# wonheeML/mtl-ssl

Measured on AMD Instinct MI355X. Metric: images/sec training, Faster R-CNN ResNet-101 + aux heads, higher is better.
Workload: dtype f32; 1 GPU; Faster R-CNN ResNet-101 + window/closeness/edgemask heads + refine, synthetic 1024x600 COCO-shaped (90 classes), per-GPU batch 2 (BASELINE.json configs[1]); global_batch=2, parallelism=dp1, pipeline_config=configs/frcnn_resnet101_coco_mtl.config

## Files before the change

### include/mtlssl_hip.h

```cpp
#ifndef MTLSSL_HIP_H_
#define MTLSSL_HIP_H_

#include <stdint.h>

#ifdef __cplusplus
extern "C" {
#endif

typedef void* mtlssl_stream_t;

#define MTLSSL_OK 0
#define MTLSSL_EINVAL (-1)
#define MTLSSL_ELAUNCH (-2)
#define MTLSSL_ECOMM (-3)

#define MTLSSL_ABI_VERSION 20

const char* mtlssl_last_error(void);
int mtlssl_abi_version(void);

int mtlssl_exp_rn(const double* x, double* y, int64_t n, mtlssl_stream_t stream);

typedef struct {
  int32_t N, H, W, C;
  int32_t K, R, S;
  int32_t OH, OW;
  int32_t stride, dilation;
  int32_t pad_t, pad_l;
  int32_t ldy;
} mtlssl_conv_desc;

#define MTLSSL_EPI_BIAS 1
#define MTLSSL_EPI_RESIDUAL 2
#define MTLSSL_EPI_RELU 4
#define MTLSSL_EPI_TANH 8
#define MTLSSL_EPI_RELU6 16
#define MTLSSL_EPI_MASK 32
#define MTLSSL_EPI_ACCUM 64
#define MTLSSL_EPI_MASK6 128

int64_t mtlssl_conv2d_workspace_bytes(const mtlssl_conv_desc* d, int mode);
int mtlssl_conv2d_fwd(const mtlssl_conv_desc* d, const float* x, const float* w,
                      const float* bias, const float* residual, float* y, int epilogue,
                      void* workspace, mtlssl_stream_t stream);
int mtlssl_conv2d_dgrad(const mtlssl_conv_desc* d, const float* dy, const float* w,
                        const float* residual, const float* mask_ref, float* dx, int epilogue,
                        void* workspace, mtlssl_stream_t stream);
int64_t mtlssl_conv2d_filter_xf_bytes(const mtlssl_conv_desc* d, int mode);
int mtlssl_conv2d_filter_xf_variant(const mtlssl_conv_desc* d, int mode);
int mtlssl_conv2d_transform_filter(const mtlssl_conv_desc* d, int mode, int variant, const float* w, float* filter_xf,
                                   mtlssl_stream_t stream);
int mtlssl_conv2d_transform_filters(int variant, int n, const void* w_ptrs, const void* xf_ptrs, const int64_t* ck,
                                    const int32_t* flip, int64_t max_ck, mtlssl_stream_t stream);
int mtlssl_conv2d_fwd_xf(const mtlssl_conv_desc* d, const float* x, const float* w, const float* bias,
                         const float* residual, float* y, int epilogue, void* workspace, const float* filter_xf,
                         int xf_variant, mtlssl_stream_t stream);
int mtlssl_conv2d_dgrad_xf(const mtlssl_conv_desc* d, const float* dy, const float* w, const float* residual,
                           const float* mask_ref, float* dx, int epilogue, void* workspace, const float* filter_xf,
                           int xf_variant, mtlssl_stream_t stream);
int64_t mtlssl_conv2d_input_xf_bytes(const mtlssl_conv_desc* d, int variant);
int mtlssl_conv2d_fwd_keep(const mtlssl_conv_desc* d, const float* x, const float* w, const float* bias,
                           const float* residual, float* y, int epilogue, void* workspace, const float* filter_xf,
                           int xf_variant, float* input_xf, int input_variant, mtlssl_stream_t stream);
int mtlssl_conv2d_wgrad_xf(const mtlssl_conv_desc* d, const float* x, const float* dy,
                           const float* out_scale, float* dw, float* dbias, float beta,
                           void* workspace, const float* input_xf, int input_variant, mtlssl_stream_t stream);
#define MTLSSL_CONV_GROUP_MAX 4
typedef struct {
  const float* w;
  float* y;
  const float* bias;
  int32_t K, ldy, epilogue, reserved;
} mtlssl_conv_group_entry;
int mtlssl_conv2d_fwd_grouped(const mtlssl_conv_desc* d, const float* x, int n, const mtlssl_conv_group_entry* entries,
                              int max_k, int sum_k, mtlssl_stream_t stream);
typedef struct {
  const float* dy;
  const float* w;
  int32_t K, ldy;
} mtlssl_conv_seg_entry;
int mtlssl_conv2d_dgrad_segmented(const mtlssl_conv_desc* d, int n, const mtlssl_conv_seg_entry* entries,
                                  const float* residual, const float* mask_ref, float* dx, int epilogue,
                                  mtlssl_stream_t stream);
int mtlssl_conv2d_wgrad_ex(const mtlssl_conv_desc* d, const float* x, const float* dy,
                           const float* out_scale, float* dw, float* dbias, const float* dbias_scale, float beta,
                           void* workspace, const float* input_xf, int input_variant, mtlssl_stream_t stream);
int64_t mtlssl_conv2d_wgrad_workspace_bytes(const mtlssl_conv_desc* d);
int mtlssl_conv2d_tile_config(const mtlssl_conv_desc* d, int mode);
int mtlssl_conv2d_force_config(const mtlssl_conv_desc* d, int mode, int cfg);
int mtlssl_conv2d_set_winograd(int mode);
int mtlssl_conv2d_set_pointwise(int on);
int mtlssl_conv2d_set_fp32_engine(int mode);
int mtlssl_conv2d_num_dispatches(const mtlssl_conv_desc* d, int mode);
#define MTLSSL_PLAN_INFO_LEN 16
#define MTLSSL_PLAN_DIRECT 0
#define MTLSSL_PLAN_PADDED 1
#define MTLSSL_PLAN_THIN 2
#define MTLSSL_PLAN_S2D 3
#define MTLSSL_PLAN_PARITY 4
#define MTLSSL_PLAN_WINO_F43 5
#define MTLSSL_PLAN_WINO_M7 6
#define MTLSSL_PLAN_VALU 7
int mtlssl_conv2d_plan_info(const mtlssl_conv_desc* d, int mode, int parity_class, int32_t* out);
int64_t mtlssl_conv2d_executed_macs(const mtlssl_conv_desc* d, int mode, int on_mfma);
int mtlssl_conv2d_wgrad(const mtlssl_conv_desc* d, const float* x, const float* dy,
                        const float* out_scale, float* dw, float* dbias, float beta,
                        void* workspace, mtlssl_stream_t stream);

int64_t mtlssl_conv2d_wgrad_grouped_workspace_bytes(const mtlssl_conv_desc* d, int n);
int mtlssl_conv2d_wgrad_grouped(const mtlssl_conv_desc* d, int n, const void* x_ptrs, const void* dy_ptrs,
                                const void* scale_ptrs, const void* dw_ptrs, float beta, void* workspace,
                                mtlssl_stream_t stream);

int mtlssl_depthwise_fwd(const mtlssl_conv_desc* d, const float* x, const float* w, const float* bias,
                         float* y, int epilogue, mtlssl_stream_t stream);
int mtlssl_depthwise_dgrad(const mtlssl_conv_desc* d, const float* dy, const float* w,
                           const float* mask_ref, float* dx, int epilogue, mtlssl_stream_t stream);
int64_t mtlssl_depthwise_wgrad_workspace_bytes(const mtlssl_conv_desc* d);
int mtlssl_depthwise_wgrad(const mtlssl_conv_desc* d, const float* x, const float* dy,
                           const float* out_scale, float* dw, float beta, void* workspace,
                           mtlssl_stream_t stream);
int64_t mtlssl_bn_param_grads_workspace_bytes(int C);
int mtlssl_bn_param_grads(const float* y, const float* g, const float* gamma, const float* beta,
                          float* dgamma, float* dbeta, int64_t rows, int C, float accum, void* workspace,
                          mtlssl_stream_t stream);

int mtlssl_avgpool_fwd(const float* x, float* y, int N, int H, int W, int C, int k, int stride, int pad_t,
                       int pad_l, int OH, int OW, mtlssl_stream_t stream);
int mtlssl_avgpool_bwd(const float* dy, float* dx, int N, int H, int W, int C, int k, int stride, int pad_t,
                       int pad_l, int OH, int OW, mtlssl_stream_t stream);
int mtlssl_copy_channels(const float* src, int src_ld, int src_c0, float* dst, int dst_ld, int dst_c0,
                         int64_t rows, int nc, int accumulate, mtlssl_stream_t stream);

int mtlssl_maxpool_fwd(const float* x, float* y, int N, int H, int W, int C, int k, int stride,
                       int pad_t, int pad_l, int OH, int OW, mtlssl_stream_t stream);
int mtlssl_maxpool_bwd(const float* x, const float* y, const float* dy, float* dx, int N, int H,
                       int W, int C, int k, int stride, int pad_t, int pad_l, int OH, int OW,
                       mtlssl_stream_t stream);
int mtlssl_maxpool_fwd_strided(const float* x, float* y, int N, int H, int W, int C, int k, int stride,
                               int pad_t, int pad_l, int OH, int OW, int ldy, mtlssl_stream_t stream);
int mtlssl_maxpool_bwd_strided(const float* x, const float* y, const float* dy, float* dx, int N, int H,
                               int W, int C, int k, int stride, int pad_t, int pad_l, int OH, int OW, int ldy,
                               mtlssl_stream_t stream);
int mtlssl_spatial_mean_fwd(const float* x, float* y, int N, int HW, int C, mtlssl_stream_t s);
int mtlssl_spatial_mean_bwd(const float* dy, float* dx, int N, int HW, int C, mtlssl_stream_t s);
int mtlssl_spatial_mean_bwd_masked(const float* dy, const float* act, float* dx, int N, int HW, int C,
                                   int relu6, mtlssl_stream_t stream);


int mtlssl_anchors_generate(float* anchors_out, int grid_h, int grid_w, const float* scales,
                            int n_scales, const float* aspect_ratios, int n_ratios, float base_h,
                            float base_w, float stride_y, float stride_x, float offset_y,
                            float offset_x, mtlssl_stream_t stream);

int mtlssl_boxes_prune_outside_window(const float* boxes, int n, float win_ymin, float win_xmin,
                                      float win_ymax, float win_xmax, int32_t* keep_idx_out,
                                      int32_t* count_out, mtlssl_stream_t stream);

int mtlssl_boxes_clip_to_window(const float* boxes, int n, float win_ymin, float win_xmin, float win_ymax,
                                float win_xmax, float* out, mtlssl_stream_t stream);
int mtlssl_gather_rows(const float* src, const int32_t* idx, float* dst, int batch, int n_src,
                       int n_idx, int row_len, mtlssl_stream_t stream);
int mtlssl_scatter_rows(const float* src, const int32_t* idx, float* dst, int batch, int n_dst,
                        int n_idx, int row_len, mtlssl_stream_t stream);

int mtlssl_boxes_decode(const float* rel_codes, const float* anchors, float* boxes_out, int batch,
                        int n, int anchors_batched, float sy, float sx, float sh, float sw,
                        mtlssl_stream_t stream);
int mtlssl_boxes_encode(const float* boxes, const float* anchors, float* codes_out, int n, float sy,
                        float sx, float sh, float sw, mtlssl_stream_t stream);

int64_t mtlssl_rpn_proposals_workspace_bytes(int batch, int n);
int mtlssl_rpn_proposals(const float* rpn_box_encodings, const float* rpn_objectness,
                         const float* anchors, int batch, int n, float img_h, float img_w,
                         float score_thresh, float iou_thresh, int max_proposals,
                         float* proposals_out, float* scores_out, int32_t* num_out,
                         void* workspace, mtlssl_stream_t stream);
int64_t mtlssl_batch_multiclass_nms_workspace_bytes(int batch, int n, int num_classes, int max_per_class);
int mtlssl_batch_multiclass_nms(const float* boxes, const float* scores, int scores_ld,
                                const int32_t* num_valid, int batch, int n, int q, int num_classes,
                                float score_thresh,
                                float iou_thresh, int max_per_class, int max_total,
                                const float* clip_window, int change_coordinate_frame, float* boxes_out,
                                float* scores_out, float* classes_out, int32_t* num_out, void* workspace,
                                mtlssl_stream_t stream);
int mtlssl_score_convert(const float* logits, float* out, int64_t rows, int C, int mode,
                         mtlssl_stream_t stream);
int64_t mtlssl_nms_workspace_bytes(int n);
int mtlssl_nms(const float* boxes, const float* scores, int n, float iou_thresh, int max_out,
               int32_t* selected_out, int32_t* num_out, void* workspace,
               mtlssl_stream_t stream);

#define MTLSSL_EVAL_NMS_MAX_SEGMENT 1024
#define MTLSSL_EVAL_NMS_STANDARD 1
#define MTLSSL_EVAL_NMS_SOFT_LINEAR 2
#define MTLSSL_EVAL_NMS_SOFT_GAUSSIAN 3
int mtlssl_eval_nms(const float* boxes, const float* scores, const int32_t* segment_offsets, int num_segments,
                    int max_segment, int nms_type, double iou_threshold, double sigma, double scale_y, double scale_x,
                    int max_output, int32_t* index_out, float* scores_out, int32_t* count_out,
                    mtlssl_stream_t stream);
int mtlssl_edgemask_agreement(const float* logits, int Hf, int Wf, const float* gt_mask, int h, int w,
                              int32_t* count_out, mtlssl_stream_t stream);
#define MTLSSL_COCO_MATCH_MAX_GT 256
int mtlssl_coco_match(const int32_t* dt_off, const int32_t* gt_off, int num_segments, int max_gt,
                      const double* dt_boxes, const double* gt_boxes, const double* gt_area, const uint8_t* gt_crowd,
                      const double* iou_thrs, int num_iou_thrs, const double* area_rng, int num_area_rng,
                      uint64_t* dt_match, uint64_t* dt_ignore, int32_t* npig, mtlssl_stream_t stream);
#define MTLSSL_PASCAL_MATCH_MAX_GT 256
#define MTLSSL_PASCAL_MATCH_LEFT_OUT 2
int mtlssl_pascal_match(const int32_t* dt_off, const int32_t* gt_off, int num_segments, int max_gt,
                        const double* dt_boxes, const double* gt_boxes, const uint64_t* gt_member,
                        double iou_threshold, int num_subsets, uint64_t* tp, uint64_t* drop, uint8_t* hit,
                        mtlssl_stream_t stream);

#define MTLSSL_AUX_MAX_GT 256
#define MTLSSL_AUX_WINDOW_ATTEMPTS 100
int mtlssl_aux_draw_windows(const float* boxes_norm, const int32_t* num, int batch, int max_gt, int num_windows,
                            double height, double width, double min_obj_size, uint32_t seed, uint32_t step,
                            uint32_t image0, float* window_boxes, mtlssl_stream_t stream);
int mtlssl_aux_window_labels(const float* boxes_norm, const float* classes_bg, const int32_t* num,
                             const float* window_boxes, int batch, int max_gt, int num_classes, int num_windows,
                             double height, double width, float* labels_out, mtlssl_stream_t stream);
int mtlssl_aux_closeness(const float* boxes_norm, const float* classes_bg, const int32_t* num, int batch, int max_gt,
                         int num_classes, double height, double width, float* closeness_out, mtlssl_stream_t stream);
int mtlssl_aux_edgemask(const float* boxes_norm, const int32_t* num, int batch, int max_gt, double height, double width,
                        int mask_size, float* edgemask_out, mtlssl_stream_t stream);

int64_t mtlssl_assign_targets_workspace_bytes(int batch, int n, int max_gt);
int mtlssl_assign_targets(const float* anchors, int anchors_batched, int batch, int n,
                          const float* gt_boxes, const int32_t* num_gt, int max_gt,
                          const float* gt_labels, int label_dim, const float* gt_extra,
                          int extra_dim, const float* unmatched_cls_target, float matched_thresh,
                          float unmatched_thresh, int force_match, int32_t* match_out,
                          float* cls_targets_out, float* cls_weights_out, float* reg_targets_out,
                          float* reg_weights_out, float* extra_targets_out, void* workspace,
                          mtlssl_stream_t stream);

int mtlssl_balanced_sample(const float* indicator, const float* labels, int batch, int n,
                           int batch_size, float positive_fraction, uint32_t seed,
                           uint32_t stream_id0, uint32_t stream_stride, float* sampled_out,
                           mtlssl_stream_t stream);

int mtlssl_sample_proposals(const float* proposals, const int32_t* num_proposals, int batch,
                            int max_p, const float* gt_boxes, const int32_t* num_gt, int max_gt,
// ... 156 lines not shown
```

### mtl_ssl_amd/csrc/conv.hip

```cpp
#include <stdlib.h>

#include <atomic>
#include <mutex>
#include <unordered_map>

#include "conv_mfma.h"
#include "conv_split.h"

namespace mtlssl {


__global__ void __launch_bounds__(256) k_wgrad_reduce(const float* ws, int nsplit, int64_t total4, int K,
                                                      const float* scale, float* dw, float beta, int main_blocks,
                                                      const float* cs_part, int cs_chunks, float* dbias,
                                                      const float* dbias_scale) {
  if ((int)blockIdx.x >= main_blocks) {
    const int lane = threadIdx.x & 63;
    const int k = ((int)blockIdx.x - main_blocks) * 4 + (threadIdx.x >> 6);
    if (k >= K) return;
    float s = 0.f;
    for (int c = lane; c < cs_chunks; c += 64) s += cs_part[(int64_t)c * K + k];
    s = wave_sum(s);
    if (dbias_scale) s *= dbias_scale[k];
    if (lane == 0) dbias[k] = beta != 0.f ? beta * dbias[k] + s : s;
    return;
  }
  const int64_t t = blockIdx.x * (int64_t)blockDim.x + threadIdx.x;
  const int64_t i = t >> 2;
  const int sl = (int)(t & 3);
  const bool live = i < total4;
  floatx4 s = {0.f, 0.f, 0.f, 0.f};
  if (live)
    for (int k = sl; k < nsplit; k += 4) s += reinterpret_cast<const floatx4*>(ws)[(int64_t)k * total4 + i];
#pragma unroll
  for (int e = 0; e < 4; ++e) {
    s[e] += __shfl_xor(s[e], 1, 64);
    s[e] += __shfl_xor(s[e], 2, 64);
  }
  if (!live || sl) return;
  if (scale) s *= *reinterpret_cast<const floatx4*>(scale + (i * 4) % K);
  floatx4* d = reinterpret_cast<floatx4*>(dw) + i;
  *d = beta != 0.f ? beta * *d + s : s;
}

__global__ void __launch_bounds__(256) k_wgrad_reduce_grouped(const float* ws, int nsplit, int64_t total4, int K,
                                                              const float* const* scale_tab, float* const* dw_tab,
                                                              float beta) {
  const int g = blockIdx.y;
  const int64_t t = blockIdx.x * (int64_t)blockDim.x + threadIdx.x;
  const int64_t i = t >> 2;
  const int sl = (int)(t & 3);
  const bool live = i < total4;
  const floatx4* w4 = reinterpret_cast<const floatx4*>(ws) + (int64_t)g * nsplit * total4;
  floatx4 s = {0.f, 0.f, 0.f, 0.f};
  if (live)
    for (int k = sl; k < nsplit; k += 4) s += w4[(int64_t)k * total4 + i];
#pragma unroll
  for (int e = 0; e < 4; ++e) {
    s[e] += __shfl_xor(s[e], 1, 64);
    s[e] += __shfl_xor(s[e], 2, 64);
  }
  if (!live || sl) return;
  const float* scale = scale_tab ? scale_tab[g] : nullptr;
  if (scale) s *= *reinterpret_cast<const floatx4*>(scale + (i * 4) % K);
  floatx4* d = reinterpret_cast<floatx4*>(dw_tab[g]) + i;
  *d = beta != 0.f ? beta * *d + s : s;
}

__global__ void k_conv_direct_fwd(ConvArgs p) {
  int64_t i = blockIdx.x * (int64_t)blockDim.x + threadIdx.x;
  int64_t total = (int64_t)p.M * p.K;
  if (i >= total) return;
  int k = i % p.K;
  int m = i / p.K;
  int ow = m % p.OW, t = m / p.OW, oh = t % p.OH, n = t / p.OH;
  float acc = 0.f;
  for (int r = 0; r < p.R; ++r) {
    int ih = oh * p.stride - p.pt + r * p.dil;
    if (ih < 0 || ih >= p.H) continue;
    for (int s = 0; s < p.S; ++s) {
      int iw = ow * p.stride - p.pl + s * p.dil;
      if (iw < 0 || iw >= p.W) continue;
      const float* xp = p.a + (((int64_t)n * p.H + ih) * p.W + iw) * p.C;
      const float* wp = p.b + ((int64_t)(r * p.S + s) * p.C) * p.K + k;
      for (int c = 0; c < p.C; ++c) acc = fmaf(xp[c], wp[(int64_t)c * p.K], acc);
    }
  }
  if (p.epi & MTLSSL_EPI_BIAS) acc += p.bias[k];
  if (p.epi & MTLSSL_EPI_RESIDUAL) acc += p.residual[i];
  if (p.epi & MTLSSL_EPI_RELU) acc = fmaxf(acc, 0.f);
  if (p.epi & MTLSSL_EPI_RELU6) acc = fminf(fmaxf(acc, 0.f), 6.f);
  if (p.epi & MTLSSL_EPI_TANH) acc = tanhf(acc);
  p.out[i] = acc;
}
__global__ void k_conv_direct_dgrad(ConvArgs p) {
  int64_t i = blockIdx.x * (int64_t)blockDim.x + threadIdx.x;
  int64_t total = (int64_t)p.M * p.C;
  if (i >= total) return;
  int c = i % p.C;
  int m = i / p.C;
  int iw = m % p.W, t = m / p.W, ih = t % p.H, n = t / p.H;
  float acc = 0.f;
  for (int r = 0; r < p.R; ++r) {
    int ny = ih + p.pt - r * p.dil;
    if (ny < 0 || ny % p.stride) continue;
    int oh = ny / p.stride;
    if (oh >= p.OH) continue;
    for (int s = 0; s < p.S; ++s) {
      int nx = iw + p.pl - s * p.dil;
      if (nx < 0 || nx % p.stride) continue;
      int ow = nx / p.stride;
      if (ow >= p.OW) continue;
      const float* gp = p.a + (((int64_t)n * p.OH + oh) * p.OW + ow) * p.K;
      const float* wp = p.b + ((int64_t)(r * p.S + s) * p.C + c) * p.K;
      for (int k = 0; k < p.K; ++k) acc = fmaf(gp[k], wp[k], acc);
    }
  }
  if (p.epi & MTLSSL_EPI_RESIDUAL) acc += p.residual[i];
  if (p.epi & MTLSSL_EPI_ACCUM) acc += p.out[i];
  if (p.epi & MASK_ANY) acc = act_mask(acc, p.mask[i], p.epi);
  p.out[i] = acc;
}
__global__ void k_conv_direct_wgrad(ConvArgs p, const float* scale, float* dw, float beta) {
  int rs = blockIdx.y, c = blockIdx.x;
  int r = rs / p.S, s = rs % p.S;
  int P = p.N * p.OH * p.OW;
  for (int k = threadIdx.x; k < p.K; k += blockDim.x) {
    float acc = 0.f;
    for (int pix = 0; pix < P; ++pix) {
      int ow = pix % p.OW, t = pix / p.OW, oh = t % p.OH, n = t / p.OH;
      int ih = oh * p.stride - p.pt + r * p.dil, iw = ow * p.stride - p.pl + s * p.dil;
      if (ih < 0 || ih >= p.H || iw < 0 || iw >= p.W) continue;
      acc = fmaf(p.a[(((int64_t)n * p.H + ih) * p.W + iw) * p.C + c], p.b[(int64_t)pix * p.K + k], acc);
    }
    if (scale) acc *= scale[k];
    int64_t o = ((int64_t)rs * p.C + c) * p.K + k;
    dw[o] = beta != 0.f ? beta * dw[o] + acc : acc;
  }
}

constexpr int STEM_MAX_CHUNKS = 512;
template <int R_, int S_, int C_>
__global__ void __launch_bounds__(256) k_conv_stem_wgrad(ConvArgs p, int pix_per_chunk, float* part) {
  constexpr int T = R_ * S_ * C_;
  const int KL = p.K <= 32 ? 32 : 64;
  const int k = threadIdx.x % KL, grp = threadIdx.x / KL, ngrp = 256 / KL;
  const int64_t P = (int64_t)p.N * p.OH * p.OW;
  int64_t p0 = (int64_t)blockIdx.x * pix_per_chunk;
  int64_t p1 = p0 + pix_per_chunk < P ? p0 + pix_per_chunk : P;
  float acc[T];
#pragma unroll
  for (int t = 0; t < T; ++t) acc[t] = 0.f;
  if (k < p.K) {
    for (int64_t pix = p0 + grp; pix < p1; pix += ngrp) {
      int ow = pix % p.OW;
      int64_t t2 = pix / p.OW;
      int oh = t2 % p.OH, n = t2 / p.OH;
      float g = p.b[pix * p.K + k];
#pragma unroll
      for (int r = 0; r < R_; ++r) {
        int ih = oh * p.stride - p.pt + r * p.dil;
#pragma unroll
        for (int s = 0; s < S_; ++s) {
// ... 1080 lines not shown
  p.b_bytes = (unsigned)((int64_t)d->R * d->S * d->C * d->K * 4);
  p.M = d->N * d->OH * d->OW;
  p.NG = d->K;
  MTLSSL_REQUIRE(desc_dense(d) || mfma_fwd_ok(d), "conv_fwd: a strided output (ldy = %d) needs C %% 16 == 0 and K >= 16", d->ldy);
  const Route r = route(d, MODE_FWD, workspace != nullptr);
  const mtlssl_conv_desc& q = r.q;
  switch (r.family == FAM_STEM_FWD ? stem_fwd_family(epi) : r.family) {
    case FAM_WINO:
      wino_fwd(d, r.wc.variant, r.wc.tile, x, w, bias, residual, y, epi, workspace, S(stream),
               (filter_xf && xf_variant == r.wc.variant) ? filter_xf : nullptr,
               (input_xf && input_variant == r.wc.variant) ? input_xf : nullptr);
      break;
    case FAM_DIRECT:
      launch_planned<MODE_FWD>(r.plan, p, (float*)workspace, S(stream));
      break;
    case FAM_PADDED: {
      float* x_pad = (float*)workspace;
      float* w_pad = (float*)((char*)workspace + r.front_a);
      hipLaunchKernelGGL(k_pad_rows, dim3(cdiv((int64_t)p.M * q.C, 256)), dim3(256), 0, S(stream), x, (int64_t)p.M, d->C, q.C, x_pad);
      (void)hipMemcpyAsync(w_pad, w, (size_t)d->C * d->K * 4, hipMemcpyDeviceToDevice, S(stream));
      (void)hipMemsetAsync(w_pad + (int64_t)d->C * d->K, 0, (size_t)(q.C - d->C) * d->K * 4, S(stream));
      launch_packed<MODE_FWD>(r, p, x_pad, w_pad, workspace, S(stream));
      break;
    }
    case FAM_THIN:
      hipLaunchKernelGGL(k_pw_thin_fwd, dim3(cdiv(p.M, 4)), dim3(256), 0, S(stream), x, w, bias, residual, y, p.M, d->C, d->K, epi);
      break;
    case FAM_GEMM_SMALL: {
      GemmArgs g{x, w, y, bias, residual, nullptr, p.M, d->K, d->C, epi, 0};
      hipLaunchKernelGGL(k_gemm_small<GM_FWD>, dim3(cdiv(g.N, 64), cdiv(g.M, 64)), dim3(256), 0, S(stream), g);
      break;
    }
    case FAM_S2D: {
      float* xs = (float*)workspace;
      float* wsf = (float*)((char*)workspace + r.front_a);
      hipLaunchKernelGGL(k_s2d_pack, dim3(cdiv((int64_t)q.N * q.H * q.W * 4, 256)), dim3(256), 0, S(stream), x, d->N, d->H, d->W,
                         d->C, d->pad_t, d->pad_l, q.H, q.W, xs);
      hipLaunchKernelGGL(k_s2d_filter, dim3(cdiv((int64_t)q.R * q.S * q.C * q.K, 256)), dim3(256), 0, S(stream), w, d->R, d->S,
                         d->C, d->K, q.R, q.S, wsf);
      launch_packed<MODE_FWD>(r, p, xs, wsf, workspace, S(stream));
      break;
    }
    case FAM_STEM_FWD: {
      dim3 grid(cdiv(d->OW, STEM_T), cdiv(d->OH, STEM_T), d->N);
      hipLaunchKernelGGL(k_conv_smallc_fwd, grid, dim3(256), stem_lds_bytes(d), S(stream), p);
      break;
    }
    default:
      hipLaunchKernelGGL(k_conv_direct_fwd, dim3(cdiv((int64_t)p.M * p.K, 256)), dim3(256), 0, S(stream), p);
  }
  return check_launch("conv2d_fwd");
}

int mtlssl_conv2d_fwd_grouped(const mtlssl_conv_desc* d, const float* x, int n, const mtlssl_conv_group_entry* entries,
                              int max_k, int sum_k, mtlssl_stream_t stream) {
  if (n <= 0) return MTLSSL_OK;
  if (int rc = check_desc(d)) return rc;
  MTLSSL_REQUIRE(is_pointwise(d) && d->dilation == 1, "fwd_grouped: pointwise problems only (1x1, stride 1, no padding)");
  MTLSSL_REQUIRE(d->C % BK == 0, "fwd_grouped: C = %d must be a multiple of %d", d->C, BK);
  MTLSSL_REQUIRE(x && entries && n <= MTLSSL_CONV_GROUP_MAX && max_k >= 16 && sum_k >= max_k, "fwd_grouped: bad arguments");
  ConvArgs p = make_args(d);
  GroupArgs ga;
  memset(&ga, 0, sizeof(ga));
  p.a = x;
  for (int i = 0; i < n; ++i) {
    const mtlssl_conv_group_entry& e = entries[i];
    MTLSSL_REQUIRE(e.w && e.y && e.K >= 16 && e.K % 4 == 0 && e.K <= max_k && (e.ldy == 0 || (e.ldy >= e.K && e.ldy % 4 == 0)) &&
                       !(e.epilogue & (MTLSSL_EPI_RESIDUAL | MASK_ANY | MTLSSL_EPI_ACCUM)) && (!(e.epilogue & MTLSSL_EPI_BIAS) || e.bias),
                   "fwd_grouped: problem %d: K = %d, ldy = %d, epilogue = %d", i, e.K, e.ldy, e.epilogue);
    ga.e[i] = e;
  }
  p.a_bytes = (unsigned)((int64_t)d->N * d->H * d->W * d->C * 4);
  p.M = d->N * d->H * d->W;
  p.NG = max_k; p.K = max_k; p.ldy = 0;
  p.nsplit = 1; p.ks_per_split = 0; p.tile_m0 = 0; p.ws_m0 = 0;
  int cfg = 2;
  double best = 1e30;
  for (int c = 0; c < NCFG; ++c) {
    const int64_t tiles = cdiv(p.M, CFG_BM[c]) * cdiv(sum_k, CFG_BN[c]);
    const double t = tile_time_us(c, tiles, d->C / CFG_BK[c], true);
    if (t < best) { best = t; cfg = c; }
  }
  p.tiles_m = (int)cdiv(p.M, CFG_BM[cfg]);
  p.tiles_n = (int)cdiv(max_k, CFG_BN[cfg]);
  dim3 grid(p.tiles_m * p.tiles_n, n, 1);
  switch (cfg) {
    case 0: hipLaunchKernelGGL((k_conv_mfma_pw_grp<128, 128>), grid, dim3(256), 0, S(stream), p, ga); break;
    case 1: hipLaunchKernelGGL((k_conv_mfma_pw_grp<128, 64>), grid, dim3(256), 0, S(stream), p, ga); break;
    case 2: hipLaunchKernelGGL((k_conv_mfma_pw_grp<64, 64>), grid, dim3(256), 0, S(stream), p, ga); break;
    default: hipLaunchKernelGGL((k_conv_mfma_pw_grp<256, 128>), grid, dim3(512), 0, S(stream), p, ga); break;
  }
  return check_launch("conv2d_fwd_grouped");
}

static int seg_dgrad_cfg_env() {
  static const int v = [] { const char* e = getenv("MTLSSL_SEG_DGRAD_CFG"); return e ? atoi(e) : -1; }();
  return v;
}
int mtlssl_conv2d_dgrad_segmented(const mtlssl_conv_desc* d, int n, const mtlssl_conv_seg_entry* entries,
                                  const float* residual, const float* mask_ref, float* dx, int epi,
                                  mtlssl_stream_t stream) {
  if (int rc = check_desc(d)) return rc;
  MTLSSL_REQUIRE(is_pointwise(d) && d->dilation == 1, "dgrad_segmented: pointwise problems only (1x1, stride 1, no padding)");
  MTLSSL_REQUIRE(entries && dx && n >= 1 && n <= MTLSSL_CONV_GROUP_MAX, "dgrad_segmented: bad arguments (n = %d)", n);
  MTLSSL_REQUIRE(d->C % 4 == 0 && d->C >= 16, "dgrad_segmented: C = %d must be a multiple of 4 and >= 16", d->C);
  MTLSSL_REQUIRE(!(epi & MASK_ANY) || mask_ref, "dgrad_segmented: mask_ref pointer required");
  MTLSSL_REQUIRE(!(epi & MTLSSL_EPI_RESIDUAL) || residual, "dgrad_segmented: residual pointer required");
  MTLSSL_REQUIRE(!(epi & ~(MTLSSL_EPI_RESIDUAL | MASK_ANY)), "dgrad_segmented: epilogue = %d (RESIDUAL / MASK / MASK6 only)", epi);
  const int64_t M = (int64_t)d->N * d->H * d->W;
  SegArgs sa;
  memset(&sa, 0, sizeof(sa));
  int sum_k = 0;
  for (int i = 0; i < n; ++i) {
    const mtlssl_conv_seg_entry& e = entries[i];
    MTLSSL_REQUIRE(e.dy && e.w && e.K >= BK && e.K % BK == 0 && (e.ldy == 0 || (e.ldy >= e.K && e.ldy % 4 == 0)),
                   "dgrad_segmented: segment %d: K = %d, ldy = %d", i, e.K, e.ldy);
    MTLSSL_REQUIRE(((M - 1) * (e.ldy ? e.ldy : e.K) + e.K) * 4 < (int64_t)1 << 32, "dgrad_segmented: segment %d exceeds 4 GiB", i);
    sa.e[i] = e;
    sum_k += e.K;
  }
  mtlssl_conv_desc q = *d;
  q.K = sum_k; q.ldy = 0;
  ConvArgs p = make_args(&q);
  p.a = entries[0].dy; p.b = entries[0].w; p.out = dx; p.residual = residual; p.mask = mask_ref; p.epi = epi;
  p.a_bytes = 0; p.b_bytes = 0;
  p.M = (int)M;
  p.NG = d->C;
  p.nsplit = 1; p.ks_per_split = 0; p.tile_m0 = 0; p.ws_m0 = 0;
  int cfg = seg_dgrad_cfg_env();
  if (cfg < 0 || cfg >= NCFG) {
    cfg = cdiv(p.M, CFG_BM[1]) * cdiv(p.NG, CFG_BN[1]) >= 512 ? 1 : 2;
  }
  p.tiles_m = (int)cdiv(p.M, CFG_BM[cfg]);
  p.tiles_n = (int)cdiv(p.NG, CFG_BN[cfg]);
  dim3 grid(p.tiles_m * p.tiles_n, 1, 1);
  switch (cfg) {
    case 0: hipLaunchKernelGGL((k_conv_mfma_pw_seg<128, 128>), grid, dim3(256), 0, S(stream), p, sa); break;
    case 1: hipLaunchKernelGGL((k_conv_mfma_pw_seg<128, 64>), grid, dim3(256), 0, S(stream), p, sa); break;
    case 2: hipLaunchKernelGGL((k_conv_mfma_pw_seg<64, 64>), grid, dim3(256), 0, S(stream), p, sa); break;
    default: hipLaunchKernelGGL((k_conv_mfma_pw_seg<256, 128>), grid, dim3(512), 0, S(stream), p, sa); break;
  }
  return check_launch("conv2d_dgrad_segmented");
}

int mtlssl_conv2d_dgrad(const mtlssl_conv_desc* d, const float* dy, const float* w,
                        const float* residual, const float* mask_ref, float* dx, int epi,
                        void* workspace, mtlssl_stream_t stream) {
  return mtlssl_conv2d_dgrad_xf(d, dy, w, residual, mask_ref, dx, epi, workspace, nullptr, -1, stream);
}

int mtlssl_conv2d_dgrad_xf(const mtlssl_conv_desc* d, const float* dy, const float* w,
                           const float* residual, const float* mask_ref, float* dx, int epi,
                           void* workspace, const float* filter_xf, int xf_variant, mtlssl_stream_t stream) {
  if (int rc = check_desc(d)) return rc;
  MTLSSL_REQUIRE(!(epi & MASK_ANY) || mask_ref, "conv_dgrad: mask_ref pointer required");
  MTLSSL_REQUIRE(!(epi & MTLSSL_EPI_RESIDUAL) || residual, "conv_dgrad: residual pointer required");
  ConvArgs p = make_args(d);
  p.a = dy; p.b = w; p.out = dx; p.residual = residual; p.mask = mask_ref; p.epi = epi;
  p.a_bytes = ydy_bytes(d);
  p.b_bytes = (unsigned)((int64_t)d->R * d->S * d->C * d->K * 4);
  p.M = d->N * d->H * d->W;
  p.NG = d->C;
  MTLSSL_REQUIRE(desc_dense(d) || mfma_dgrad_ok(d),
                 "conv_dgrad: a strided dy (ldy = %d) needs K %% 16 == 0, C %% 4 == 0 and C >= 16", d->ldy);
  const Route r = route(d, MODE_DGRAD, workspace != nullptr);
  switch (r.family) {
    case FAM_WINO:
      wino_dgrad(d, r.wc.variant, r.wc.tile, dy, w, residual, mask_ref, dx, epi, workspace, S(stream),
                 (filter_xf && xf_variant == r.wc.variant) ? filter_xf : nullptr);
      break;
    case FAM_PARITY:
      parity_dgrad(r, d, dy, w, residual, mask_ref, dx, epi, workspace, S(stream));
      break;
    case FAM_DIRECT:
      launch_planned<MODE_DGRAD>(r.plan, p, (float*)workspace, S(stream));
      break;
    case FAM_PADDED: {
      float* dy_pad = (float*)workspace;
      float* w_pad = (float*)((char*)workspace + r.front_a);
      hipLaunchKernelGGL(k_pad_rows, dim3(cdiv((int64_t)p.M * r.q.K, 256)), dim3(256), 0, S(stream), dy, (int64_t)p.M, d->K, r.q.K, dy_pad);
      hipLaunchKernelGGL(k_pad_rows, dim3(cdiv((int64_t)d->C * r.q.K, 256)), dim3(256), 0, S(stream), w, (int64_t)d->C, d->K, r.q.K, w_pad);
      launch_packed<MODE_DGRAD>(r, p, dy_pad, w_pad, workspace, S(stream));
      break;
    }
    case FAM_GEMM_SMALL: {
      GemmArgs g{dy, w, dx, nullptr, residual, mask_ref, p.M, d->C, d->K, epi, 0};
      hipLaunchKernelGGL(k_gemm_small<GM_DGRAD>, dim3(cdiv(g.N, 64), cdiv(g.M, 64)), dim3(256), 0, S(stream), g);
      break;
    }
    default:
      hipLaunchKernelGGL(k_conv_direct_dgrad, dim3(cdiv((int64_t)p.M * p.C, 256)), dim3(256), 0, S(stream), p);
  }
  return check_launch("conv2d_dgrad");
}

int mtlssl_conv2d_tile_config(const mtlssl_conv_desc* d, int mode) {
  if (!d || mode < MODE_FWD || mode > MODE_WGRAD) return -1;
  const Route r = route(d, mode);
  if (r.family == FAM_WINO) return make_code(1 + r.wc.variant, r.wc.tile);
  if (r.family != FAM_DIRECT && r.family != FAM_PARITY) return -1;
  return make_code(0, mode == MODE_WGRAD ? r.wg.cfg : r.plan.cfg);
}

int64_t mtlssl_conv2d_executed_macs(const mtlssl_conv_desc* d, int mode, int on_mfma) {
  if (!d || mode < MODE_FWD || mode > MODE_WGRAD || check_desc(d)) return 0;
  const int64_t P_out = (int64_t)d->N * d->OH * d->OW, P_in = (int64_t)d->N * d->H * d->W;
  const int64_t taps = (int64_t)d->R * d->S;
  const int64_t direct = (mode == MODE_DGRAD && d->stride == 1 ? P_in : P_out) * taps * d->C * d->K;
  const int64_t gathered = P_in * taps * d->C * d->K;
  const Route r = route(d, mode);
  const mtlssl_conv_desc& q = r.q;
  int64_t mfma = 0;
  switch (r.family) {
    case FAM_WINO: mfma = wino_input_bytes(d, r.wc.variant) / 4 * d->K; break;
    case FAM_DIRECT: mfma = mode == MODE_DGRAD ? gathered : direct; break;
    case FAM_PARITY: mfma = gathered / ((int64_t)d->stride * d->stride); break;
    case FAM_PADDED: mfma = (mode == MODE_DGRAD ? P_in : P_out) * q.C * q.K; break;
    case FAM_S2D: mfma = P_out * q.R * q.S * q.C * q.K; break;
    default: return on_mfma ? 0 : direct;
  }
  return on_mfma ? mfma : 0;
}

int mtlssl_conv2d_force_config(const mtlssl_conv_desc* d, int mode, int cfg) {
  MTLSSL_REQUIRE(d != nullptr && mode >= MODE_FWD && mode <= MODE_WGRAD, "force_config: bad arguments");
  MTLSSL_REQUIRE(cfg < CODE_END, "force_config: plan code out of range (0..%d)", CODE_END - 1);
  TunedKey k = make_key(d, mode);
  {
    std::lock_guard<std::mutex> g(tuned_mutex());
    if (cfg < 0) tuned_map().erase(k); else tuned_map()[k] = cfg;
  }
  routes_clear();
  return MTLSSL_OK;
}

int mtlssl_conv2d_set_fp32_engine(int mode) {
  const int prev = fp32_engine();
  if (mode == 0 || mode == 1) fp32_engine_ref().store(mode);
  return prev;
}

int mtlssl_conv2d_set_winograd(int mode) {
  const int prev = wino_env();
  if (mode >= 0 && mode <= 2) { wino_mode_ref().store(mode); routes_clear(); }
  return prev;
}

int mtlssl_conv2d_set_pointwise(int on) {
  const int prev = pointwise_ref().load();
  if (on == 0 || on == 1) pointwise_ref().store(on);
  return prev;
}

int mtlssl_conv2d_num_dispatches(const mtlssl_conv_desc* d, int mode) {
  if (!d) return 0;
  if (mode != MODE_FWD && mode != MODE_DGRAD) return 1;
  const Route r = route(d, mode);
  return (r.family == FAM_DIRECT || r.family == FAM_PARITY) && r.plan.tail_rows > 0 ? 2 : 1;
}

static void plan_info_gemm(const Plan& pl, int64_t M, int64_t NG, int ksteps, int32_t* out) {
  out[2] = pl.cfg; out[3] = pl.nsplit; out[4] = pl.ks_per_split;
  out[5] = pl.tail_rows; out[6] = pl.tail_rows > 0 ? pl.tail_nsplit : 0; out[7] = pl.tail_rows > 0 ? pl.tail_ks : 0;
  out[8] = ksteps; out[9] = (int32_t)M; out[10] = (int32_t)NG; out[11] = CFG_BM[pl.cfg]; out[12] = CFG_BN[pl.cfg];
}
int mtlssl_conv2d_plan_info(const mtlssl_conv_desc* d, int mode, int parity_class, int32_t* out) {
  MTLSSL_REQUIRE(d != nullptr && out != nullptr && mode >= MODE_FWD && mode <= MODE_WGRAD, "plan_info: bad arguments");
  if (int rc = check_desc(d)) return rc;
  static const int32_t PUBLIC[] = {MTLSSL_PLAN_WINO_F43, MTLSSL_PLAN_DIRECT, MTLSSL_PLAN_PARITY, MTLSSL_PLAN_PADDED, MTLSSL_PLAN_S2D,
                                   MTLSSL_PLAN_THIN,     MTLSSL_PLAN_VALU,   MTLSSL_PLAN_VALU,   MTLSSL_PLAN_VALU,   MTLSSL_PLAN_VALU};
  const Route r = route(d, mode);
  const mtlssl_conv_desc& q = r.q;
  for (int i = 0; i < MTLSSL_PLAN_INFO_LEN; ++i) out[i] = 0;
  out[0] = PUBLIC[r.family];
  out[1] = mtlssl_conv2d_tile_config(d, mode);
  out[2] = -1;
  out[14] = mtlssl_conv2d_num_dispatches(d, mode);
  const int64_t P = (int64_t)d->N * d->OH * d->OW, M = mode == MODE_FWD ? P : (int64_t)d->N * d->H * d->W;
  switch (r.family) {
    case FAM_WINO:
      if (r.wc.variant != 0) out[0] = MTLSSL_PLAN_WINO_M7;
      out[2] = r.wc.tile; out[3] = 1;
      out[9] = (int32_t)(mode == MODE_WGRAD ? d->C : M);
      out[10] = mode == MODE_DGRAD ? d->C : d->K;
      out[11] = CFG_BM[r.wc.tile]; out[12] = CFG_BN[r.wc.tile];
      break;
    case FAM_PARITY: {
      MTLSSL_REQUIRE(parity_class >= 0 && parity_class < 4, "plan_info: parity class %d of an input-parity dgrad", parity_class);
      const ParityProblem c = parity_problem(d, parity_class >> 1, parity_class & 1);
      if (c.Hs == 0 || c.Ws == 0 || c.Rs == 0 || c.Ss == 0) break;
      const Plan& pl = r.parity[parity_class];
      plan_info_gemm(pl, (int64_t)d->N * c.Hs * c.Ws, d->C, c.Rs * c.Ss * (d->K / CFG_BK[pl.cfg]), out);
      break;
    }
    case FAM_DIRECT: case FAM_PADDED: case FAM_S2D:
      if (mode == MODE_WGRAD) {
        const int cfg = r.wg.cfg;
        out[2] = cfg; out[3] = r.wg.nsplit; out[4] = r.wg.pps / CFG_BK[cfg]; out[8] = (int32_t)cdiv(P, CFG_BK[cfg]);
        out[9] = q.C; out[10] = q.K; out[11] = CFG_BM[cfg]; out[12] = CFG_BN[cfg]; out[13] = r.wg.pps;
      } else {
        plan_info_gemm(r.plan, M, mode == MODE_FWD ? q.K : q.C, q.R * q.S * ((mode == MODE_FWD ? q.C : q.K) / CFG_BK[r.plan.cfg]), out);
      }
      break;
    default: break;
  }
  return MTLSSL_OK;
}

int64_t mtlssl_conv2d_wgrad_workspace_bytes(const mtlssl_conv_desc* d) {
  if (!d) return 256;
  return colsum_bytes(d) + route(d, MODE_WGRAD).bytes;
}

static void wgrad_group_plan(const mtlssl_conv_desc* d, int n, int* cfg, int* nsplit, int* pps) {
  const int64_t P = (int64_t)d->N * d->OH * d->OW;
  const int RS = d->R * d->S;
  double best_t = 1e30;
  *cfg = 2; *nsplit = 1; *pps = (int)align_up(P, 16);
  for (int c = 0; c < NCFG; ++c) {
    const int ksteps = (int)cdiv(P, CFG_BK[c]);
    const int64_t tiles = cdiv(d->C, CFG_BM[c]) * cdiv(d->K, CFG_BN[c]) * RS * n;
    for (int s = 1; s <= 16; ++s) {
      if (s > 1 && ksteps * CFG_BK[c] / s < 128) break;
      const int per = (int)cdiv(ksteps, s), ns = (int)cdiv(ksteps, per);
      if (ns != s) continue;
      const double t = tile_time_us(c, tiles * ns, per, desc_is_pointwise(d)) + 2.0 + (double)n * RS * d->C * d->K * 4.0 * (ns + 1) / 3.0e6;
      if (t < best_t) { best_t = t; *cfg = c; *nsplit = ns; *pps = per * CFG_BK[c]; }
    }
  }
}
int64_t mtlssl_conv2d_wgrad_grouped_workspace_bytes(const mtlssl_conv_desc* d, int n) {
  if (!d || n <= 0 || check_desc(d) || !mfma_wgrad_ok(d)) return 0;
  int cfg, ns, pps;
  wgrad_group_plan(d, n, &cfg, &ns, &pps);
  return align_up((int64_t)n * ns * d->R * d->S * d->C * d->K * 4, 256);
}
int mtlssl_conv2d_wgrad_grouped(const mtlssl_conv_desc* d, int n, const void* x_ptrs, const void* dy_ptrs,
                                const void* scale_ptrs, const void* dw_ptrs, float beta, void* workspace,
                                mtlssl_stream_t stream) {
  if (n <= 0) return MTLSSL_OK;
  if (int rc = check_desc(d)) return rc;
  MTLSSL_REQUIRE(mfma_wgrad_ok(d), "wgrad_grouped: the problem is not on the MFMA path (C, K multiples of 4 and >= 16)");
  MTLSSL_REQUIRE(x_ptrs && dy_ptrs && dw_ptrs && workspace, "wgrad_grouped: null table / workspace");
  MTLSSL_REQUIRE(n <= 1024, "wgrad_grouped: at most 1024 problems per launch");
  hipStream_t st = S(stream);
  ConvArgs p = make_args(d);
  p.a_bytes = (unsigned)((int64_t)d->N * d->H * d->W * d->C * 4);
  p.b_bytes = ydy_bytes(d);
  p.a_tab = (const float* const*)x_ptrs;
  p.b_tab = (const float* const*)dy_ptrs;
  int cfg, ns, pps;
  wgrad_group_plan(d, n, &cfg, &ns, &pps);
  MTLSSL_REQUIRE((int64_t)n * ns <= 65535, "wgrad_grouped: grid too large");
  p.out = (float*)workspace;
  p.M = d->C; p.NG = d->K; p.nsplit = ns; p.pix_per_split = pps;
  launch_mfma<MODE_WGRAD>(cfg, p, dim3(1, d->R * d->S, n * ns), st);
  const int64_t total4 = (int64_t)d->R * d->S * d->C * d->K / 4;
  hipLaunchKernelGGL(k_wgrad_reduce_grouped, dim3(cdiv(total4 * 4, 256), n), dim3(256), 0, st, (const float*)workspace, ns,
                     total4, d->K, (const float* const*)scale_ptrs, (float* const*)dw_ptrs, beta);
  return check_launch("conv2d_wgrad_grouped");
}

int mtlssl_conv2d_wgrad(const mtlssl_conv_desc* d, const float* x, const float* dy,
                        const float* out_scale, float* dw, float* dbias, float beta,
                        void* workspace, mtlssl_stream_t stream) {
  return mtlssl_conv2d_wgrad_xf(d, x, dy, out_scale, dw, dbias, beta, workspace, nullptr, -1, stream);
}

int mtlssl_conv2d_wgrad_xf(const mtlssl_conv_desc* d, const float* x, const float* dy,
                           const float* out_scale, float* dw, float* dbias, float beta,
                           void* workspace, const float* input_xf, int input_variant, mtlssl_stream_t stream) {
  return mtlssl_conv2d_wgrad_ex(d, x, dy, out_scale, dw, dbias, nullptr, beta, workspace, input_xf, input_variant, stream);
}

int mtlssl_conv2d_wgrad_ex(const mtlssl_conv_desc* d, const float* x, const float* dy,
                           const float* out_scale, float* dw, float* dbias, const float* dbias_scale, float beta,
                           void* workspace, const float* input_xf, int input_variant, mtlssl_stream_t stream) {
  if (int rc = check_desc(d)) return rc;
  hipStream_t st = S(stream);
  ConvArgs p = make_args(d);
  p.a = x; p.b = dy;
  p.a_bytes = (unsigned)((int64_t)d->N * d->H * d->W * d->C * 4);
  p.b_bytes = ydy_bytes(d);
  const int ldy = desc_ldy(d);
  MTLSSL_REQUIRE(desc_dense(d) || mfma_wgrad_ok(d),
                 "conv_wgrad: a strided dy (ldy = %d) needs C, K %% 4 == 0 and C, K >= 16", d->ldy);
  int64_t P = (int64_t)d->N * d->OH * d->OW;
  MTLSSL_REQUIRE(workspace != nullptr, "conv_wgrad: workspace required");
  float* ws_main = (float*)((char*)workspace + colsum_bytes(d));
  ColsumPlan cp = colsum_plan(P, d->K);
  bool colsum_folded = false;
  auto colsum_partial = [&]() {
    const int kg = (int)cdiv(d->K, (d->K & 3) ? 1 : 4);
    dim3 grid(cdiv(kg, cp.CQ), cp.chunks);
    if (d->K & 3)
      hipLaunchKernelGGL(k_colsum_partial<float>, grid, dim3(256), 0, st, dy, (int)P, d->K, ldy, cp.per_chunk, cp.CQ,
                         (float*)workspace);
    else
      hipLaunchKernelGGL(k_colsum_partial<floatx4>, grid, dim3(256), 0, st, dy, (int)P, d->K, ldy, cp.per_chunk, cp.CQ,
                         (float*)workspace);
  };
  const Route r = route(d, MODE_WGRAD);
  switch (r.family) {
    case FAM_WINO:
      wino_wgrad(d, r.wc.variant, r.wc.tile, x, dy, out_scale, dw, beta, ws_main, st,
                 (input_xf && input_variant == r.wc.variant) ? input_xf : nullptr);
      break;
    case FAM_DIRECT: {
      const bool split = wgrad_on_split_engine(r, d);
      const int ns = split ? r.split_ns : r.wg.nsplit, pps = split ? r.split_pps : r.wg.pps;
      const bool ride = dbias && !split && ns <= COLSUM_MAX_PARTS;
      if (dbias && !ride) colsum_partial();
      p.out = ws_main;
      p.M = d->C; p.NG = d->K; p.nsplit = ns; p.pix_per_split = pps;
      p.cs_part = ride ? (float*)workspace : nullptr;
      if (split) launch_split<MODE_WGRAD, false>(p, dim3(1, d->R * d->S, ns), st);
      else launch_mfma<MODE_WGRAD>(r.wg.cfg, p, dim3(1, d->R * d->S, ns), st);
      int64_t total4 = (int64_t)d->R * d->S * d->C * d->K / 4;
      const int main_blocks = (int)cdiv(total4 * 4, 256);
      hipLaunchKernelGGL(k_wgrad_reduce, dim3(main_blocks + (dbias ? (int)cdiv(d->K, 4) : 0)), dim3(256), 0, st,
                         (const float*)ws_main, ns, total4, d->K, out_scale, dw, beta, main_blocks,
                         (const float*)workspace, ride ? ns : cp.chunks, dbias, dbias_scale);
      colsum_folded = dbias != nullptr;
      break;
    }
    case FAM_PADDED: {
      const mtlssl_conv_desc& q = r.q;
      const int ns = r.wg.nsplit;
      float* dy_pad = ws_main;
      float* ws_q = (float*)((char*)ws_main + r.front_bytes);
      hipLaunchKernelGGL(k_pad_rows, dim3(cdiv(P * q.K, 256)), dim3(256), 0, st, dy, P, d->K, q.K, dy_pad);
      ConvArgs pq = make_args(&q);
      pq.a = x; pq.b = dy_pad; pq.out = ws_q;
      pq.a_bytes = p.a_bytes; pq.b_bytes = (unsigned)(P * q.K * 4);
      pq.M = q.C; pq.NG = q.K; pq.nsplit = ns; pq.pix_per_split = r.wg.pps;
      const bool ride = dbias && (int64_t)ns * q.K <= (int64_t)COLSUM_MAX_PARTS * d->K;
      pq.cs_part = ride ? (float*)workspace : nullptr;
      launch_mfma<MODE_WGRAD>(r.wg.cfg, pq, dim3(1, 1, ns), st);
      const int main_blocks = (int)cdiv((int64_t)d->C * d->K, 256);
      hipLaunchKernelGGL(k_wgrad_reduce_unpad, dim3(main_blocks + (ride ? (int)cdiv(d->K, 256) : 0)), dim3(256), 0, st,
                         (const float*)ws_q, ns, d->C, q.K, d->K, out_scale, dw, beta, main_blocks, (const float*)workspace,
                         dbias, dbias_scale);
      colsum_folded = ride;
      break;
    }
    case FAM_GEMM_SMALL: {
      GemmArgs g{x, dy, ws_main, nullptr, nullptr, nullptr, d->C, d->K, (int)P, 0, r.wg.pps};
      hipLaunchKernelGGL(k_gemm_small<GM_WGRAD>, dim3(cdiv(g.N, 64), cdiv(g.M, 64), r.wg.nsplit), dim3(256), 0, st, g);
      int64_t total = (int64_t)d->C * d->K;
      hipLaunchKernelGGL(k_small_reduce, dim3(cdiv(total, 256)), dim3(256), 0, st, (const float*)ws_main, r.wg.nsplit,
                         total, d->K, out_scale, dw, beta);
      break;
    }
    case FAM_STEM3_WGRAD: {
      hipLaunchKernelGGL((k_conv_stem_wgrad<3, 3, 3>), dim3(r.wg.nsplit), dim3(256), 0, st, p, r.wg.pps, ws_main);
      int64_t total = (int64_t)27 * d->K;
      hipLaunchKernelGGL(k_small_reduce, dim3(cdiv(total, 256)), dim3(256), 0, st, (const float*)ws_main, r.wg.nsplit,
                         total, d->K, out_scale, dw, beta);
      break;
    }
    default:
      hipLaunchKernelGGL(k_conv_direct_wgrad, dim3(d->C, d->R * d->S), dim3(64), 0, st, p, out_scale, dw, beta);
  }
  if (dbias && !colsum_folded) {
    colsum_partial();
    hipLaunchKernelGGL(k_colsum_fold, dim3(cdiv(d->K, 4)), dim3(256), 0, st, (const float*)workspace, cp.chunks, d->K,
                       dbias, beta, dbias_scale);
  }
  return check_launch("conv2d_wgrad");
}

}
```

### mtl_ssl_amd/csrc/conv_mfma.h

```cpp
#pragma once
#include <type_traits>

#include "common.h"

namespace mtlssl {

typedef float floatx16 __attribute__((ext_vector_type(16)));
typedef float floatx4 __attribute__((ext_vector_type(4)));

enum { MODE_FWD = 0, MODE_DGRAD = 1, MODE_WGRAD = 2 };
__device__ __forceinline__ float act_mask(float g, float y, int epi) {
  bool on = y > 0.f && (!(epi & MTLSSL_EPI_MASK6) || y < 6.f);
  return on ? g : 0.f;
}
constexpr int MASK_ANY = MTLSSL_EPI_MASK | MTLSSL_EPI_MASK6;
constexpr int BK = 16;
#ifndef MTLSSL_LAB_FLAGS
#define MTLSSL_LAB_FLAGS 0
#endif
constexpr int LAB = MTLSSL_LAB_FLAGS;

struct ConvArgs {
  const float* a;
  const float* b;
  float* out;
  const float* bias;
  const float* residual;
  const float* mask;
  float* splitk_ws;
  int N, H, W, C, K, R, S, OH, OW, stride, dil, pt, pl;
  int M;
  int NG;
  int epi;
  int tiles_m, tiles_n;
  unsigned a_bytes, b_bytes;
  int nsplit;
  int ks_per_split;
  int pix_per_split;
  int tile_m0;
  int ws_m0;
  int ldy;
  float* cs_part;
  int64_t a_bs, b_bs, o_bs;
  const float* const* a_tab;
  const float* const* b_tab;
};

typedef unsigned uintx4 __attribute__((ext_vector_type(4)));
__host__ __device__ __forceinline__ int args_ldy(const ConvArgs& p) { return p.ldy ? p.ldy : p.K; }

__device__ __forceinline__ floatx4 bufload4(__amdgpu_buffer_rsrc_t rsrc, unsigned voffset,
                                            unsigned soffset) {
  return __builtin_bit_cast(floatx4, __builtin_amdgcn_raw_buffer_load_b128(rsrc, voffset, soffset, 0));
}

template <int BM, int BN, int MODE, int NW, bool PREFETCH_RES = false>
__device__ __forceinline__ void conv_epilogue(const ConvArgs& p, floatx16 (&acc)[BM / (16 * NW)][BN / 64], float* smem,
                                              int m0, int n0) {
  constexpr int WR = NW / 2, TM = BM / (32 * WR), TN = BN / 64, LDT = 36;
  const int tid = threadIdx.x, lane = tid & 63, wid = tid >> 6;
  const int wr = wid >> 1, wc = wid & 1;
  const int lo = lane & 31, hi = lane >> 5;
  if constexpr (LAB & 16)
    if (p.epi != 0x7fffffff) {
      float t = 0.f;
#pragma unroll
      for (int i = 0; i < TM; ++i)
#pragma unroll
        for (int j = 0; j < TN; ++j)
#pragma unroll
          for (int e = 0; e < 16; ++e) t += acc[i][j][e];
      if (t == 1.2345e-30f) p.out[0] = t;
      return;
    }
  const int ldo = p.NG;
  const int ldf = MODE == MODE_FWD ? args_ldy(p) : p.NG;
  float* outp = p.out;
  if constexpr (MODE == MODE_WGRAD)
    outp += ((int64_t)blockIdx.z * gridDim.y + blockIdx.y) * (int64_t)p.M * p.NG;
  const bool raw = (MODE != MODE_WGRAD) && p.nsplit > 1;
  if (raw) outp = p.splitk_ws + (int64_t)blockIdx.z * (int64_t)(p.M - p.ws_m0) * p.NG;
  if (!(p.NG & 3)) {
    float* tile = smem + wid * (32 * LDT);
    const int r_in = lane >> 3, c4 = (lane & 7) * 4;
    const bool use_res = PREFETCH_RES && !raw && (MODE == MODE_FWD || MODE == MODE_DGRAD) && (p.epi & MTLSSL_EPI_RESIDUAL);
    floatx4 res_cur[4], res_nxt[4];
    auto fetch_res = [&](int t, floatx4 (&dst)[4]) {
      const int i = t / TN, j = t % TN;
      const int col = n0 + wc * (BN / 2) + j * 32 + c4;
#pragma unroll
      for (int k = 0; k < 4; ++k) {
        const int row = m0 + wr * (BM / WR) + i * 32 + r_in + 8 * k;
        dst[k] = floatx4{0.f, 0.f, 0.f, 0.f};
        if (use_res && row < p.M && col < p.NG) dst[k] = *reinterpret_cast<const floatx4*>(p.residual + (int64_t)row * ldo + col);
      }
    };
    if constexpr (PREFETCH_RES) fetch_res(0, res_cur);
#pragma unroll
    for (int i = 0; i < TM; ++i) {
#pragma unroll
      for (int j = 0; j < TN; ++j) {
        if constexpr (PREFETCH_RES)
          if (i * TN + j + 1 < TM * TN) fetch_res(i * TN + j + 1, res_nxt);
#pragma unroll
        for (int e = 0; e < 16; ++e) tile[((e & 3) + 8 * (e >> 2) + 4 * hi) * LDT + lo] = acc[i][j][e];
        const int col = n0 + wc * (BN / 2) + j * 32 + c4;
        floatx4 bv = {0.f, 0.f, 0.f, 0.f};
        if constexpr (MODE == MODE_FWD)
          if ((p.epi & MTLSSL_EPI_BIAS) && col < p.NG && !raw) bv = *reinterpret_cast<const floatx4*>(p.bias + col);
#pragma unroll
        for (int k = 0; k < 4; ++k) {
          const int rt = r_in + 8 * k;
          floatx4 v = *reinterpret_cast<const floatx4*>(tile + rt * LDT + c4);
          const int row = m0 + wr * (BM / WR) + i * 32 + rt;
          if (row >= p.M || col >= p.NG) continue;
          if (raw) {
            *reinterpret_cast<floatx4*>(outp + (int64_t)(row - p.ws_m0) * ldo + col) = v;
            continue;
          }
          const int64_t o = (int64_t)row * ldo + col;
          const int64_t of = MODE == MODE_FWD ? (int64_t)row * ldf + col : o;
          if constexpr (MODE == MODE_FWD) {
            v += bv;
            if (p.epi & MTLSSL_EPI_RESIDUAL) v += PREFETCH_RES ? res_cur[k] : *reinterpret_cast<const floatx4*>(p.residual + o);
#pragma unroll
            for (int q = 0; q < 4; ++q) {
              if (p.epi & MTLSSL_EPI_RELU) v[q] = fmaxf(v[q], 0.f);
              if (p.epi & MTLSSL_EPI_RELU6) v[q] = fminf(fmaxf(v[q], 0.f), 6.f);
              if (p.epi & MTLSSL_EPI_TANH) v[q] = tanhf(v[q]);
            }
          } else if constexpr (MODE == MODE_DGRAD) {
            if (p.epi & MTLSSL_EPI_RESIDUAL) v += PREFETCH_RES ? res_cur[k] : *reinterpret_cast<const floatx4*>(p.residual + o);
            if (p.epi & MTLSSL_EPI_ACCUM) v += *reinterpret_cast<const floatx4*>(outp + o);
            if (p.epi & MASK_ANY) {
              floatx4 mk = *reinterpret_cast<const floatx4*>(p.mask + o);
#pragma unroll
              for (int q = 0; q < 4; ++q) v[q] = act_mask(v[q], mk[q], p.epi);
            }
          }
          *reinterpret_cast<floatx4*>(outp + of) = v;
        }
        if constexpr (PREFETCH_RES) {
#pragma unroll
          for (int k = 0; k < 4; ++k) res_cur[k] = res_nxt[k];
        }
      }
    }
    return;
  }
#pragma unroll
  for (int i = 0; i < TM; ++i) {
#pragma unroll
    for (int j = 0; j < TN; ++j) {
      const int col = n0 + wc * (BN / 2) + j * 32 + lo;
      const bool col_ok = col < p.NG;
      float bv = 0.f;
      if constexpr (MODE == MODE_FWD)
        if ((p.epi & MTLSSL_EPI_BIAS) && col_ok) bv = p.bias[col];
#pragma unroll
      for (int e = 0; e < 16; ++e) {
        const int row = m0 + wr * (BM / WR) + i * 32 + (e & 3) + 8 * (e >> 2) + 4 * hi;
        if (row >= p.M || !col_ok) continue;
        const int64_t o = (int64_t)row * ldo + col;
        const int64_t of = MODE == MODE_FWD ? (int64_t)row * ldf + col : o;
        float v = acc[i][j][e];
        if (raw) {
          outp[(int64_t)(row - p.ws_m0) * ldo + col] = v;
          continue;
        }
        if constexpr (MODE == MODE_FWD) {
          v += bv;
          if (p.epi & MTLSSL_EPI_RESIDUAL) v += p.residual[o];
          if (p.epi & MTLSSL_EPI_RELU) v = fmaxf(v, 0.f);
          if (p.epi & MTLSSL_EPI_RELU6) v = fminf(fmaxf(v, 0.f), 6.f);
          if (p.epi & MTLSSL_EPI_TANH) v = tanhf(v);
        } else if constexpr (MODE == MODE_DGRAD) {
          if (p.epi & MTLSSL_EPI_RESIDUAL) v += p.residual[o];
          if (p.epi & MTLSSL_EPI_ACCUM) v += outp[o];
          if (p.epi & MASK_ANY) v = act_mask(v, p.mask[o], p.epi);
        }
        outp[of] = v;
      }
    }
  }
}

struct SegArgs { mtlssl_conv_seg_entry e[MTLSSL_CONV_GROUP_MAX]; };
template <int BM, int BN, int MODE, int BKT, bool BATCH, bool PW = false, bool CS = false, bool SEG = false>
__device__ __forceinline__ void conv_mfma_body(ConvArgs p, const SegArgs sg = SegArgs{}) {
  static_assert(!SEG || (PW && MODE == MODE_DGRAD && !BATCH), "segments: pointwise dgrad only");
  constexpr int NW = BM > 128 ? 8 : 4, NT = 64 * NW, WR = NW / 2;
  constexpr int LDA = BM + 4, LDB = BN + 4;
  constexpr int KQ = BKT / 4;
  constexpr int RP = NT / KQ;
  constexpr int TM = BM / (32 * WR), TN = BN / 64;
  constexpr bool A_KC = (MODE != MODE_WGRAD);
  constexpr bool B_KC = (MODE == MODE_DGRAD);
  constexpr int A_LD = BM / RP, B_LD = BN / RP;
  constexpr unsigned OOB = 0xFFFFFFF0u;
  constexpr int LDT = 36;
  constexpr int SMEM_OPS = 2 * BKT * (LDA + LDB), SMEM_EPI = NW * 32 * LDT;
  __shared__ __attribute__((aligned(16))) float smem[SMEM_OPS > SMEM_EPI ? SMEM_OPS : SMEM_EPI];
  float* const sA = smem;
  float* const sB = smem + 2 * BKT * LDA;

  int nwg = p.tiles_m * p.tiles_n;
  int bid = blockIdx.x;
  {
    int q = nwg / 8, r = nwg % 8, xcd = bid % 8, loc = bid / 8;
    bid = (xcd < r ? xcd * (q + 1) : r * (q + 1) + (xcd - r) * q) + loc;
  }
  const int tile_m = bid / p.tiles_n + p.tile_m0, tile_n = bid % p.tiles_n;
  const int m0 = tile_m * BM, n0 = tile_n * BN;
  const int tid = threadIdx.x, lane = tid & 63, wid = tid >> 6;
  const int wr = wid >> 1, wc = wid & 1;
  const int lo = lane & 31, hi = lane >> 5;
  const int kq4 = (tid % KQ) * 4;

  if constexpr (BATCH) {
    p.a += (int64_t)blockIdx.y * p.a_bs;
    p.b += (int64_t)blockIdx.y * p.b_bs;
    if constexpr (MODE != MODE_WGRAD) p.out += (int64_t)blockIdx.y * p.o_bs;
  }
  if constexpr (MODE == MODE_WGRAD && !BATCH) {
    if (p.a_tab) {
      const int grp = blockIdx.z / p.nsplit;
      p.a = p.a_tab[grp];
      p.b = p.b_tab[grp];
    }
  }
  const int ldy = args_ldy(p);
  int rs_fixed = 0, pix0 = 0, pix1 = 0, ksteps, ks_begin = 0;
  if constexpr (MODE == MODE_FWD) {
    ksteps = p.R * p.S * (p.C / BKT);
  } else if constexpr (MODE == MODE_DGRAD) {
    ksteps = p.R * p.S * (p.K / BKT);
  } else {
    rs_fixed = BATCH ? 0 : blockIdx.y;
    int split = (!BATCH && p.a_tab) ? blockIdx.z % p.nsplit : blockIdx.z;
    int P = p.N * p.OH * p.OW;
    pix0 = split * p.pix_per_split;
    pix1 = min(P, pix0 + p.pix_per_split);
    ksteps = (max(pix1 - pix0, 0) + BKT - 1) / BKT;
  }
  unsigned a_rec = p.a_bytes, b_rec = p.b_bytes;
  if constexpr (PW && MODE == MODE_WGRAD) {
    a_rec = min(a_rec, (unsigned)(max(pix1, 0) * p.C) * 4u);
    b_rec = min(b_rec, (unsigned)(max(pix1, 0) * ldy) * 4u);
  }
  __amdgpu_buffer_rsrc_t rsrc_a = __builtin_amdgcn_make_buffer_rsrc(const_cast<float*>(p.a), 0, a_rec, 0x00020000);
  __amdgpu_buffer_rsrc_t rsrc_b = __builtin_amdgcn_make_buffer_rsrc(const_cast<float*>(p.b), 0, b_rec, 0x00020000);
  if constexpr (MODE != MODE_WGRAD) {
    if (p.nsplit > 1) {
      ks_begin = blockIdx.z * p.ks_per_split;
      ksteps = min(ksteps, ks_begin + p.ks_per_split);
    }
  }

  int a_base[A_LD], a_y[A_LD], a_x[A_LD], a_n[A_LD];
  bool a_ok[A_LD];
  unsigned a_voff[A_LD];
  unsigned b_base[B_LD];
  if constexpr (PW && MODE == MODE_WGRAD) {
#pragma unroll
    for (int i = 0; i < A_LD; ++i) {
      const int u = tid + NT * i;
      const int col = m0 + (u % (BM / 4)) * 4;
      a_voff[i] = col < p.M ? (unsigned)((pix0 + u / (BM / 4)) * p.C + col) * 4u : OOB;
    }
  } else if constexpr (PW) {
#pragma unroll
    for (int i = 0; i < A_LD; ++i) {
      const int m = m0 + (tid / KQ) + RP * i;
      const int ld = MODE == MODE_FWD ? p.C : ldy;
      a_voff[i] = m < p.M ? (unsigned)(m * ld + kq4) * 4u : OOB;
    }
  } else if constexpr (A_KC) {
#pragma unroll
    for (int i = 0; i < A_LD; ++i) {
      int m = m0 + (tid / KQ) + RP * i;
      a_ok[i] = m < p.M;
      int mm = a_ok[i] ? m : 0;
      if constexpr (MODE == MODE_FWD) {
        int ow = mm % p.OW, t = mm / p.OW;
        a_x[i] = ow * p.stride - p.pl;
        a_y[i] = (t % p.OH) * p.stride - p.pt;
        a_n[i] = t / p.OH;
        a_base[i] = ((a_n[i] * p.H + a_y[i]) * p.W + a_x[i]) * p.C + kq4;
      } else {
        int iw = mm % p.W, t = mm / p.W;
        a_x[i] = iw + p.pl;
        a_y[i] = (t % p.H) + p.pt;
        a_n[i] = t / p.H;
        a_base[i] = ((a_n[i] * p.OH + a_y[i]) * p.OW + a_x[i]) * ldy + kq4;
      }
    }
  }
#pragma unroll
  for (int i = 0; i < B_LD; ++i) {
    if constexpr (MODE == MODE_FWD) {
      int u = tid + NT * i;
      int col = n0 + (u % (BN / 4)) * 4;
      b_base[i] = col < p.NG ? (unsigned)((u / (BN / 4)) * p.K + col) * 4u : OOB;
    } else if constexpr (MODE == MODE_DGRAD) {
      int row = n0 + (tid / KQ) + RP * i;
      b_base[i] = row < p.NG ? (unsigned)(row * p.K + kq4) * 4u : OOB;
    } else {
      int u = tid + NT * i;
      int col = n0 + (u % (BN / 4)) * 4;
      if constexpr (PW)
        b_base[i] = col < p.NG ? (unsigned)((pix0 + u / (BN / 4)) * ldy + col) * 4u : OOB;
      else
        b_base[i] = col < p.NG ? (unsigned)col * 4u : OOB;
    }
  }

  int seg_ks0 = 0;
  int seg_b[MTLSSL_CONV_GROUP_MAX] = {0, 0, 0, 0};
  auto seg_setup = [&](auto SI) {
    constexpr int s = decltype(SI)::value;
    const int e_K = sg.e[s].K;
    const int ld = sg.e[s].ldy ? sg.e[s].ldy : e_K;
    rsrc_a = __builtin_amdgcn_make_buffer_rsrc(const_cast<float*>(sg.e[s].dy), 0, (unsigned)((p.M - 1) * ld + e_K) * 4u, 0x00020000);
    rsrc_b = __builtin_amdgcn_make_buffer_rsrc(const_cast<float*>(sg.e[s].w), 0, (unsigned)(p.NG * e_K) * 4u, 0x00020000);
#pragma unroll
    for (int i = 0; i < A_LD; ++i) {
      const int m = m0 + (tid / KQ) + RP * i;
      a_voff[i] = m < p.M ? (unsigned)(m * ld + kq4) * 4u : OOB;
    }
#pragma unroll
    for (int i = 0; i < B_LD; ++i) {
      const int row = n0 + (tid / KQ) + RP * i;
      b_base[i] = row < p.NG ? (unsigned)(row * e_K + kq4) * 4u : OOB;
    }
    seg_ks0 = seg_b[s];
  };
  if constexpr (SEG) {
    static_assert(MTLSSL_CONV_GROUP_MAX == 4, "the boundary ladder in load_tile covers four segments");
    int at = 0;
#pragma unroll
    for (int s = 0; s < MTLSSL_CONV_GROUP_MAX; ++s) {
      seg_b[s] = sg.e[s].K > 0 ? at : 0x7fffffff;
      at += sg.e[s].K / BKT;
    }
    seg_setup(std::integral_constant<int, 0>{});
  }

  int t_r = 0, t_s = 0, t_c = 0;
  if constexpr (!PW && MODE != MODE_WGRAD) {
    const int cpk = (MODE == MODE_FWD ? p.C : p.K) / BKT;
    const int rs = ks_begin / cpk;
    t_c = (ks_begin - rs * cpk) * BKT;
    t_r = rs / p.S;
    t_s = rs - t_r * p.S;
  }
  auto next_tap = [&]() {
    t_c += BKT;
    if (t_c >= (MODE == MODE_FWD ? p.C : p.K)) {
      t_c = 0;
      if (++t_s == p.S) { t_s = 0; ++t_r; }
    }
  };
  int w_n[A_LD], w_oh[A_LD], w_ow[A_LD];
  if constexpr (!PW && MODE == MODE_WGRAD) {
#pragma unroll
    for (int i = 0; i < A_LD; ++i) {
      const int pix = pix0 + (tid + NT * i) / (BM / 4);
      w_ow[i] = pix % p.OW;
      const int t = pix / p.OW;
      w_oh[i] = t % p.OH;
      w_n[i] = t / p.OH;
    }
  }

  floatx4 rA[2][A_LD], rB[2][B_LD];
  using Set0 = std::integral_constant<int, 0>;
  using Set1 = std::integral_constant<int, 1>;

  auto load_tile = [&](int ks, auto SET) {
    floatx4 (&ra)[A_LD] = rA[decltype(SET)::value];
    floatx4 (&rb)[B_LD] = rB[decltype(SET)::value];
    if constexpr (PW && MODE == MODE_WGRAD) {
      const unsigned sa = (unsigned)(ks * BKT * p.C) * 4u, sb = (unsigned)(ks * BKT * ldy) * 4u;
#pragma unroll
      for (int i = 0; i < A_LD; ++i) ra[i] = bufload4(rsrc_a, __builtin_elementwise_add_sat(a_voff[i], sa), 0);
#pragma unroll
      for (int i = 0; i < B_LD; ++i) rb[i] = bufload4(rsrc_b, __builtin_elementwise_add_sat(b_base[i], sb), 0);
    } else if constexpr (PW) {
      if constexpr (SEG) {
        if (ks == seg_b[1]) seg_setup(std::integral_constant<int, 1>{});
        else if (ks == seg_b[2]) seg_setup(std::integral_constant<int, 2>{});
        else if (ks == seg_b[3]) seg_setup(std::integral_constant<int, 3>{});
      }
      const unsigned ka = (unsigned)((SEG ? ks - seg_ks0 : ks) * BKT) * 4u;
#pragma unroll
      for (int i = 0; i < A_LD; ++i) ra[i] = bufload4(rsrc_a, a_voff[i], ka);
      const unsigned so = MODE == MODE_FWD ? (unsigned)(ks * BKT * p.K) * 4u : ka;
#pragma unroll
      for (int i = 0; i < B_LD; ++i) rb[i] = bufload4(rsrc_b, b_base[i], so);
      if constexpr (MODE == MODE_FWD)
        if (p.NG & 3) {
#pragma unroll
          for (int i = 0; i < B_LD; ++i) {
            int left = p.NG - (n0 + ((tid + NT * i) % (BN / 4)) * 4);
#pragma unroll
            for (int e = 1; e < 4; ++e) rb[i][e] = e < left ? rb[i][e] : 0.f;
          }
        }
    } else if constexpr (MODE == MODE_FWD) {
      const int dy = t_r * p.dil, dx = t_s * p.dil;
      const int tapoff = (dy * p.W + dx) * p.C + t_c;
      next_tap();
#pragma unroll
      for (int i = 0; i < A_LD; ++i) {
        int ih = a_y[i] + dy, iw = a_x[i] + dx;
        bool ok = a_ok[i] && (unsigned)ih < (unsigned)p.H && (unsigned)iw < (unsigned)p.W;
        ra[i] = bufload4(rsrc_a, ok ? (unsigned)(a_base[i] + tapoff) * 4u : OOB, 0);
      }
      unsigned so = (unsigned)(ks * BKT * p.K) * 4u;
#pragma unroll
      for (int i = 0; i < B_LD; ++i) rb[i] = bufload4(rsrc_b, b_base[i], so);
      if (p.NG & 3) {
#pragma unroll
        for (int i = 0; i < B_LD; ++i) {
          int left = p.NG - (n0 + ((tid + NT * i) % (BN / 4)) * 4);
#pragma unroll
          for (int e = 1; e < 4; ++e) rb[i][e] = e < left ? rb[i][e] : 0.f;
        }
      }
    } else if constexpr (MODE == MODE_DGRAD) {
      const int rs = t_r * p.S + t_s, k0 = t_c;
      const int dy = t_r * p.dil, dx = t_s * p.dil;
      next_tap();
      if (p.stride == 1) {
        int tapoff = k0 - (dy * p.OW + dx) * ldy;
#pragma unroll
        for (int i = 0; i < A_LD; ++i) {
          int oh = a_y[i] - dy, ow = a_x[i] - dx;
          bool ok = a_ok[i] && (unsigned)oh < (unsigned)p.OH && (unsigned)ow < (unsigned)p.OW;
          ra[i] = bufload4(rsrc_a, ok ? (unsigned)(a_base[i] + tapoff) * 4u : OOB, 0);
        }
      } else {
#pragma unroll
        for (int i = 0; i < A_LD; ++i) {
          int ny = a_y[i] - dy, nx = a_x[i] - dx;
          bool ok = a_ok[i] && ny >= 0 && nx >= 0 && (ny % p.stride == 0) && (nx % p.stride == 0);
          int oh = ny / p.stride, ow = nx / p.stride;
          ok = ok && oh < p.OH && ow < p.OW;
          int off = ((a_n[i] * p.OH + oh) * p.OW + ow) * ldy + k0 + kq4;
          ra[i] = bufload4(rsrc_a, ok ? (unsigned)off * 4u : OOB, 0);
        }
      }
      unsigned so = (unsigned)(rs * p.C * p.K + k0) * 4u;
#pragma unroll
      for (int i = 0; i < B_LD; ++i) rb[i] = bufload4(rsrc_b, b_base[i], so);
    } else {
      int r = rs_fixed / p.S, s = rs_fixed - r * p.S;
#pragma unroll
      for (int i = 0; i < A_LD; ++i) {
        int u = tid + NT * i;
        int kr = u / (BM / 4), m4 = u % (BM / 4);
        int pix = pix0 + ks * BKT + kr;
        bool ok = pix < pix1;
        const int ih = w_oh[i] * p.stride - p.pt + r * p.dil, iw = w_ow[i] * p.stride - p.pl + s * p.dil;
        ok = ok && (unsigned)ih < (unsigned)p.H && (unsigned)iw < (unsigned)p.W && (m0 + m4 * 4) < p.M;
        const int off = ((w_n[i] * p.H + ih) * p.W + iw) * p.C;
        ra[i] = bufload4(rsrc_a, ok ? (unsigned)(off + m0 + m4 * 4) * 4u : OOB, 0);
        w_ow[i] += BKT;
        while (w_ow[i] >= p.OW) {
          w_ow[i] -= p.OW;
          if (++w_oh[i] == p.OH) { w_oh[i] = 0; ++w_n[i]; }
        }
      }
#pragma unroll
      for (int i = 0; i < B_LD; ++i) {
        int u = tid + NT * i;
        int pix = pix0 + ks * BKT + u / (BN / 4);
        rb[i] = bufload4(rsrc_b, (pix < pix1 && b_base[i] != OOB) ? b_base[i] + (unsigned)(pix * ldy) * 4u : OOB, 0);
      }
    }
  };

  static_assert(!CS || (MODE == MODE_WGRAD && !BATCH), "column sums ride on the plain wgrad launch only");
  bool do_cs = false;
  floatx4 cs[CS ? B_LD : 1];
  if constexpr (CS) {
    do_cs = p.cs_part != nullptr && tile_m == 0 && rs_fixed == 0 && p.a_tab == nullptr;
#pragma unroll
    for (int i = 0; i < B_LD; ++i) cs[i] = floatx4{0.f, 0.f, 0.f, 0.f};
  }
  auto store_tile = [&](int buf, auto SET) {
    floatx4 (&ra)[A_LD] = rA[decltype(SET)::value];
    floatx4 (&rb)[B_LD] = rB[decltype(SET)::value];
    float* a = sA + buf * (BKT * LDA);
    float* b = sB + buf * (BKT * LDB);
    if constexpr (CS)
      if (do_cs) {
#pragma unroll
        for (int i = 0; i < B_LD; ++i) cs[i] += rb[i];
      }
#pragma unroll
    for (int i = 0; i < A_LD; ++i) {
      if constexpr (A_KC) {
        int row = (tid / KQ) + RP * i;
        a[(kq4 + 0) * LDA + row] = ra[i].x; a[(kq4 + 1) * LDA + row] = ra[i].y;
        a[(kq4 + 2) * LDA + row] = ra[i].z; a[(kq4 + 3) * LDA + row] = ra[i].w;
      } else {
        int u = tid + NT * i;
        *reinterpret_cast<floatx4*>(a + (u / (BM / 4)) * LDA + (u % (BM / 4)) * 4) = ra[i];
      }
    }
#pragma unroll
    for (int i = 0; i < B_LD; ++i) {
      if constexpr (B_KC) {
        int row = (tid / KQ) + RP * i;
        b[(kq4 + 0) * LDB + row] = rb[i].x; b[(kq4 + 1) * LDB + row] = rb[i].y;
        b[(kq4 + 2) * LDB + row] = rb[i].z; b[(kq4 + 3) * LDB + row] = rb[i].w;
      } else {
        int u = tid + NT * i;
        *reinterpret_cast<floatx4*>(b + (u / (BN / 4)) * LDB + (u % (BN / 4)) * 4) = rb[i];
      }
    }
  };

  floatx16 acc[TM][TN];
#pragma unroll
  for (int i = 0; i < TM; ++i)
#pragma unroll
    for (int j = 0; j < TN; ++j)
#pragma unroll
      for (int e = 0; e < 16; ++e) acc[i][j][e] = 0.f;

  const int nk = ksteps - ks_begin;
  if (nk > 0) {
    load_tile(ks_begin, Set0{});
    store_tile(0, Set0{});
  }
  if (nk > 1) load_tile(ks_begin + 1, Set1{});
  __syncthreads();
  auto kstep = [&](int it, auto next, auto spare) {
    const int cur = it & 1;
    if constexpr (!(LAB & 1))
      if (it + 2 < nk) load_tile(ks_begin + it + 2, spare);
    const float* a = sA + cur * (BKT * LDA) + wr * (BM / WR) + lo;
    const float* b = sB + cur * (BKT * LDB) + wc * (BN / 2) + lo;
    float fa[2][TM], fb[2][TN];
#pragma unroll
    for (int i = 0; i < TM; ++i) fa[0][i] = a[hi * LDA + i * 32];
#pragma unroll
    for (int j = 0; j < TN; ++j) fb[0][j] = b[hi * LDB + j * 32];
#pragma unroll
    for (int kk = 0; kk < BKT / 2; ++kk) {
      const int cs = kk & 1, ns = cs ^ 1;
      if (kk + 1 < BKT / 2) {
        const int kr = 2 * (kk + 1) + hi;
        if constexpr (LAB & 8) {
#pragma unroll
          for (int i = 0; i < TM; ++i) fa[ns][i] = fa[cs][i] * 1.0001f;
#pragma unroll
          for (int j = 0; j < TN; ++j) fb[ns][j] = fb[cs][j] * 0.9999f;
        } else {
#pragma unroll
          for (int i = 0; i < TM; ++i) fa[ns][i] = a[kr * LDA + i * 32];
#pragma unroll
          for (int j = 0; j < TN; ++j) fb[ns][j] = b[kr * LDB + j * 32];
        }
      }
      __builtin_amdgcn_sched_barrier(0);
#pragma unroll
      for (int i = 0; i < TM; ++i)
#pragma unroll
        for (int j = 0; j < TN; ++j)
          acc[i][j] = __builtin_amdgcn_mfma_f32_32x32x2f32(fa[cs][i], fb[cs][j], acc[i][j], 0, 0, 0);
      __builtin_amdgcn_sched_barrier(0);
    }
    if constexpr (!(LAB & 2))
      if (it + 1 < nk) store_tile(cur ^ 1, next);
    if constexpr (!(LAB & 4)) __syncthreads();
  };
  for (int it = 0; it < nk; it += 2) {
    kstep(it, Set1{}, Set0{});
    if (it + 1 < nk) kstep(it + 1, Set0{}, Set1{});
  }

  if constexpr (CS) {
    if (do_cs) {
      floatx4* red = reinterpret_cast<floatx4*>(smem);
#pragma unroll
      for (int i = 0; i < B_LD; ++i) red[tid + NT * i] = cs[i];
      __syncthreads();
      if (tid < BN / 4) {
        floatx4 t = red[tid];
#pragma unroll
        for (int r = 1; r < BKT; ++r) t += red[r * (BN / 4) + tid];
        const int col = n0 + tid * 4;
        if (col < p.NG) *reinterpret_cast<floatx4*>(p.cs_part + (int64_t)blockIdx.z * p.NG + col) = t;
      }
      __syncthreads();
    }
  }
  conv_epilogue<BM, BN, MODE, NW>(p, acc, smem, m0, n0);
}


template <int BM, int BN, int MODE, int BKT, int NSTAGE, bool BATCH, bool PWISE = false, bool CS = false>
__device__ __forceinline__ void conv_glds_body(ConvArgs p) {
  constexpr int NW = BM > 128 ? 8 : 4, WR = NW / 2;
  constexpr int TM = BM / (32 * WR), TN = BN / 64;
  constexpr bool A_KC = (MODE != MODE_WGRAD);
  constexpr bool B_KC = (MODE == MODE_DGRAD);
  constexpr int QPR = BKT / 4;
  constexpr int RPP = 64 / QPR;
  constexpr int RSH = QPR == 4 ? 2 : 1;
  constexpr int A_FL = BM * BKT, B_FL = BN * BKT;
  constexpr int STAGE = A_FL + B_FL;
  constexpr int PA = BM * BKT / 256 / NW, PB = BN * BKT / 256 / NW;
  constexpr int G = BKT / 8;
  constexpr unsigned OOB = 0xFFFFFFF0u;
  constexpr int LDT = 36;
  constexpr int SMEM_OPS = NSTAGE * STAGE, SMEM_EPI = NW * 32 * LDT;
  __shared__ __attribute__((aligned(16))) float smem[SMEM_OPS > SMEM_EPI ? SMEM_OPS : SMEM_EPI];
  typedef __attribute__((address_space(3))) void* lds_ptr_t;

  int nwg = p.tiles_m * p.tiles_n;
  int bid = blockIdx.x;
  {
    int q = nwg / 8, r = nwg % 8, xcd = bid % 8, loc = bid / 8;
    bid = (xcd < r ? xcd * (q + 1) : r * (q + 1) + (xcd - r) * q) + loc;
  }
  const int tile_m = bid / p.tiles_n + p.tile_m0, tile_n = bid % p.tiles_n;
  const int m0 = tile_m * BM, n0 = tile_n * BN;
  const int tid = threadIdx.x, lane = tid & 63, wid = tid >> 6;
  const int wr = wid >> 1, wc = wid & 1;
  const int lo = lane & 31, hi = lane >> 5;
  auto kc_row = [&](int piece) { return piece * RPP + lane / QPR; };
  auto kc_quad4 = [&](int row) { return (((lane % QPR) ^ ((row >> RSH) & (QPR - 1)))) * 4; };

  if constexpr (BATCH) {
    p.a += (int64_t)blockIdx.y * p.a_bs;
    p.b += (int64_t)blockIdx.y * p.b_bs;
    if constexpr (MODE != MODE_WGRAD) p.out += (int64_t)blockIdx.y * p.o_bs;
  }
  int rs_fixed = 0, pix0 = 0, pix1 = 0, ksteps, ks_begin = 0;
  if constexpr (MODE == MODE_FWD) {
    ksteps = p.R * p.S * (p.C / BKT);
  } else if constexpr (MODE == MODE_DGRAD) {
    ksteps = p.R * p.S * (p.K / BKT);
  } else {
    rs_fixed = BATCH ? 0 : blockIdx.y;
    int split = blockIdx.z;
    int P = p.N * p.OH * p.OW;
    pix0 = split * p.pix_per_split;
    pix1 = min(P, pix0 + p.pix_per_split);
    ksteps = (max(pix1 - pix0, 0) + BKT - 1) / BKT;
  }
  if constexpr (MODE != MODE_WGRAD) {
    if (p.nsplit > 1) {
      ks_begin = blockIdx.z * p.ks_per_split;
      ksteps = min(ksteps, ks_begin + p.ks_per_split);
    }
  }

  const int ldy = args_ldy(p);
  unsigned a_rec = p.a_bytes, b_rec = p.b_bytes;
  if constexpr (PWISE && MODE == MODE_WGRAD) {
    a_rec = min(a_rec, (unsigned)(max(pix1, 0) * p.C) * 4u);
    b_rec = min(b_rec, (unsigned)(max(pix1, 0) * ldy) * 4u);
  }
  const __amdgpu_buffer_rsrc_t rsrc_a = __builtin_amdgcn_make_buffer_rsrc(const_cast<float*>(p.a), 0, a_rec, 0x00020000);
  const __amdgpu_buffer_rsrc_t rsrc_b = __builtin_amdgcn_make_buffer_rsrc(const_cast<float*>(p.b), 0, b_rec, 0x00020000);

  int a_base[PA], a_y[PA], a_x[PA], a_n[PA], a_q4[PA];
  bool a_ok[PA];
  unsigned a_voff[PA];
  unsigned b_base[PB];
  if constexpr (PWISE && MODE == MODE_WGRAD) {
#pragma unroll
    for (int i = 0; i < PA; ++i) {
      const int pos = (wid * PA + i) * 64 + lane;
      const int col = m0 + (pos % (BM / 4)) * 4;
      a_voff[i] = col < p.M ? (unsigned)((pix0 + pos / (BM / 4)) * p.C + col) * 4u : OOB;
    }
  } else if constexpr (PWISE) {
#pragma unroll
    for (int i = 0; i < PA; ++i) {
      const int row = kc_row(wid * PA + i);
      const int m = m0 + row;
      a_voff[i] = m < p.M ? (unsigned)(m * (MODE == MODE_FWD ? p.C : ldy) + kc_quad4(row)) * 4u : OOB;
    }
  } else if constexpr (A_KC) {
#pragma unroll
    for (int i = 0; i < PA; ++i) {
      const int row = kc_row(wid * PA + i);
      a_q4[i] = kc_quad4(row);
      int m = m0 + row;
      a_ok[i] = m < p.M;
      int mm = a_ok[i] ? m : 0;
      if constexpr (MODE == MODE_FWD) {
        int ow = mm % p.OW, t = mm / p.OW;
        a_x[i] = ow * p.stride - p.pl;
        a_y[i] = (t % p.OH) * p.stride - p.pt;
        a_n[i] = t / p.OH;
        a_base[i] = ((a_n[i] * p.H + a_y[i]) * p.W + a_x[i]) * p.C + a_q4[i];
      } else {
        int iw = mm % p.W, t = mm / p.W;
        a_x[i] = iw + p.pl;
        a_y[i] = (t % p.H) + p.pt;
        a_n[i] = t / p.H;
        a_base[i] = ((a_n[i] * p.OH + a_y[i]) * p.OW + a_x[i]) * ldy + a_q4[i];
      }
    }
  }
#pragma unroll
  for (int i = 0; i < PB; ++i) {
    const int pos = (wid * PB + i) * 64 + lane;
    if constexpr (MODE == MODE_FWD) {
      int col = n0 + (pos % (BN / 4)) * 4;
      b_base[i] = col < p.NG ? (unsigned)((pos / (BN / 4)) * p.K + col) * 4u : OOB;
    } else if constexpr (MODE == MODE_DGRAD) {
      const int row = kc_row(wid * PB + i);
      b_base[i] = n0 + row < p.NG ? (unsigned)((n0 + row) * p.K + kc_quad4(row)) * 4u : OOB;
    } else {
      int col = n0 + (pos % (BN / 4)) * 4;
      if constexpr (PWISE)
        b_base[i] = col < p.NG ? (unsigned)((pix0 + pos / (BN / 4)) * ldy + col) * 4u : OOB;
      else
        b_base[i] = col < p.NG ? (unsigned)col * 4u : OOB;
    }
  }

  auto issue_tile = [&](int ks, int st) {
    if constexpr (LAB & 32) ks = ks_begin;
    float* sa = smem + st * STAGE + wid * (PA * 256);
    float* sb = smem + st * STAGE + A_FL + wid * (PB * 256);
    if constexpr (PWISE && MODE == MODE_WGRAD) {
      const unsigned sa_off = (unsigned)(ks * BKT * p.C) * 4u, sb_off = (unsigned)(ks * BKT * ldy) * 4u;
#pragma unroll
      for (int i = 0; i < PA; ++i)
        __builtin_amdgcn_raw_ptr_buffer_load_lds(rsrc_a, (lds_ptr_t)(sa + i * 256), 16, __builtin_elementwise_add_sat(a_voff[i], sa_off), 0, 0, 0);
#pragma unroll
      for (int i = 0; i < PB; ++i)
        __builtin_amdgcn_raw_ptr_buffer_load_lds(rsrc_b, (lds_ptr_t)(sb + i * 256), 16, __builtin_elementwise_add_sat(b_base[i], sb_off), 0, 0, 0);
    } else if constexpr (PWISE) {
      const unsigned ka = (unsigned)(ks * BKT) * 4u;
      const unsigned so = MODE == MODE_FWD ? (unsigned)(ks * BKT * p.K) * 4u : ka;
#pragma unroll
      for (int i = 0; i < PA; ++i)
        __builtin_amdgcn_raw_ptr_buffer_load_lds(rsrc_a, (lds_ptr_t)(sa + i * 256), 16, a_voff[i], ka, 0, 0);
#pragma unroll
      for (int i = 0; i < PB; ++i)
        __builtin_amdgcn_raw_ptr_buffer_load_lds(rsrc_b, (lds_ptr_t)(sb + i * 256), 16, b_base[i], so, 0, 0);
    } else if constexpr (MODE == MODE_FWD) {
      int cpk = p.C / BKT;
      int rs = ks / cpk, c0 = (ks - rs * cpk) * BKT;
      int r = rs / p.S, s = rs - r * p.S;
      int dy = r * p.dil, dx = s * p.dil;
      int tapoff = (dy * p.W + dx) * p.C + c0;
      if constexpr (!(LAB & 64)) {
#pragma unroll
        for (int i = 0; i < PA; ++i) {
          int ih = a_y[i] + dy, iw = a_x[i] + dx;
          bool ok = a_ok[i] && (unsigned)ih < (unsigned)p.H && (unsigned)iw < (unsigned)p.W;
          __builtin_amdgcn_raw_ptr_buffer_load_lds(rsrc_a, (lds_ptr_t)(sa + i * 256), 16,
                                                   ok ? (unsigned)(a_base[i] + tapoff) * 4u : OOB, 0, 0, 0);
        }
      }
      unsigned so = (unsigned)(ks * BKT * p.K) * 4u;
      if constexpr (!(LAB & 128)) {
#pragma unroll
        for (int i = 0; i < PB; ++i)
          __builtin_amdgcn_raw_ptr_buffer_load_lds(rsrc_b, (lds_ptr_t)(sb + i * 256), 16, b_base[i], so, 0, 0);
      }
    } else if constexpr (MODE == MODE_DGRAD) {
      int kpk = p.K / BKT;
      int rs = ks / kpk, k0 = (ks - rs * kpk) * BKT;
      int r = rs / p.S, s = rs - r * p.S;
      int dy = r * p.dil, dx = s * p.dil;
      if (p.stride == 1) {
        int tapoff = k0 - (dy * p.OW + dx) * ldy;
#pragma unroll
        for (int i = 0; i < PA; ++i) {
          int oh = a_y[i] - dy, ow = a_x[i] - dx;
          bool ok = a_ok[i] && (unsigned)oh < (unsigned)p.OH && (unsigned)ow < (unsigned)p.OW;
          __builtin_amdgcn_raw_ptr_buffer_load_lds(rsrc_a, (lds_ptr_t)(sa + i * 256), 16,
                                                   ok ? (unsigned)(a_base[i] + tapoff) * 4u : OOB, 0, 0, 0);
        }
      } else {
#pragma unroll
        for (int i = 0; i < PA; ++i) {
          int ny = a_y[i] - dy, nx = a_x[i] - dx;
          bool ok = a_ok[i] && ny >= 0 && nx >= 0 && (ny % p.stride == 0) && (nx % p.stride == 0);
          int oh = ny / p.stride, ow = nx / p.stride;
          ok = ok && oh < p.OH && ow < p.OW;
          int off = ((a_n[i] * p.OH + oh) * p.OW + ow) * ldy + k0 + a_q4[i];
          __builtin_amdgcn_raw_ptr_buffer_load_lds(rsrc_a, (lds_ptr_t)(sa + i * 256), 16,
                                                   ok ? (unsigned)off * 4u : OOB, 0, 0, 0);
        }
      }
      unsigned so = (unsigned)(rs * p.C * p.K + k0) * 4u;
#pragma unroll
      for (int i = 0; i < PB; ++i)
        __builtin_amdgcn_raw_ptr_buffer_load_lds(rsrc_b, (lds_ptr_t)(sb + i * 256), 16, b_base[i], so, 0, 0);
    } else {
      int r = rs_fixed / p.S, s = rs_fixed - r * p.S;
#pragma unroll
      for (int i = 0; i < PA; ++i) {
        const int pos = (wid * PA + i) * 64 + lane;
        int kr = pos / (BM / 4), m4 = pos % (BM / 4);
        int pix = pix0 + ks * BKT + kr;
        bool ok = pix < pix1;
        int off = 0;
        if (p.R == 1 && p.S == 1 && p.stride == 1) {
          off = pix * p.C;
        } else {
          int ow = pix % p.OW, t = pix / p.OW;
          int oh = t % p.OH, n = t / p.OH;
          int ih = oh * p.stride - p.pt + r * p.dil, iw = ow * p.stride - p.pl + s * p.dil;
          ok = ok && (unsigned)ih < (unsigned)p.H && (unsigned)iw < (unsigned)p.W;
          off = ((n * p.H + ih) * p.W + iw) * p.C;
        }
        ok = ok && (m0 + m4 * 4) < p.M;
        __builtin_amdgcn_raw_ptr_buffer_load_lds(rsrc_a, (lds_ptr_t)(sa + i * 256), 16,
                                                 ok ? (unsigned)(off + m0 + m4 * 4) * 4u : OOB, 0, 0, 0);
      }
#pragma unroll
      for (int i = 0; i < PB; ++i) {
        const int pos = (wid * PB + i) * 64 + lane;
        int pix = pix0 + ks * BKT + pos / (BN / 4);
        __builtin_amdgcn_raw_ptr_buffer_load_lds(
            rsrc_b, (lds_ptr_t)(sb + i * 256), 16,
            (pix < pix1 && b_base[i] != OOB) ? b_base[i] + (unsigned)(pix * ldy) * 4u : OOB, 0, 0, 0);
      }
    }
  };

  floatx16 acc[TM][TN];
#pragma unroll
  for (int i = 0; i < TM; ++i)
#pragma unroll
    for (int j = 0; j < TN; ++j)
#pragma unroll
      for (int e = 0; e < 16; ++e) acc[i][j][e] = 0.f;

  int fa_off[TM], fb_off[TN];
#pragma unroll
  for (int i = 0; i < TM; ++i) {
    const int row = wr * (BM / WR) + i * 32 + lo;
    fa_off[i] = A_KC ? row * BKT + (((hi * (QPR / 2)) ^ ((row >> RSH) & (QPR - 1))) * 4) : hi * (BKT / 2) * BM + row;
  }
#pragma unroll
  for (int j = 0; j < TN; ++j) {
    const int col = wc * (BN / 2) + j * 32 + lo;
    fb_off[j] = B_KC ? col * BKT + (((hi * (QPR / 2)) ^ ((col >> RSH) & (QPR - 1))) * 4) : hi * (BKT / 2) * BN + col;
  }

  const int nk = ksteps - ks_begin;
  constexpr int NDMA = ((LAB & 64) ? 0 : PA) + ((LAB & 128) ? 0 : PB);
#pragma unroll
  for (int s = 0; s < NSTAGE - 1; ++s)
    if (s < nk) issue_tile(ks_begin + s, s);
  if (NSTAGE == 3 && nk > 1) asm volatile("s_waitcnt vmcnt(%0)" ::"n"(NDMA) : "memory");
  else asm volatile("s_waitcnt vmcnt(0)" ::: "memory");
  __builtin_amdgcn_s_barrier();
  asm volatile("" ::: "memory");

  bool do_cs = false;
  float csum = 0.f;
  static_assert(!CS || (MODE == MODE_WGRAD && !BATCH), "column sums ride on the plain wgrad launch only");
  if constexpr (CS) do_cs = p.cs_part != nullptr && tile_m == 0 && rs_fixed == 0;
  int cur = 0, nxt = NSTAGE - 1;
  for (int it = 0; it < nk; ++it) {
    const bool more = it + NSTAGE - 1 < nk;
    if constexpr (!(LAB & 1))
      if (more) issue_tile(ks_begin + it + NSTAGE - 1, nxt);
    const float* a = smem + cur * STAGE;
    const float* b = a + A_FL;
    if constexpr (CS)
      if (do_cs && tid < BN) {
#pragma unroll
        for (int k = 0; k < BKT; ++k) csum += b[k * BN + tid];
      }
    float fa[TM][BKT / 2], fb[TN][BKT / 2];
    auto read_group = [&](auto GI) {
      constexpr int g = decltype(GI)::value;
#pragma unroll
      for (int i = 0; i < TM; ++i) {
        if constexpr (A_KC) {
          floatx4 v = *reinterpret_cast<const floatx4*>(a + (fa_off[i] ^ (g * 4)));
          fa[i][4 * g + 0] = v.x; fa[i][4 * g + 1] = v.y; fa[i][4 * g + 2] = v.z; fa[i][4 * g + 3] = v.w;
        } else {
#pragma unroll
          for (int t = 0; t < 4; ++t) fa[i][4 * g + t] = a[fa_off[i] + (4 * g + t) * BM];
        }
      }
#pragma unroll
      for (int j = 0; j < TN; ++j) {
        if constexpr (B_KC) {
          floatx4 v = *reinterpret_cast<const floatx4*>(b + (fb_off[j] ^ (g * 4)));
          fb[j][4 * g + 0] = v.x; fb[j][4 * g + 1] = v.y; fb[j][4 * g + 2] = v.z; fb[j][4 * g + 3] = v.w;
        } else {
#pragma unroll
          for (int t = 0; t < 4; ++t) fb[j][4 * g + t] = b[fb_off[j] + (4 * g + t) * BN];
        }
      }
    };
    auto mma = [&](int t) {
#pragma unroll
      for (int i = 0; i < TM; ++i)
#pragma unroll
        for (int j = 0; j < TN; ++j)
          acc[i][j] = __builtin_amdgcn_mfma_f32_32x32x2f32(fa[i][t], fb[j][t], acc[i][j], 0, 0, 0);
    };
    if constexpr (LAB & 8) {
#pragma unroll
      for (int t = 0; t < BKT / 2; ++t) {
#pragma unroll
        for (int i = 0; i < TM; ++i) fa[i][t] = (float)(lane + it + t) * 1e-3f;
#pragma unroll
        for (int j = 0; j < TN; ++j) fb[j][t] = (float)(lane - it - t) * 1e-3f;
      }
#pragma unroll
      for (int t = 0; t < BKT / 2; ++t) mma(t);
    } else {
      read_group(std::integral_constant<int, 0>{});
      auto group = [&](auto GI) {
        constexpr int g = decltype(GI)::value;
        __builtin_amdgcn_sched_barrier(0);
        mma(4 * g);
        __builtin_amdgcn_sched_barrier(0);
        if constexpr (g + 1 < G) read_group(std::integral_constant<int, g + 1>{});
        __builtin_amdgcn_sched_barrier(0);
        mma(4 * g + 1); mma(4 * g + 2); mma(4 * g + 3);
      };
      group(std::integral_constant<int, 0>{});
      group(std::integral_constant<int, 1>{});
      if constexpr (G > 2) {
        group(std::integral_constant<int, 2>{});
        group(std::integral_constant<int, 3>{});
      }
    }
    __builtin_amdgcn_sched_barrier(0);
    if constexpr (!(LAB & 4)) {
      if (NSTAGE == 3 && more) asm volatile("s_waitcnt vmcnt(%0)" ::"n"(NDMA) : "memory");
      else asm volatile("s_waitcnt vmcnt(0)" ::: "memory");
      __builtin_amdgcn_s_barrier();
    }
    asm volatile("" ::: "memory");
    cur = cur + 1 == NSTAGE ? 0 : cur + 1;
    nxt = nxt + 1 == NSTAGE ? 0 : nxt + 1;
  }
  if constexpr (CS)
    if (do_cs && tid < BN && n0 + tid < p.NG) p.cs_part[(int64_t)blockIdx.z * p.NG + n0 + tid] = csum;
  conv_epilogue<BM, BN, MODE, NW>(p, acc, smem, m0, n0);
}

template <int BM, int BN, int BKT, int NSTAGE>
constexpr int glds_waves() {
  constexpr int lds = NSTAGE * (BM + BN) * BKT * 4;
  constexpr int nw = BM > 128 ? 8 : 4;
  constexpr int blocks = 163840 / lds;
  constexpr int w = blocks * nw / 4;
  return w > 4 ? 4 : (w < 1 ? 1 : w);
}
template <int BM, int BN, int MODE, int BKT, int NSTAGE>
__global__ void __launch_bounds__(BM > 128 ? 512 : 256, (glds_waves<BM, BN, BKT, NSTAGE>()))
k_conv_glds(ConvArgs p) {
  conv_glds_body<BM, BN, MODE, BKT, NSTAGE, false>(p);
}
template <int BM, int BN, int MODE, int BKT, int NSTAGE>
__global__ void __launch_bounds__(BM > 128 ? 512 : 256, (glds_waves<BM, BN, BKT, NSTAGE>()))
k_conv_glds_pw(ConvArgs p) {
  conv_glds_body<BM, BN, MODE, BKT, NSTAGE, false, true>(p);
}
template <int BM, int BN, int BKT, int NSTAGE>
__global__ void __launch_bounds__(BM > 128 ? 512 : 256, (glds_waves<BM, BN, BKT, NSTAGE>()))
k_conv_glds_cs(ConvArgs p) {
  conv_glds_body<BM, BN, MODE_WGRAD, BKT, NSTAGE, false, false, true>(p);
}
template <int BM, int BN, int BKT, int NSTAGE>
__global__ void __launch_bounds__(BM > 128 ? 512 : 256, (glds_waves<BM, BN, BKT, NSTAGE>()))
k_conv_glds_pw_cs(ConvArgs p) {
  conv_glds_body<BM, BN, MODE_WGRAD, BKT, NSTAGE, false, true, true>(p);
}
template <int BM, int BN, int MODE, int BKT, int NSTAGE>
__global__ void __launch_bounds__(BM > 128 ? 512 : 256, (glds_waves<BM, BN, BKT, NSTAGE>()))
k_wino_glds(ConvArgs p) {
  conv_glds_body<BM, BN, MODE, BKT, NSTAGE, true, true>(p);
}

template <int BM, int BN, int MODE, int BKT>
__global__ void __launch_bounds__(BM > 128 ? 512 : 256, (BM > 128 ? 2 : BM * BN >= 128 * 128 ? (BKT > 16 ? 2 : 3) : 4))
k_conv_mfma(ConvArgs p) {
  conv_mfma_body<BM, BN, MODE, BKT, false>(p);
}
template <int BM, int BN, int MODE>
__global__ void __launch_bounds__(BM > 128 ? 512 : 256, (BM > 128 ? 2 : BM * BN >= 128 * 128 ? 3 : 4))
k_conv_mfma_pw(ConvArgs p) {
  conv_mfma_body<BM, BN, MODE, 16, false, true>(p);
}
template <int BM, int BN, int BKT>
__global__ void __launch_bounds__(BM > 128 ? 512 : 256, (BM > 128 ? 2 : BM * BN >= 128 * 128 ? (BKT > 16 ? 2 : 3) : 4))
k_conv_mfma_cs(ConvArgs p) {
  conv_mfma_body<BM, BN, MODE_WGRAD, BKT, false, false, true>(p);
}
template <int BM, int BN>
__global__ void __launch_bounds__(BM > 128 ? 512 : 256, (BM > 128 ? 2 : BM * BN >= 128 * 128 ? 3 : 4))
k_conv_mfma_pw_cs(ConvArgs p) {
  conv_mfma_body<BM, BN, MODE_WGRAD, 16, false, true, true>(p);
}
struct GroupArgs { mtlssl_conv_group_entry e[MTLSSL_CONV_GROUP_MAX]; };
template <int BM, int BN>
__global__ void __launch_bounds__(BM > 128 ? 512 : 256, (BM > 128 ? 2 : BM * BN >= 128 * 128 ? 3 : 4))
k_conv_mfma_pw_grp(ConvArgs p, GroupArgs g) {
  static_assert(MTLSSL_CONV_GROUP_MAX == 4, "the select chain below covers four problems");
  const int gy = blockIdx.y;
  const mtlssl_conv_group_entry e = gy == 0 ? g.e[0] : gy == 1 ? g.e[1] : gy == 2 ? g.e[2] : g.e[3];
  p.b = e.w; p.out = e.y; p.bias = e.bias;
  p.NG = e.K; p.K = e.K; p.ldy = e.ldy; p.epi = e.epilogue;
  p.b_bytes = (unsigned)(p.C * e.K) * 4u;
  p.tiles_n = (e.K + BN - 1) / BN;
  if ((int)blockIdx.x >= p.tiles_m * p.tiles_n) return;
  conv_mfma_body<BM, BN, MODE_FWD, 16, false, true>(p);
}
template <int BM, int BN>
__global__ void __launch_bounds__(BM > 128 ? 512 : 256, (BM > 128 ? 2 : BM * BN >= 128 * 128 ? 3 : 4))
k_conv_mfma_pw_seg(ConvArgs p, SegArgs g) {
  conv_mfma_body<BM, BN, MODE_DGRAD, 16, false, true, false, true>(p, g);
// ... 51 lines not shown
```

### mtl_ssl_amd/frcnn.py

```python
import os

import torch

from . import nn, ops

f32, i32 = torch.float32, torch.int32


def _init_from_hyperparams(hp):
    ini = hp.initializer
    which = ini.which_oneof(["truncated_normal_initializer", "variance_scaling_initializer"])
    if which == "truncated_normal_initializer":
        return ("truncated_normal", float(ini.truncated_normal_initializer.stddev))
    if which == "variance_scaling_initializer":
        v = ini.variance_scaling_initializer
        return ("variance_scaling", float(v.factor), str(v.mode), bool(v.uniform))
    return ("variance_scaling", 1.0, "FAN_AVG", True)


def _l2_from_hyperparams(hp):
    reg = hp.regularizer
    if reg.has("l2_regularizer"):
        return float(reg.l2_regularizer.weight)
    return 0.0
# ... 555 lines not shown
        clo = pd["closeness_predictions"] if mtl.closeness else None
        net = ops.refine_concat(cls, win, clo, B, N2, self.N_EXPAND, bool(mtl.global_closeness))
        hidden, sctx = net, None
        if self.refine_stack is not None:
            hidden, sctx = self.refine_stack.forward(net, self._is_training, self.seed, self.step)
        refined = self.refine_fc.forward(hidden)
        pd["_refine_hidden"], pd["_refine_ctx"] = hidden, sctx
        if mtl.refine_residue:
            ops.axpby(cls, refined, 1.0, 1.0)
        pd["mtl_refined_class_predictions_with_background"] = refined
        pd["_refine_in"] = net
        return pd

    def postprocess(self, pd):
        c = self.cfg
        B, H, W, _ = pd["image_shape"]
        if c.first_stage_only:
            boxes, scores, num = ops.rpn_proposals(
                pd["rpn_box_encodings"], pd["rpn_objectness_predictions_with_background"], pd["anchors"],
                H, W, c.first_stage_nms_score_threshold, c.first_stage_nms_iou_threshold,
                int(c.first_stage_max_proposals))
            if self._is_training:
                gt = self._format_groundtruth_data(H, W)
                _, norm, num = self._second_stage_proposals(boxes, num, gt, H, W)
                return {"detection_boxes": norm, "num_detections": num}
            return {"detection_boxes": ops.scale_channels(boxes, self._hw_scales(H, W)[1]), "detection_scores": scores,
                    "num_detections": num}
        key = "mtl_refined_class_predictions_with_background"
        cls = pd[key] if (self._mtl.refine and key in pd) else pd["class_predictions_with_background"]
        N, K = self.max_num_proposals, self.num_classes
        enc = pd["refined_box_encodings"].reshape(1, B * N * K, 4).contiguous()
        tiled = pd["proposal_boxes"].view(B, N, 1, 4).expand(B, N, K, 4).reshape(B * N * K, 4).contiguous()
        boxes = ops.boxes_decode(enc, tiled).view(B, N, K, 4)
        pp = c.second_stage_post_processing
        conv = ops.score_convert(cls.reshape(B * N, K + 1).contiguous(), pp.score_converter).view(B, N, K + 1)
        nms = pp.batch_non_max_suppression
        ob, os_, oc, on = ops.batch_multiclass_nms(
            boxes, conv, nms.score_threshold, nms.iou_threshold, int(nms.max_detections_per_class),
            int(nms.max_total_detections), clip_window=[0.0, 0.0, float(H), float(W)],
            change_coordinate_frame=True, num_valid=pd["num_proposals"], col0=1, num_classes=K)
        return {"detection_boxes": ob, "detection_scores": os_, "detection_classes": oc, "num_detections": on}

    def loss(self, pd, loss_scale=1.0, part="all"):
        second = not self._first_stage_only
        new = {}
        if part == "late":
            losses, d, cls_s = pd["_losses_early"], pd["_d"], pd["_cls_s"]
        else:
            losses, d, cls_s = {}, {}, None
            self._loss_rpn(pd, self.step, losses, new, True)
            if second:
                cls_s = self._loss_box_classifier(pd, losses, new, True)
                self._loss_window_class(pd, losses, new, True)
            self._loss_edgemask(pd, losses, new, True)
        if part == "early":
            pd["_losses_early"], pd["_cls_s"] = losses, cls_s
        elif second:
            self._loss_refined_classifier(pd, cls_s, losses, new, True)
        g = float(loss_scale)
        if g != 1.0:
            for t in new.values():
                ops.axpby(t, t, g, 0.0)
        d.update(new)
        pd["_d"] = d
        return losses

    def eval_loss(self, pd, image_index=0):
        if self._is_training:
            raise ValueError("eval_loss is the loss of an inference model; a training model calls loss()")
        if self._hard_miner is not None:
            raise ValueError("eval_config.calc_loss with a hard_example_miner is not supported")
        second = not self._first_stage_only
        losses = {}
        self._loss_rpn(pd, int(image_index), losses, None, False)
        if second:
            cls_s = self._loss_box_classifier(pd, losses, None, False)
            if self._mtl.window and self._window["classes"].numel() == 0:
                losses["window_class_loss"] = torch.zeros((1,), dtype=f32, device=self.ps.device)
            else:
                self._loss_window_class(pd, losses, None, False)
        self._loss_edgemask(pd, losses, None, False)
        if second:
            self._loss_refined_classifier(pd, cls_s, losses, None, False)
        return losses

    def _unmatched_class_targets(self):
        if "um" not in self._consts:
            dev = self.ps.device
            self._consts["um"] = torch.zeros((1,), dtype=f32, device=dev)
            self._consts["um2"] = torch.tensor([1.0] + [0.0] * self.num_classes, dtype=f32, device=dev)
        return self._consts["um"], self._consts["um2"]

    def _loss_rpn(self, pd, draw, losses, d, want_grad):
        c = self.cfg
        B, H, W, _ = pd["image_shape"]
        gt = self._format_groundtruth_data(H, W)
        anchors = pd["anchors"]
        n = anchors.shape[0]
        um, _ = self._unmatched_class_targets()
        tg = ops.assign_targets(anchors, gt["boxes_abs"], gt["num"], None, um, 0.7, 0.3, True)
        cls_t = tg["cls_targets"].view(B, n)
        sampled = ops.balanced_sample(tg["cls_weights"], cls_t, int(c.first_stage_minibatch_size),
                                      c.first_stage_positive_balance_fraction, self.seed,
                                      (2 * draw * 65536) & 0xFFFFFFFF, 2)
        loc_s, obj_s = ops.rpn_loss_scales(sampled, tg["reg_weights"],
                                           c.first_stage_localization_loss_weight / B,
                                           c.first_stage_objectness_loss_weight / B)
        rl, d_enc = ops.smooth_l1(pd["rpn_box_encodings"], tg["reg_targets"], loc_s, 3.0, want_grad=want_grad)
        losses["first_stage_localization_loss"] = ops.reduce_sum(rl)
        rl, d_obj = ops.softmax_ce(pd["rpn_objectness_predictions_with_background"], ops.onehot2(cls_t), obj_s,
                                   want_grad=want_grad)
        losses["first_stage_objectness_loss"] = ops.reduce_sum(rl)
        if want_grad:
            d["rpn_box_encodings"], d["rpn_objectness"] = d_enc, d_obj
        pd["_rpn_targets"] = dict(tg, sampled=sampled)

    def _loss_box_classifier(self, pd, losses, d, want_grad):
        c, mtl = self.cfg, self._mtl
        B, H, W, _ = pd["image_shape"]
        gt = self._format_groundtruth_data(H, W)
        N2, K1 = self.max_num_proposals, self.num_classes + 1
        _, um2 = self._unmatched_class_targets()
        dt = ops.assign_targets(pd["proposal_boxes"], gt["boxes_abs"], gt["num"], gt["classes_bg"], um2,
                                0.5, 0.5, False, gt_extra=gt["closeness"] if mtl.closeness else None)
        cls_s, loc_s2, clo_s = ops.detector_loss_scales(
            dt["cls_weights"], dt["reg_weights"], pd["num_proposals"],
            dt.get("extra_targets") if mtl.closeness else None,
            c.second_stage_classification_loss_weight, c.second_stage_localization_loss_weight,
            mtl.closeness_loss_weight)
        cls_targets = dt["cls_targets"].view(B * N2, K1)
        rl_loc, d_box = ops.box_select_smooth_l1(pd["refined_box_encodings"], cls_targets,
                                                 dt["reg_targets"].view(B * N2, 4), loc_s2.view(-1), 1.0,
                                                 want_grad=want_grad)
        rl_cls, d_cls = ops.softmax_ce(pd["class_predictions_with_background"], cls_targets, cls_s.view(-1),
                                       want_grad=want_grad)
        if self._hard_miner is not None:
            hm = self._hard_miner
            lm, cm, sel, nsel = ops.hard_example_mining(rl_loc.view(B, N2), rl_cls.view(B, N2), pd["proposal_boxes"],
                                                        pd["num_proposals"], d_box, d_cls, hm["num_hard_examples"],
                                                        hm["iou_threshold"], hm["loss_type"])
            rl_loc, rl_cls = lm, cm
            pd["_mined"] = (sel, nsel)
        losses["second_stage_localization_loss"] = ops.reduce_sum(rl_loc)
        losses["second_stage_classification_loss"] = ops.reduce_sum(rl_cls)
        if want_grad:
            d["refined_box_encodings"], d["class_predictions"] = d_box, d_cls
        pd["_det_targets"] = dt
        if mtl.closeness:
            rl, d_clo = ops.softmax_ce(pd["closeness_predictions"], dt["extra_targets"].view(B * N2, K1),
                                       clo_s.view(-1), col0=1, want_grad=want_grad)
            losses["closeness_classification_loss"] = ops.reduce_sum(rl)
            if want_grad:
                d["closeness_predictions"] = d_clo
        return cls_s

    def _loss_refined_classifier(self, pd, cls_s, losses, d, want_grad):
        c, mtl = self.cfg, self._mtl
        if not mtl.refine:
            return
        dt = pd["_det_targets"]
        rs = cls_s if c.second_stage_classification_loss_weight == mtl.refined_classification_loss_weight \
            else ops.detector_loss_scales(dt["cls_weights"], dt["reg_weights"], pd["num_proposals"], None,
                                          mtl.refined_classification_loss_weight, 0.0, 0.0)[0]
        cls_targets = dt["cls_targets"].view(-1, self.num_classes + 1)
        rl, d_ref = ops.softmax_ce(pd["mtl_refined_class_predictions_with_background"], cls_targets, rs.view(-1),
                                   want_grad=want_grad)
        losses["refined_classification_loss"] = ops.reduce_sum(rl)
        if want_grad:
            d["refined_class_predictions"] = d_ref

    def _loss_window_class(self, pd, losses, d, want_grad):
        mtl = self._mtl
        if not mtl.window:
            return
        wc = self._window["classes"].view(-1, self.num_classes + 1)
        ws = torch.full((wc.shape[0],), mtl.window_class_loss_weight / wc.shape[0], dtype=f32, device=self.ps.device)
        rl, d_win = ops.softmax_ce(pd["window_class_predictions"], wc, ws, want_grad=want_grad)
        losses["window_class_loss"] = ops.reduce_sum(rl)
        if want_grad:
            d["window_class_predictions"] = d_win

    def _loss_edgemask(self, pd, losses, d, want_grad):
        mtl = self._mtl
        if not mtl.edgemask:
            return
        B = pd["image_shape"][0]
        em = self._edgemask
        mh, mw = em.shape[2], em.shape[3]
        tgt, sc = ops.edgemask_targets(em, mtl.edgemask_loss_weight / (B * mh * mw))
        pr = ops.resize_bilinear_fwd(pd["edgemask_predictions"], mh, mw)
        rl, d_pr = ops.softmax_ce(pr, tgt, sc.view(-1), want_grad=want_grad)
        losses["edgemask_loss"] = ops.reduce_sum(rl)
        if want_grad:
            d["edgemask_resized"] = d_pr

    def _backward_refiner(self, pd, d):
        mtl = self._mtl
        d_ref = d["refined_class_predictions"]
        self.refine_fc.wgrad(pd["_refine_hidden"], d_ref)
        if self.refine_stack is not None:
            g_h = self.refine_fc.dgrad(pd["_refine_hidden"].shape, d_ref)
            self.refine_stack.backward(pd["_refine_ctx"], g_h, need_input_grad=False)
        if mtl.refine_residue and not mtl.stop_gradient_for_prediction_org:
            ops.axpby(d_ref, d["class_predictions"], 1.0, 1.0)

    def backward(self, pd):
        mtl = self._mtl
        d = pd["_d"]
        F = pd["rpn_features_to_crop"]
        B = F.shape[0]
        if self._first_stage_only:
            dF = torch.zeros_like(F)
            return self._backward_first_stage(pd, d, F, dF, B)
        dF = torch.empty_like(F)
        if mtl.refine:
            self._backward_refiner(pd, d)
        d_cls = d["class_predictions"]
        c = self.cfg
        feat = pd["_feat"]
        g_feat = self.box_predictor.backward(pd["_bp"], d_cls, d["refined_box_encodings"].view(feat.shape[0], -1),
                                             feat.shape, **self.tower.out_mask(feat))
        stop = bool(mtl.stop_gradient_for_aux_tasks)
        shared = self._shared_classifier
        gw_shared = None
        if shared:
            if mtl.closeness:
                gcl = self.closeness_predictor.backward(pd["_cp"], d["closeness_predictions"], None, feat.shape,
                                                        need_feat_grad=not stop, **self.tower.out_mask(feat))
                if not stop:
                    ops.axpby(gcl, g_feat, 1.0, 1.0)
            if mtl.window and not stop:
                wfeat = pd["_wfeat"]
                g = self.window_predictor.backward(pd["_wp"], d["window_class_predictions"], None, wfeat.shape,
                                                   **self.window_tower.out_mask(wfeat))
                hook, self.ps.grad_ready_hook = self.ps.grad_ready_hook, None
                gw_shared = self.tower.backward(g, wfeat, pd["_wctx"], need_input_grad=True, masked=True)
                self.ps.grad_ready_hook = hook
        crop_args = (int(c.initial_crop_size), int(c.maxpool_kernel_size), int(c.maxpool_stride))

        def aux_backward(collect=None):
            if shared:
                if mtl.window and stop:
                    wfeat = pd["_wfeat"]
                    self.window_predictor.backward(pd["_wp"], d["window_class_predictions"], None, wfeat.shape,
                                                   need_feat_grad=False)
                return
            todo = []
            if mtl.closeness:
                cfeat = pd["_cfeat"]
                g = self.closeness_predictor.backward(pd["_cp"], d["closeness_predictions"], None, cfeat.shape,
                                                      **self.closeness_tower.out_mask(cfeat))
                gc = self.closeness_tower.backward(g, cfeat, pd["_cctx"], need_input_grad=not stop, masked=True)
                if not stop:
                    todo.append((gc, pd["_argmax"], pd["proposal_boxes_normalized"].view(-1, 4), pd["_box_ind"]))
            if mtl.window:
                wfeat = pd["_wfeat"]
                g = self.window_predictor.backward(pd["_wp"], d["window_class_predictions"], None, wfeat.shape,
                                                   **self.window_tower.out_mask(wfeat))
                gw = self.window_tower.backward(g, wfeat, pd["_wctx"], need_input_grad=not stop, masked=True)
                if not stop:
                    todo.append((gw, pd["_wargmax"], pd["_wboxes"], pd["_wbox_ind"]))
            if collect is not None:
                collect.extend(todo)
            else:
                for gx, am, bx, bi in todo:
                    ops.roi_crop_pool_bwd(gx, am, F.shape, bx, bi, *crop_args, dfeat=dF)

        cur = torch.cuda.current_stream()
        aux = self._aux_stream() if (mtl.closeness or mtl.window) else None
        pending = []
        if aux is not None and not shared:
            aux.wait_stream(cur)
            with torch.cuda.stream(aux):
                aux_backward(collect=pending)
        g_crops = self.tower.backward(g_feat, feat, pd["_tower_ctx"], need_input_grad=True, masked=True,
                                      wgrad=nn.INLINE_WGRAD if shared else self._wgrad_exec())
        ops.roi_crop_pool_bwd(g_crops, pd["_argmax"], F.shape, pd["proposal_boxes_normalized"].view(-1, 4),
                              pd["_box_ind"], *crop_args, dfeat=dF, accumulate=False)
        if gw_shared is not None:
            ops.roi_crop_pool_bwd(gw_shared, pd["_wargmax"], F.shape, pd["_wboxes"], pd["_wbox_ind"], *crop_args, dfeat=dF)
        if pending:
            ops.wait_on(aux, "backward: aux towers released early", cur)
            for gx, am, bx, bi in pending:
                gx.record_stream(cur)
                ops.roi_crop_pool_bwd(gx, am, F.shape, bx, bi, *crop_args, dfeat=dF)
        if aux is None:
            aux_backward()
        elif shared and stop:
            aux.wait_stream(cur)
            with torch.cuda.stream(aux):
                aux_backward()
        return self._backward_first_stage(pd, d, F, dF, B, aux if stop else None)

    def _backward_first_stage(self, pd, d, F, dF, B, side=None):
        mtl = self._mtl
        if mtl.edgemask:
            em_pred = pd["edgemask_predictions"]
            g = ops.resize_bilinear_bwd(d["edgemask_resized"], em_pred.shape)
            g = ops.tanh_bwd(em_pred, g)
            self.edgemask_conv.wgrad(F, g)
            self.edgemask_conv.dgrad(F.shape, g, out=dF, accum=True)
        rpn_feat = pd["rpn_box_predictor_features"]
        n_all = pd["_n_all"]
        g_enc = ops.scatter_rows(d["rpn_box_encodings"], pd["_keep"], n_all).view(B, F.shape[1], F.shape[2], -1)
        g_obj = ops.scatter_rows(d["rpn_objectness"], pd["_keep"], n_all).view(B, F.shape[1], F.shape[2], -1)
        self.rpn_box.wgrad(rpn_feat, g_enc)
        self.rpn_cls.wgrad(rpn_feat, g_obj)
        g_rf = self.rpn_box.dgrad(rpn_feat.shape, g_enc)
        relu = self.rpn_conv.activation == "relu"
        self.rpn_cls.dgrad(rpn_feat.shape, g_obj, out=g_rf, accum=True, mask_ref=rpn_feat if relu else None)
        wg = self._wgrad_exec()
        wg.run(self.rpn_conv, F, g_rf)
        gpF = self.rpn_conv.dgrad(F.shape, g_rf, out=dF, accum=True, mask_ref=F,
                                  mask6=self._feature_extractor.out_act == "relu6")
        pd["_gpF"] = gpF
        ops.mark("heads_backward")
        self._feature_extractor.backward_proposal_features(gpF, pd["_trunk_ctx"], wgrad=wg)
        if side is not None:
            ops.wait_on(side, "backward end: aux stream")
        if wg.stream is not None:
            ops.wait_on(wg.stream, "backward end: filter-gradient stream")
```

### mtl_ssl_amd/inception_resnet_v2.py

```python
import torch

from . import nn, ops

EPS = 1e-3
XAVIER = ("variance_scaling", 1.0, "FAN_AVG", True)


def _conv(ps, scope, cin, cout, k, stride=1, padding="SAME", rate=1, trainable=True, wd=0.0):
    return nn.ConvBN(ps, scope, cin, cout, k, stride, rate, padding, trainable, wd, EPS, init=XAVIER,
                     bn_trainable=trainable, bn_scale=False)


class Pool(nn.Layer):

    def __init__(self, kind, k, stride, padding):
        super().__init__()
        self.kind, self.k, self.stride, self.padding = kind, k, stride, padding

    def forward(self, x, out=None):
        if self.kind == "max":
            y, self.pads = ops.maxpool_fwd(x, self.k, self.stride, self.padding, out=out)
        else:
            assert out is None
            y, self.pads = ops.avgpool_fwd(x, self.k, self.stride, self.padding)
# ... 127 lines not shown
            segs = []
            for ci, ch in enumerate(self.chains):
                a = acts[ci]
                gp = g_cat[..., self.offs[ci]:self.offs[ci] + self.couts[ci]]
                for li in range(len(ch) - 1, 0, -1):
                    l, xin = ch[li], a[li]
                    if isinstance(l, Pool):
                        gp = l.input_grad(xin, a[li + 1], gp)
                    else:
                        wgrad.run(l, xin, gp)
                        gp = l.dgrad(xin.shape, gp, mask_ref=None if isinstance(ch[li - 1], Pool) else xin)
                wgrad.run(ch[0], x, gp)
                segs.append((ch[0].desc(x.shape), gp, ch[0].w_eff))
            if not need_input_grad:
                return None
            return ops.conv2d_dgrad_segmented(segs, residual, mask_ref, nn.dgrad_epilogue(residual, mask_ref=mask_ref))
        order = sorted(range(len(self.chains)), key=lambda i: not isinstance(self.chains[i][0], Pool))
        assert not isinstance(self.chains[order[-1]][0], Pool)
        dx = None
        for n, ci in enumerate(order):
            ch, a = self.chains[ci], acts[ci]
            gp = g_cat[..., self.offs[ci]:self.offs[ci] + self.couts[ci]]
            last = n == len(order) - 1
            for li in range(len(ch) - 1, -1, -1):
                l, xin = ch[li], a[li]
                if not isinstance(l, Pool):
                    wgrad.run(l, xin, gp)
                if li > 0:
                    if isinstance(l, Pool):
                        gp = l.input_grad(xin, a[li + 1], gp)
                    else:
                        prev_pool = isinstance(ch[li - 1], Pool)
                        gp = l.dgrad(xin.shape, gp, mask_ref=None if prev_pool else xin)
                    continue
                if not need_input_grad:
                    break
                if isinstance(l, Pool):
                    g_in = l.input_grad(xin, a[1], gp)
                    if dx is None:
                        dx = g_in
                        if residual is not None:
                            ops.axpby(residual, dx, 1.0, 1.0)
                    else:
                        ops.axpby(g_in, dx, 1.0, 1.0)
                elif dx is None:
                    dx = l.dgrad(x.shape, gp, residual=residual, mask_ref=mask_ref if last else None)
                else:
                    l.dgrad(x.shape, gp, out=dx, accum=True, mask_ref=mask_ref if last else None)
        return dx


class ResBlock:

    def __init__(self, ps, scope, cin, chains, scale, relu, trainable, wd):
        self.br = Branches(chains)
        mixed_c = sum(ch[-1].w.shape[-1] for ch in chains)
        self.up = ResidualUp(ps, scope + "/Conv2d_1x1", mixed_c, cin, scale, trainable, wd)
        self.relu = relu

    def layers(self):
        return self.br.layers() + [self.up]

    def forward(self, x, save):
        mixed, acts = self.br.forward(x, save)
        return self.up.forward(mixed, x, self.relu), ((mixed, acts) if save else None)

    def backward(self, gp, ctx, mask_input=True, wgrad=nn.INLINE_WGRAD):
        mixed, acts = ctx
        x = acts[0][0]
        wgrad.run(self.up, mixed, gp)
        g_mixed = self.up.dgrad(mixed.shape, gp, mask_ref=mixed)
        return self.br.backward(g_mixed, acts, residual=gp, mask_ref=x if mask_input else None, wgrad=wgrad)


class MixedBlock:

    def __init__(self, chains):
        self.br = Branches(chains)

    def layers(self):
        return self.br.layers()

    def forward(self, x, save):
        return self.br.forward(x, save)

    def backward(self, g_cat, acts, mask_input=True, need_input_grad=True, wgrad=nn.INLINE_WGRAD):
        return self.br.backward(g_cat, acts, None, acts[0][0] if mask_input else None, need_input_grad, wgrad=wgrad)


def block35(ps, s, t, wd):
    ch = [[_conv(ps, s + "/Branch_0/Conv2d_1x1", 320, 32, 1, trainable=t, wd=wd)],
          [_conv(ps, s + "/Branch_1/Conv2d_0a_1x1", 320, 32, 1, trainable=t, wd=wd),
           _conv(ps, s + "/Branch_1/Conv2d_0b_3x3", 32, 32, 3, trainable=t, wd=wd)],
          [_conv(ps, s + "/Branch_2/Conv2d_0a_1x1", 320, 32, 1, trainable=t, wd=wd),
           _conv(ps, s + "/Branch_2/Conv2d_0b_3x3", 32, 48, 3, trainable=t, wd=wd),
           _conv(ps, s + "/Branch_2/Conv2d_0c_3x3", 48, 64, 3, trainable=t, wd=wd)]]
    return ResBlock(ps, s, 320, ch, 0.17, True, t, wd)


def block17(ps, s, t, wd, rate):
    ch = [[_conv(ps, s + "/Branch_0/Conv2d_1x1", 1088, 192, 1, trainable=t, wd=wd)],
          [_conv(ps, s + "/Branch_1/Conv2d_0a_1x1", 1088, 128, 1, trainable=t, wd=wd),
           _conv(ps, s + "/Branch_1/Conv2d_0b_1x7", 128, 160, (1, 7), rate=rate, trainable=t, wd=wd),
           _conv(ps, s + "/Branch_1/Conv2d_0c_7x1", 160, 192, (7, 1), rate=rate, trainable=t, wd=wd)]]
    return ResBlock(ps, s, 1088, ch, 0.10, True, t, wd)


def block8(ps, s, t, wd, scale=0.20, relu=True):
    ch = [[_conv(ps, s + "/Branch_0/Conv2d_1x1", 2080, 192, 1, trainable=t, wd=wd)],
          [_conv(ps, s + "/Branch_1/Conv2d_0a_1x1", 2080, 192, 1, trainable=t, wd=wd),
           _conv(ps, s + "/Branch_1/Conv2d_0b_1x3", 192, 224, (1, 3), trainable=t, wd=wd),
           _conv(ps, s + "/Branch_1/Conv2d_0c_3x1", 224, 256, (3, 1), trainable=t, wd=wd)]]
    return ResBlock(ps, s, 2080, ch, scale, relu, t, wd)


class InceptionTower(nn.Tower):
    out_act = "relu"
    supports_wgrad_stream = True

    def __init__(self, ps, scope, trainable, wd):
        p, t = scope + "/InceptionResnetV2/", trainable
        m = p + "Mixed_7a/"
        self.mixed_7a = MixedBlock([
            [_conv(ps, m + "Branch_0/Conv2d_0a_1x1", 1088, 256, 1, trainable=t, wd=wd),
             _conv(ps, m + "Branch_0/Conv2d_1a_3x3", 256, 384, 3, 2, "VALID", trainable=t, wd=wd)],
            [_conv(ps, m + "Branch_1/Conv2d_0a_1x1", 1088, 256, 1, trainable=t, wd=wd),
             _conv(ps, m + "Branch_1/Conv2d_1a_3x3", 256, 288, 3, 2, "VALID", trainable=t, wd=wd)],
            [_conv(ps, m + "Branch_2/Conv2d_0a_1x1", 1088, 256, 1, trainable=t, wd=wd),
             _conv(ps, m + "Branch_2/Conv2d_0b_3x3", 256, 288, 3, trainable=t, wd=wd),
             _conv(ps, m + "Branch_2/Conv2d_1a_3x3", 288, 320, 3, 2, "VALID", trainable=t, wd=wd)],
            [Pool("max", 3, 2, "VALID")]])
        self.blocks = [block8(ps, p + "Repeat/block8_%d" % (i + 1), t, wd) for i in range(9)]
        self.blocks.append(block8(ps, p + "Block8", t, wd, scale=1.0, relu=False))
        self.conv_7b = _conv(ps, p + "Conv2d_7b_1x1", 2080, 1536, 1, trainable=t, wd=wd)
        self.cout, self.trainable = 1536, trainable

    def layers(self):
        return self.mixed_7a.layers() + [l for b in self.blocks for l in b.layers()] + [self.conv_7b]

    @staticmethod
    def out_hw(p):
        q = (p - 3) // 2 + 1
        return (q, q)

    def forward(self, crops, save):
        x, c7 = self.mixed_7a.forward(crops, save)
        ctxs = []
        for b in self.blocks:
            x, c = b.forward(x, save)
            ctxs.append(c)
        out = self.conv_7b.forward(x)
        return out, ((c7, ctxs, x) if save else None)

    def backward(self, g_out, out, ctx, need_input_grad, masked=False, wgrad=nn.INLINE_WGRAD):
        c7, ctxs, pre7b = ctx
        gp = g_out if masked else ops.relu_bwd(out, g_out)
        wgrad.run(self.conv_7b, pre7b, gp)
        gp = self.conv_7b.dgrad(pre7b.shape, gp)
        for i in range(len(self.blocks) - 1, -1, -1):
            gp = self.blocks[i].backward(gp, ctxs[i], mask_input=True, wgrad=wgrad)
        return self.mixed_7a.backward(gp, c7, mask_input=False, need_input_grad=need_input_grad, wgrad=wgrad)


class FasterRCNNInceptionResnetV2FeatureExtractor(nn.FeatureExtractor):
    out_act = "relu"
    supports_wgrad_stream = True
    min_image_size = None

    def __init__(self, ps, is_training, first_stage_features_stride=16, weight_decay=0.0,
                 first_stage_scope="FirstStageFeatureExtractor"):
        super().__init__(ps, is_training, first_stage_features_stride, weight_decay)
        t, wd = is_training, weight_decay
        atrous = first_stage_features_stride == 8
        p = first_stage_scope + "/InceptionResnetV2/"
        self.stem = [_conv(ps, p + "Conv2d_1a_3x3", 3, 32, 3, 2, trainable=t, wd=wd),
                     _conv(ps, p + "Conv2d_2a_3x3", 32, 32, 3, trainable=t, wd=wd),
                     _conv(ps, p + "Conv2d_2b_3x3", 32, 64, 3, trainable=t, wd=wd),
                     Pool("max", 3, 2, "SAME"),
                     _conv(ps, p + "Conv2d_3b_1x1", 64, 80, 1, trainable=t, wd=wd),
                     _conv(ps, p + "Conv2d_4a_3x3", 80, 192, 3, trainable=t, wd=wd),
                     Pool("max", 3, 2, "SAME")]
        m = p + "Mixed_5b/"
        self.mixed_5b = MixedBlock([
            [_conv(ps, m + "Branch_0/Conv2d_1x1", 192, 96, 1, trainable=t, wd=wd)],
            [_conv(ps, m + "Branch_1/Conv2d_0a_1x1", 192, 48, 1, trainable=t, wd=wd),
             _conv(ps, m + "Branch_1/Conv2d_0b_5x5", 48, 64, 5, trainable=t, wd=wd)],
            [_conv(ps, m + "Branch_2/Conv2d_0a_1x1", 192, 64, 1, trainable=t, wd=wd),
             _conv(ps, m + "Branch_2/Conv2d_0b_3x3", 64, 96, 3, trainable=t, wd=wd),
             _conv(ps, m + "Branch_2/Conv2d_0c_3x3", 96, 96, 3, trainable=t, wd=wd)],
            [Pool("avg", 3, 1, "SAME"), _conv(ps, m + "Branch_3/Conv2d_0b_1x1", 192, 64, 1, trainable=t, wd=wd)]])
        self.blocks35 = [block35(ps, p + "Repeat/block35_%d" % (i + 1), t, wd) for i in range(10)]
        m = p + "Mixed_6a/"
        s6 = 1 if atrous else 2
        self.mixed_6a = MixedBlock([
            [_conv(ps, m + "Branch_0/Conv2d_1a_3x3", 320, 384, 3, s6, trainable=t, wd=wd)],
            [_conv(ps, m + "Branch_1/Conv2d_0a_1x1", 320, 256, 1, trainable=t, wd=wd),
             _conv(ps, m + "Branch_1/Conv2d_0b_3x3", 256, 256, 3, trainable=t, wd=wd),
             _conv(ps, m + "Branch_1/Conv2d_1a_3x3", 256, 384, 3, s6, trainable=t, wd=wd)],
            [Pool("max", 3, s6, "SAME")]])
        rate = 2 if atrous else 1
        self.blocks17 = [block17(ps, p + "Repeat_1/block17_%d" % (i + 1), t, wd, rate) for i in range(20)]
        self.cout = 1088

    def layers(self):
        return (list(self.stem) + self.mixed_5b.layers() + [l for b in self.blocks35 for l in b.layers()]
                + self.mixed_6a.layers() + [l for b in self.blocks17 for l in b.layers()])

    def preprocess(self, resized_inputs):
        return self.to_unit_range(resized_inputs)

    def extract_proposal_features(self, x, save=True):
        self.check_inputs(x)
        acts = [x]
        for l in self.stem:
            acts.append(l.forward(acts[-1]))
        x, c5 = self.mixed_5b.forward(acts[-1], save)
        c35 = []
        for b in self.blocks35:
            x, c = b.forward(x, save)
            c35.append(c)
        x, c6 = self.mixed_6a.forward(x, save)
        c17 = []
        for b in self.blocks17:
            x, c = b.forward(x, save)
            c17.append(c)
        return x, ((acts, c5, c35, c6, c17) if save else None)

    def backward_proposal_features(self, gp, ctx, wgrad=nn.INLINE_WGRAD):
        if not self.is_training:
            return
        acts, c5, c35, c6, c17 = ctx
        for i in range(len(self.blocks17) - 1, -1, -1):
            gp = self.blocks17[i].backward(gp, c17[i], wgrad=wgrad)
        gp = self.mixed_6a.backward(gp, c6, wgrad=wgrad)
        for i in range(len(self.blocks35) - 1, -1, -1):
            gp = self.blocks35[i].backward(gp, c35[i], wgrad=wgrad)
        g = self.mixed_5b.backward(gp, c5, mask_input=False, wgrad=wgrad)
        for i in range(len(self.stem) - 1, -1, -1):
            l, xin, y = self.stem[i], acts[i], acts[i + 1]
            if isinstance(l, Pool):
                g = l.input_grad(xin, y, g)
                g = ops.relu_bwd(xin, g, out=g)
                continue
            wgrad.run(l, xin, g)
            if i == 0:
                break
            prev_pool = isinstance(self.stem[i - 1], Pool)
            g = l.dgrad(xin.shape, g, mask_ref=None if prev_pool else xin)

    def box_classifier_tower(self, scope, trainable):
        return InceptionTower(self.ps, scope, trainable and self.is_training, self.weight_decay)
```

### mtl_ssl_amd/lib.py

```python
import ctypes
import os
import re

HERE = os.path.dirname(os.path.abspath(__file__))
HEADER = os.path.join(HERE, "..", "include", "mtlssl_hip.h")
LIB_PATH = os.environ.get("MTLSSL_LIB_PATH") or os.path.join(HERE, "libmtlssl_hip.so")


class ConvDesc(ctypes.Structure):
    _fields_ = [(n, ctypes.c_int32) for n in
                ("N", "H", "W", "C", "K", "R", "S", "OH", "OW", "stride", "dilation",
                 "pad_t", "pad_l", "ldy")]


_SCALARS = {
    "int": ctypes.c_int, "int32_t": ctypes.c_int32, "int64_t": ctypes.c_int64,
    "uint32_t": ctypes.c_uint32, "float": ctypes.c_float, "double": ctypes.c_double,
    "mtlssl_stream_t": ctypes.c_void_p, "mtlssl_comm_t": ctypes.c_void_p,
}


def _ctype(decl):
    decl = decl.strip()
    if "*" in decl:
        if "mtlssl_conv_desc" in decl:
            return ctypes.POINTER(ConvDesc)
        return ctypes.c_void_p
    base = decl.replace("const", "").split()
    return _SCALARS[base[0]]


def parse_header(path=HEADER):
    text = open(path).read()
    text = re.sub(r"/\*.*?\*/", "", text, flags=re.S)
    protos = {}
    for m in re.finditer(r"\b(int|int64_t|const char\*)\s+(mtlssl_\w+)\s*\(([^)]*)\)\s*;", text):
        ret, name, args = m.group(1), m.group(2), m.group(3)
        restype = {"int": ctypes.c_int, "int64_t": ctypes.c_int64,
                   "const char*": ctypes.c_char_p}[ret]
        argtypes = []
        if args.strip() not in ("", "void"):
            for a in args.split(","):
                a = a.strip()
                a = re.sub(r"\s*\w+$", "", a) if not a.endswith("*") else a
                argtypes.append(_ctype(a))
        protos[name] = (restype, argtypes)
    return protos


class MtlsslError(RuntimeError):
    pass


class _Lib:
    def __init__(self):
        if not os.path.exists(LIB_PATH):
            raise MtlsslError(
                "%s not found: build it with `python -m mtl_ssl_amd.build` "
                "(there is no CPU fallback for the product path)" % LIB_PATH)
        import torch
        self.cdll = ctypes.CDLL(LIB_PATH)
        self.protos = parse_header()
        want = int(re.search(r"#define\s+MTLSSL_ABI_VERSION\s+(\d+)", open(HEADER).read()).group(1))
        self.cdll.mtlssl_abi_version.restype = ctypes.c_int
        have = self.cdll.mtlssl_abi_version()
        if have != want:
            raise MtlsslError("%s has ABI version %d, include/mtlssl_hip.h declares %d: rebuild it with "
                              "`python -m mtl_ssl_amd.build`" % (LIB_PATH, have, want))
        for name, (restype, argtypes) in self.protos.items():
            fn = getattr(self.cdll, name)
            fn.restype = restype
            fn.argtypes = argtypes
            if restype is ctypes.c_int and name not in ("mtlssl_abi_version", "mtlssl_conv2d_tile_config", "mtlssl_conv2d_num_dispatches",
                                                        "mtlssl_conv2d_set_winograd", "mtlssl_conv2d_set_fp32_engine", "mtlssl_conv2d_filter_xf_variant",
                                                        "mtlssl_conv2d_set_pointwise"):
                setattr(self, name[len("mtlssl_"):], self._checked(fn, name))
            else:
                setattr(self, name[len("mtlssl_"):], fn)

    def _checked(self, fn, name):
        last_error = self.cdll.mtlssl_last_error

        def call(*args):
            rc = fn(*args)
            if rc != 0:
                raise MtlsslError("%s failed (%d): %s" % (name, rc, last_error().decode()))
        return call


_lib = None


def lib():
    global _lib
    if _lib is None:
        _lib = _Lib()
    return _lib


def ptr(t):
    return None if t is None else t.data_ptr()
```

### mtl_ssl_amd/mobilenet.py

```python
from . import nn, ops

_CONV_DEFS = [("conv", 2, 32), ("sep", 1, 64), ("sep", 2, 128), ("sep", 1, 128), ("sep", 2, 256),
              ("sep", 1, 256), ("sep", 2, 512), ("sep", 1, 512), ("sep", 1, 512), ("sep", 1, 512),
              ("sep", 1, 512), ("sep", 1, 512)]
_INIT = ("truncated_normal", 0.09)
EPS = 1e-3
_DW_GAMMA = 3.5


class _PlainDepthwise(nn.DepthwiseBN):

    def __init__(self, ps, scope, c, stride, trainable):
        super().__init__(ps, scope, c, 3, stride, 1, trainable, 0.0, EPS, None, _INIT, batch_norm=False)

    def prepare(self):
        self.scale = None
        self.shift = None
        self.w_eff = self.ps.value(self.w.name).view(self.w_eff_shape)

    def forward(self, x):
        return ops.depthwise_fwd(self.desc(x.shape), x, self.w_eff, None, 0)


class MobilenetTower(nn.Tower):
    out_act = "relu6"

    def __init__(self, ps, scope, cin, trainable, weight_decay):
        p = scope + "/MobilenetV1/"
        self.dw12 = _PlainDepthwise(ps, p + "Conv2d_12_pointwise", cin, 2, trainable)
        self.pw12 = _sep_pointwise(ps, p + "Conv2d_12_pointwise", cin, 1024, trainable)
        self.dw13 = _PlainDepthwise(ps, p + "Conv2d_13_pointwise", 1024, 1, trainable)
        self.pw13 = _sep_pointwise(ps, p + "Conv2d_13_pointwise", 1024, 1024, trainable)
        self.cout = 1024
        self.trainable = trainable

    def layers(self):
        return [self.dw12, self.pw12, self.dw13, self.pw13]

    @staticmethod
    def out_hw(p):
        return (-(-p // 2), -(-p // 2))

    def forward(self, crops, save):
        d12 = self.dw12.forward(crops)
        a12 = self.pw12.forward(d12)
        d13 = self.dw13.forward(a12)
        a13 = self.pw13.forward(d13)
        return a13, ((crops, d12, a12, d13) if save else None)

    def backward(self, g_out, out, ctx, need_input_grad, masked=False, wgrad=nn.INLINE_WGRAD):
        crops, d12, a12, d13 = ctx
        gp = g_out if masked else ops.relu6_bwd(out, g_out)
        self.pw13.bn_grad(out, gp)
        self.pw13.wgrad(d13, gp)
        g = self.pw13.dgrad(d13.shape, gp)
        self.dw13.wgrad(a12, g)
        gp = self.dw13.dgrad(a12.shape, g, mask_ref=a12, mask6=True)
        self.pw12.bn_grad(a12, gp)
        self.pw12.wgrad(d12, gp)
        g = self.pw12.dgrad(d12.shape, gp)
        self.dw12.wgrad(crops, g)
        return self.dw12.dgrad(crops.shape, g) if need_input_grad else None


def _sep_pointwise(ps, scope, cin, cout, trainable):
    return nn.ConvBN(ps, scope, cin, cout, 1, 1, 1, "SAME", trainable, 0.0, EPS, act="relu6", init=_INIT,
                     bn_trainable=trainable, weights_name="pointwise_weights")


class FasterRCNNMobilenetV1FeatureExtractor(nn.FeatureExtractor):
    out_act = "relu6"

    def __init__(self, ps, is_training, first_stage_features_stride=16, weight_decay=0.0,
                 first_stage_scope="FirstStageFeatureExtractor"):
        super().__init__(ps, is_training, first_stage_features_stride, weight_decay)
        if first_stage_features_stride != 16:
            raise ValueError("MobileNet extractor: only first_stage_features_stride 16 is built")
        p = first_stage_scope + "/MobilenetV1/"
        self.stages = []
        cin = 3
        for i, (kind, stride, depth) in enumerate(_CONV_DEFS):
            if kind == "conv":
                self.stages.append(nn.ConvBN(ps, p + "Conv2d_%d" % i, cin, depth, 3, stride, 1, "SAME",
                                             is_training, weight_decay, EPS, act="relu6", init=_INIT,
                                             bn_trainable=is_training))
            else:
                self.stages.append(nn.DepthwiseBN(ps, p + "Conv2d_%d_depthwise" % i, cin, 3, stride, 1,
                                                  is_training, 0.0, EPS, "relu6", _INIT, is_training,
                                                  gamma_init=_DW_GAMMA))
                self.stages.append(nn.ConvBN(ps, p + "Conv2d_%d_pointwise" % i, cin, depth, 1, 1, 1, "SAME",
                                             is_training, weight_decay, EPS, act="relu6", init=_INIT,
                                             bn_trainable=is_training))
            cin = depth
        self.cout = cin

    def layers(self):
        return list(self.stages)

    def preprocess(self, resized_inputs):
        return self.to_unit_range(resized_inputs)

    def extract_proposal_features(self, x, save=True):
        self.check_inputs(x)
        acts = [x]
        for l in self.stages:
            x = l.forward(x)
            acts.append(x)
        return x, (acts if save else None)

    def backward_proposal_features(self, gp, acts, wgrad=nn.INLINE_WGRAD):
        if not self.is_training:
            return
        for i in range(len(self.stages) - 1, -1, -1):
            l, xin = self.stages[i], acts[i]
            l.bn_grad(acts[i + 1], gp)
            l.wgrad(xin, gp)
            if i == 0:
                break
            gp = l.dgrad(xin.shape, gp, mask_ref=xin, mask6=True)

    def box_classifier_tower(self, scope, trainable):
        return MobilenetTower(self.ps, scope, self.cout, trainable and self.is_training, self.weight_decay)
```

### mtl_ssl_amd/nn.py

```python
import torch

from . import ops

f32 = torch.float32


def _refresh_bn(layer):
    if layer.bn_trainable:
        ps = layer.ps
        if layer.gamma is not None:
            torch.mul(ps.value(layer.gamma.name), layer.inv_std, out=layer.scale)
        torch.addcmul(ps.value(layer.beta.name), ps.value(layer.mean.name), layer.scale, value=-1.0,
                      out=layer.shift)


class WgradStream:

    def __init__(self, stream):
        self.stream = stream

    def run(self, layer, x, g):
        if not layer.trainable:
            return
        ev = torch.cuda.Event()
        ev.record(torch.cuda.current_stream())
        self.stream.wait_event(ev)
        for t in (x, g):
            t.record_stream(self.stream)
        with torch.cuda.stream(self.stream):
            layer.wgrad(x, g)


class _InlineWgrad:
    stream = None

    @staticmethod
    def run(layer, x, g):
        layer.wgrad(x, g)


INLINE_WGRAD = _InlineWgrad()


_ACT_EPILOGUE = {None: 0, "relu": ops.EPI_RELU, "relu6": ops.EPI_RELU6, "tanh": ops.EPI_TANH}


def act_epilogue(act):
    return _ACT_EPILOGUE[act]


def dgrad_epilogue(residual=None, accum=False, mask_ref=None, mask6=False):
    return ((ops.EPI_RESIDUAL if residual is not None else 0) | (ops.EPI_ACCUM if accum else 0)
            | ((ops.EPI_MASK6 if mask6 else ops.EPI_MASK) if mask_ref is not None else 0))


class Layer:
    trainable = False
    bn_trainable = False
    gamma = beta = None
    w_eff = None
    ldy = 0

    def __init__(self):
        self._desc = {}

    def prepare(self):
        """Allocate what depends on the finalized ParamStore (shadow filters, normaliser constants)."""

    def refold(self):
        """Recompute the normaliser constants after an optimizer step (the CPU path of FasterRCNNMetaArch.refold)."""

    def wgrad(self, x, g):
        """Accumulate the gradients of the layer's variables and report them final (ParamStore.grad_ready)."""

    def grad_vars(self):
        bn = (self.gamma, self.beta) if self.bn_trainable else ()
        return tuple(v for v in ((self.w,) if self.trainable else ()) + bn if v is not None)

    def geometry(self):
        raise NotImplementedError

    def desc(self, shape):
        d = self._desc.get(tuple(shape))
        if d is None:
            d = self._desc[tuple(shape)] = ops.conv_desc(shape, *self.geometry(), ldy=self.ldy)
        return d


class _FrozenBN(Layer):

    def _add_batch_norm(self, c, gamma_init, bn_scale=True):
        ps, bn, t = self.ps, self.scope + "/BatchNorm/", self.bn_trainable
        if bn_scale:
            self.gamma = ps.add(bn + "gamma", (c,), ("uniform", 0.8 * gamma_init, 1.2 * gamma_init), t)
        self.beta = ps.add(bn + "beta", (c,), ("uniform", -0.1, 0.1), t)
        self.mean = ps.add(bn + "moving_mean", (c,), ("uniform", -0.1, 0.1), False)
        self.var = ps.add(bn + "moving_variance", (c,), ("uniform", 0.8, 1.2), False)

    def prepare(self):
        ps = self.ps
        b = ps.value(self.beta.name)
        m, v = ps.value(self.mean.name), ps.value(self.var.name)
        self.inv_std = torch.rsqrt(v + self.eps)
        self.scale = ((ps.value(self.gamma.name) * self.inv_std) if self.gamma is not None
                      else self.inv_std.clone()).contiguous()
        self.shift = (b - m * self.scale).contiguous()
        if self.w.trainable:
            self.w_eff = ps.register_fold(self.w, self.scale).view(self.w_eff_shape)
        else:
            self.w_eff = torch.empty(self.w_eff_shape, dtype=f32, device=ps.device)
            ops.scale_channels(ps.value(self.w.name).view(self.w_eff_shape), self.scale, self.w_eff)

    def refold(self):
        _refresh_bn(self)

    def bn_grad(self, y, gp):
        if self.bn_trainable and self.gamma is not None:
            ps = self.ps
            ops.bn_param_grads(y, gp, ps.value(self.gamma.name), ps.value(self.beta.name),
                               ps.grad(self.gamma.name), ps.grad(self.beta.name), beta=1.0)
            ps.grad_ready(self.gamma, self.beta)


class ConvBN(_FrozenBN):

    def __init__(self, ps, scope, cin, cout, k, stride=1, dilation=1, padding="SAME",
                 trainable=True, weight_decay=0.0, eps=1e-5, gamma_init=1.0, relu=True, act=None,
                 init=("variance_scaling", 2.0, "FAN_IN", False), bn_trainable=False,
                 weights_name="weights", bn_scale=True):
        super().__init__()
        self.ps, self.scope = ps, scope
        self.bn_trainable = bn_trainable
        self.k, self.stride, self.dilation, self.padding, self.eps = k, stride, dilation, padding, eps
        self.trainable = trainable
        self.act = act if act is not None else ("relu" if relu else None)
        self.relu = self.act is not None
        kh, kw = k if isinstance(k, tuple) else (k, k)
        self.w = ps.add(scope + "/" + weights_name, (kh, kw, cin, cout), init, trainable, weight_decay)
        self.w_eff_shape = self.w.shape
        self._add_batch_norm(cout, gamma_init, bn_scale)
        self._kept = {}

    def geometry(self):
        return self.w.shape, self.stride, self.dilation, self.padding

    def forward(self, x, residual=None, relu=None, keep=False, out=None):
        act = self.act if relu is None else ("relu" if relu else None)
        epi = ops.EPI_BIAS | act_epilogue(act) | (ops.EPI_RESIDUAL if residual is not None else 0)
        return ops.conv2d_fwd(self.desc(x.shape), x, self.w_eff, self.shift, residual, epi, out=out,
                              xf_cache=self.ps.filter_cache,
                              keep_input_xf=self._keep_slot() if (keep and self.trainable and self.k == 3) else None)

    def _keep_slot(self):
        if len(self._kept) > 8:
            self._kept.clear()
        return self._kept

    def wgrad(self, x, g):
        if self.trainable:
            db = self.ps.grad(self.beta.name) if (self.bn_trainable and self.gamma is None) else None
            ops.conv2d_wgrad(self.desc(x.shape), x, g, self.ps.grad(self.w.name), out_scale=self.scale,
                             dbias=db, beta=1.0, input_xf=self._kept.pop(x.data_ptr(), None))
            self.ps.grad_ready(self.w, self.beta if db is not None else None)

    def dgrad(self, x_shape, g, residual=None, mask_ref=None, out=None, accum=False, mask6=False):
        return ops.conv2d_dgrad(self.desc(x_shape), g, self.w_eff, residual, mask_ref,
                                dgrad_epilogue(residual, accum, mask_ref, mask6), out=out, xf_cache=self.ps.filter_cache)


class DepthwiseBN(_FrozenBN):

    def __init__(self, ps, scope, c, k=3, stride=1, dilation=1, trainable=True, weight_decay=0.0, eps=1e-3,
                 act="relu6", init=("truncated_normal", 0.09), bn_trainable=False, gamma_init=1.0, batch_norm=True):
        super().__init__()
        self.ps, self.scope, self.c = ps, scope, c
        self.bn_trainable = bn_trainable
        self.k, self.stride, self.dilation, self.eps, self.act = k, stride, dilation, eps, act
        self.trainable = trainable
        self.w = ps.add(scope + "/depthwise_weights", (k, k, c, 1), init, trainable, weight_decay)
        self.w_eff_shape = (k, k, c)
        if batch_norm:
            self._add_batch_norm(c, gamma_init)

    def geometry(self):
        return (self.k, self.k, self.c, self.c), self.stride, self.dilation, "SAME"

    def forward(self, x):
        return ops.depthwise_fwd(self.desc(x.shape), x, self.w_eff, self.shift, ops.EPI_BIAS | act_epilogue(self.act))

    def wgrad(self, x, g):
        if self.trainable:
            ops.depthwise_wgrad(self.desc(x.shape), x, g, self.ps.grad(self.w.name), out_scale=self.scale,
                                beta=1.0)
            self.ps.grad_ready(self.w)

    def dgrad(self, x_shape, g, mask_ref=None, mask6=False):
        return ops.depthwise_dgrad(self.desc(x_shape), g, self.w_eff, mask_ref,
                                   dgrad_epilogue(None, False, mask_ref, mask6))


class Conv(Layer):

    def __init__(self, ps, scope, cin, cout, k, init, trainable=True, weight_decay=0.0,
                 activation=None, fc=False, rate=1):
        super().__init__()
        self.ps, self.scope, self.k, self.trainable, self.activation = ps, scope, k, trainable, activation
        self.rate = rate
        shape = (cin, cout) if fc else (k, k, cin, cout)
        self.fc = fc
        self.w = ps.add(scope + "/weights", shape, init, trainable, weight_decay)
        self.b = ps.add(scope + "/biases", (cout,), ("zeros",), trainable)
        self.cin, self.cout = cin, cout

    def _w4(self):
        w = self.ps.value(self.w.name)
        return w.view(1, 1, self.cin, self.cout) if self.fc else w

    def geometry(self):
        return (self.k, self.k, self.cin, self.cout), 1, self.rate, "SAME"

    def forward(self, x):
        x4 = x.view(x.shape[0], 1, 1, self.cin) if self.fc else x
        epi = ops.EPI_BIAS | act_epilogue(self.activation)
        y = ops.conv2d_fwd(self.desc(x4.shape), x4, self._w4(), self.ps.value(self.b.name), None, epi,
                           xf_cache=self.ps.filter_cache)
        return y.view(x.shape[0], self.cout) if self.fc else y

    def wgrad(self, x, g):
        if not self.trainable:
            return
        x4 = x.view(x.shape[0], 1, 1, self.cin) if self.fc else x
        g4 = g.view(g.shape[0], 1, 1, self.cout) if self.fc else g
        gw = self.ps.grad(self.w.name)
        ops.conv2d_wgrad(self.desc(x4.shape), x4, g4, gw.view(self.k, self.k, self.cin, self.cout),
                         dbias=self.ps.grad(self.b.name), beta=1.0)
        self.ps.grad_ready(self.w, self.b)

    def dgrad(self, x_shape, g, residual=None, mask_ref=None, out=None, accum=False, mask6=False):
        x4s = (x_shape[0], 1, 1, self.cin) if self.fc else tuple(x_shape)
        g4 = g.view(g.shape[0], 1, 1, self.cout) if self.fc else g
        dx = ops.conv2d_dgrad(self.desc(x4s), g4, self._w4(), residual, mask_ref,
                              dgrad_epilogue(residual, accum, mask_ref, mask6), out=out, xf_cache=self.ps.filter_cache)
        return dx.view(x_shape) if self.fc else dx


DROPOUT_SEED_SALT = 0x6D2B79F5


def dropout_stream(step, slot):
    return (((int(step) & 0xFFFFFF) << 8) | (int(slot) & 0xFF)) & 0xFFFFFFFF


class FCStack:

    def __init__(self, ps, scopes, cin, widths, init, trainable, weight_decay, activation="relu", keep_prob=None,
                 slot0=0):
        if activation not in ("relu", None):
            raise ValueError("fully connected stacks support RELU or NONE activations, got %r" % (activation,))
        self.layers, self.activation = [], activation
        for scope, cout in zip(scopes, widths):
            self.layers.append(Conv(ps, scope, cin, cout, 1, init, trainable, weight_decay, activation=activation, fc=True))
            cin = cout
        self.cout = cin
        self.keep_prob = None if (keep_prob is None or keep_prob >= 1.0) else float(keep_prob)
        self.slot0 = slot0

    def forward(self, x, training, seed, step):
        ctx = []
        for i, l in enumerate(self.layers):
            a = l.forward(x)
            drop = training and self.keep_prob is not None
            dseed = (int(seed) ^ DROPOUT_SEED_SALT) & 0xFFFFFFFF
            y = ops.dropout(a, self.keep_prob, dseed, dropout_stream(step, self.slot0 + i)) if drop else a
            ctx.append((x, a, (dseed, dropout_stream(step, self.slot0 + i)) if drop else None))
            x = y
        return x, ctx

    def backward(self, ctx, g, need_input_grad=True):
        for i in range(len(self.layers) - 1, -1, -1):
            l = self.layers[i]
            x, a, drop = ctx[i]
            if drop is not None:
                g = ops.dropout(g, self.keep_prob, drop[0], drop[1])
            if self.activation == "relu":
                g = ops.relu_bwd(a, g)
            l.wgrad(x, g)
            if i == 0 and not need_input_grad:
                return None
            g = l.dgrad(x.shape, g)
        return g


class Bottleneck:

    def __init__(self, ps, scope, cin, depth, depth_bottleneck, stride, rate=1, trainable=True,
                 weight_decay=0.0, bn_trainable=False):
        s = scope + "/bottleneck_v1/"
        self.stride, self.cin, self.depth = stride, cin, depth
        self.shortcut = None
        if depth != cin:
            self.shortcut = ConvBN(ps, s + "shortcut", cin, depth, 1, stride, 1, "SAME", trainable,
                                   weight_decay, relu=False, bn_trainable=bn_trainable)
        self.conv1 = ConvBN(ps, s + "conv1", cin, depth_bottleneck, 1, 1, 1, "SAME", trainable, weight_decay,
                            bn_trainable=bn_trainable)
        self.conv2 = ConvBN(ps, s + "conv2", depth_bottleneck, depth_bottleneck, 3, stride, rate,
                            "RESNET_SAME", trainable, weight_decay, bn_trainable=bn_trainable)
        self.conv3 = ConvBN(ps, s + "conv3", depth_bottleneck, depth, 1, 1, 1, "SAME", trainable,
                            weight_decay, gamma_init=0.3, relu=True, bn_trainable=bn_trainable)
        self.trainable = trainable
        self.bn_trainable = bn_trainable

    def layers(self):
        return [l for l in (self.shortcut, self.conv1, self.conv2, self.conv3) if l is not None]

    def forward(self, x, save):
        if self.shortcut is not None:
            sc = self.shortcut.forward(x)
        elif self.stride > 1:
            sc, _ = ops.maxpool_fwd(x, 1, self.stride, "SAME")
        else:
            sc = x
        a1 = self.conv1.forward(x)
        a2 = self.conv2.forward(a1, keep=save)
        out = self.conv3.forward(a2, residual=sc)
        ctx = (x, a1, a2, sc if (self.shortcut is None and self.stride > 1) else None) if save else None
        if save and self.bn_trainable:
            ctx = ctx + (out, sc)
        return out, ctx

    def backward(self, gp, ctx, need_input_grad=True, mask_input=True, wgrad=INLINE_WGRAD):
        x, a1, a2, sc_sub = ctx[:4]
        if self.bn_trainable:
            out, sc = ctx[4], ctx[5]
            o3 = ops.axpby(sc, out.clone(), -1.0, 1.0)
            self.conv3.bn_grad(o3, gp)
            del o3
            if self.shortcut is not None:
                self.shortcut.bn_grad(sc, gp)
        wgrad.run(self.conv3, a2, gp)
        gp2 = self.conv3.dgrad(a2.shape, gp, mask_ref=a2)
        if self.bn_trainable:
            self.conv2.bn_grad(a2, gp2)
        wgrad.run(self.conv2, a1, gp2)
        gp1 = self.conv2.dgrad(a1.shape, gp2, mask_ref=a1)
        if self.bn_trainable:
            self.conv1.bn_grad(a1, gp1)
        wgrad.run(self.conv1, x, gp1)
        if self.shortcut is not None:
            wgrad.run(self.shortcut, x, gp)
        if not need_input_grad:
            return None
        if self.shortcut is not None:
            addend = self.shortcut.dgrad(x.shape, gp)
        elif self.stride > 1:
            addend = ops.maxpool_bwd(x, sc_sub, gp, 1, self.stride, (0, 0))
        else:
            addend = gp
        return self.conv1.dgrad(x.shape, gp1, residual=addend, mask_ref=x if mask_input else None)


class BlockStack:

    def __init__(self, ps, prefix, cin, blocks, output_stride=None, current_stride=1, weight_decay=0.0,
                 bn_trainable=False):
        self.units = []
        rate = 1
        for (scope, base_depth, num_units, stride, trainable) in blocks:
            for i in range(num_units):
                ustride = stride if i == num_units - 1 else 1
                name = "%s/%s/unit_%d" % (prefix, scope, i + 1)
                if output_stride is not None and current_stride == output_stride:
                    u = Bottleneck(ps, name, cin, base_depth * 4, base_depth, 1, rate, trainable, weight_decay, bn_trainable)
                    rate *= ustride
                else:
                    u = Bottleneck(ps, name, cin, base_depth * 4, base_depth, ustride, 1, trainable, weight_decay,
                                   bn_trainable)
                    current_stride *= ustride
                u.block = scope
                self.units.append(u)
                cin = base_depth * 4
        self.cout = cin

    def layers(self):
        return [l for u in self.units for l in u.layers()]


class Tower:
    supports_wgrad_stream = False

    @staticmethod
    def out_hw(p):
        return (p, p)

    @classmethod
    def out_mask(cls, feat):
        return dict(mask_ref=None if cls.out_act is None else feat, mask6=cls.out_act == "relu6")

    def backward(self, g_out, out, ctx, need_input_grad, masked=False, wgrad=INLINE_WGRAD):
        raise NotImplementedError


class FeatureExtractor:
    supports_wgrad_stream = False
    supports_rfcn = True
    min_image_size = 33
    _neg_one = None

    def __init__(self, ps, is_training, first_stage_features_stride, weight_decay):
        if first_stage_features_stride not in (8, 16):
            raise ValueError("`first_stage_features_stride` must be 8 or 16.")
        self.ps, self.is_training, self.weight_decay = ps, is_training, weight_decay

    def check_inputs(self, x):
        if x.dim() != 4:
            raise ValueError("`preprocessed_inputs` must be 4 dimensional, got a tensor of shape %s" % (tuple(x.shape),))
        m = self.min_image_size
        if m is not None and (x.shape[1] < m or x.shape[2] < m):
            raise ValueError("image size must at least be %d in both height and width." % m)

    def to_unit_range(self, resized_inputs):
        x = torch.empty_like(resized_inputs)
        ops.axpby(resized_inputs, x, 2.0 / 255.0, 0.0)
        if self._neg_one is None:
            self._neg_one = torch.full((3,), -1.0, dtype=torch.float32, device=x.device)
        return ops.bias_add_channels(x, self._neg_one)

    def backward_proposal_features(self, gp, ctx, wgrad=INLINE_WGRAD):
        raise NotImplementedError
```

### mtl_ssl_amd/ops.py

```python
import ctypes
import os

import numpy as np
import torch

from .lib import ConvDesc, lib, ptr

EPI_BIAS, EPI_RESIDUAL, EPI_RELU, EPI_TANH, EPI_RELU6, EPI_MASK, EPI_ACCUM, EPI_MASK6 = 1, 2, 4, 8, 16, 32, 64, 128
f32 = torch.float32
i32 = torch.int32


_raw_stream = getattr(torch._C, "_cuda_getCurrentRawStream", None)
_cur_device = getattr(torch._C, "_cuda_getDevice", None)


def _stream():
    if _raw_stream is not None and _cur_device is not None:
        return _raw_stream(_cur_device())
    return torch.cuda.current_stream().cuda_stream


def _chk(t, dtype=f32):
    assert t.is_cuda and t.is_contiguous() and t.dtype == dtype, (t.device, t.dtype, t.is_contiguous())
# ... 321 lines not shown
    return lib().conv2d_set_pointwise(int(on))


def set_fp32_engine(mode):
    return lib().conv2d_set_fp32_engine(int(mode))


def _autotune(d, mode, run):
    key = _plan_key(d, mode)
    if key in _tuned:
        return
    _tuned[key] = None
    L, ref = lib(), ctypes.byref(d)
    default = L.conv2d_tile_config(ref, mode)
    if default < 0:
        return
    known = _plans().get(",".join(str(v) for v in key))
    if known is not None:
        if known >= 0:
            L.conv2d_force_config(ref, mode, int(known))
        return
    if not AUTOTUNE:
        return
    times = {}
    for cfg in (PLAN_CODES if TUNE_ENGINES else PLAN_CODES[:ENGINE1_CFG0]):
        L.conv2d_force_config(ref, mode, cfg)
        if L.conv2d_tile_config(ref, mode) != cfg:
            continue
        run()
        s, e = torch.cuda.Event(enable_timing=True), torch.cuda.Event(enable_timing=True)
        s.record()
        for _ in range(TUNE_RUNS):
            run()
        e.record()
        e.synchronize()
        times[cfg] = s.elapsed_time(e)
    L.conv2d_force_config(ref, mode, -1)
    best = min(times, key=times.get)
    if not (best != default and times[best] < (1.0 - TUNE_MARGIN) * times.get(default, float("inf"))):
        best = default
    if best != default:
        L.conv2d_force_config(ref, mode, best)
    _tuned[key] = (default, best, times)


class FilterXfCache:

    def __init__(self):
        self.entries = {}

    def get(self, d, mode, w):
        variant = lib().conv2d_filter_xf_variant(ctypes.byref(d), mode)
        if variant < 0:
            return None, -1
        key = (w.data_ptr(), d.C, d.K, mode, variant)
        cur = torch.cuda.current_stream()
        e = self.entries.get(key)
        if e is None:
            nbytes = lib().conv2d_filter_xf_bytes(ctypes.byref(d), mode)
            e = {"U": torch.empty(int(nbytes) // 4, dtype=f32, device=w.device), "d": d, "mode": mode, "variant": variant,
                 "w": w, "event": torch.cuda.Event(), "waited": {cur.cuda_stream}}
            lib().conv2d_transform_filter(ctypes.byref(d), mode, variant, ptr(_chk(w)), ptr(e["U"]), cur.cuda_stream)
            e["event"].record(cur)
            self.entries[key] = e
        elif cur.cuda_stream not in e["waited"]:
            wait_on(e["event"], "filter_cache_refresh", cur)
            e["waited"].add(cur.cuda_stream)
        return e["U"], variant

    CHUNK_BYTES = 48 << 20

    def _tables(self):
        if getattr(self, "_tab_n", None) != (len(self.entries), self.CHUNK_BYTES):
            chunks, cur, cur_bytes = [], [], 0
            for e in self.entries.values():
                nb = e["U"].numel() * 4
                if cur and (cur[0]["variant"] != e["variant"] or (cur_bytes + nb > self.CHUNK_BYTES > 0)):
                    chunks.append(cur)
                    cur, cur_bytes = [], 0
                cur.append(e)
                cur_bytes += nb
            if cur:
                chunks.append(cur)
            self._tab = []
            for es in chunks:
                dev = es[0]["U"].device
                self._tab.append(dict(
                    variant=es[0]["variant"], entries=es,
                    n=len(es), max_ck=max(e["d"].C * e["d"].K for e in es),
                    w=torch.tensor([e["w"].data_ptr() for e in es], dtype=torch.int64, device=dev),
                    u=torch.tensor([e["U"].data_ptr() for e in es], dtype=torch.int64, device=dev),
                    ck=torch.tensor([e["d"].C * e["d"].K for e in es], dtype=torch.int64, device=dev),
                    flip=torch.tensor([int(e["mode"] == 1) for e in es], dtype=i32, device=dev)))
            self._tab_n = (len(self.entries), self.CHUNK_BYTES)
        return self._tab

    def refresh(self, stream=None):
        if not self.entries:
            return
        cur = torch.cuda.current_stream()
        run_on = stream if stream is not None else cur
        tabs = self._tables()
        if stream is not None:
            stream.wait_stream(cur)
        for t in tabs:
            lib().conv2d_transform_filters(t["variant"], t["n"], ptr(t["w"]), ptr(t["u"]), ptr(t["ck"]), ptr(t["flip"]),
                                           t["max_ck"], run_on.cuda_stream)
            ev = torch.cuda.Event()
            ev.record(run_on)
            for e in t["entries"]:
                e["event"], e["waited"] = ev, {run_on.cuda_stream}


def _shared_input_variant(d):
    if not (d.R == 3 and d.S == 3):
        return -1
    v = lib().conv2d_filter_xf_variant(ctypes.byref(d), 0)
    return v if (v >= 0 and v == lib().conv2d_filter_xf_variant(ctypes.byref(d), 2)) else -1


def _conv_ws(d, mode, device):
    nb = lib().conv2d_workspace_bytes(ctypes.byref(d), mode)
    return workspace(nb, "wgrad" if mode == 2 else "splitk", device) if nb else None


def conv2d_fwd(d, x, w, bias=None, residual=None, epilogue=0, out=None, xf_cache=None, keep_input_xf=None):
    if d.ldy:
        assert out is not None, "a strided forward writes into the caller's concatenated map"
        _chk_y(d, out)
    y = out if out is not None else torch.empty((d.N, d.OH, d.OW, d.K), dtype=f32, device=x.device)
    if PROFILER is None:
        def run():
            lib().conv2d_fwd(ctypes.byref(d), ptr(_chk(x)), ptr(_chk(w)), ptr(bias), ptr(residual), ptr(y), epilogue,
                             ptr(_conv_ws(d, 0, x.device)), _stream())
        _autotune(d, 0, run)
    t0 = PROFILER.begin(d, 0) if PROFILER is not None else None
    if ACCOUNT is not None:
        ACCOUNT.add(d, 0)
    ws = _conv_ws(d, 0, x.device)
    U, variant = xf_cache.get(d, 0, w) if (xf_cache is not None and d.R == 3 and d.S == 3) else (None, -1)
    V, vvar = None, -1
    if keep_input_xf is not None:
        vvar = _shared_input_variant(d)
        if vvar >= 0:
            V = torch.empty(int(lib().conv2d_input_xf_bytes(ctypes.byref(d), vvar)) // 4, dtype=f32, device=x.device)
            keep_input_xf[x.data_ptr()] = (V, vvar)
    lib().conv2d_fwd_keep(ctypes.byref(d), ptr(_chk(x)), ptr(_chk(w)), ptr(bias), ptr(residual),
                          ptr(y), epilogue, ptr(ws), ptr(U), variant, ptr(V), vvar, _stream())
    if t0 is not None:
        PROFILER.end(d, 0, t0)
    return y


def conv2d_dgrad(d, dy, w, residual=None, mask_ref=None, epilogue=0, out=None, xf_cache=None):
    dx = out if out is not None else torch.empty((d.N, d.H, d.W, d.C), dtype=f32, device=dy.device)
    if PROFILER is None:
        def run():
            tmp = workspace(4 * d.N * d.H * d.W * d.C, "tune_out", dy.device)
            lib().conv2d_dgrad(ctypes.byref(d), ptr(_chk_y(d, dy)), ptr(_chk(w)), ptr(residual), ptr(mask_ref), ptr(tmp),
                               epilogue & ~EPI_ACCUM, ptr(_conv_ws(d, 1, dy.device)), _stream())
        _autotune(d, 1, run)
    t0 = PROFILER.begin(d, 1) if PROFILER is not None else None
    if ACCOUNT is not None:
        ACCOUNT.add(d, 1)
    ws = _conv_ws(d, 1, dy.device)
    U, variant = xf_cache.get(d, 1, w) if (xf_cache is not None and d.R == 3 and d.S == 3) else (None, -1)
    lib().conv2d_dgrad_xf(ctypes.byref(d), ptr(_chk_y(d, dy)), ptr(_chk(w)), ptr(residual), ptr(mask_ref),
                          ptr(dx), epilogue, ptr(ws), ptr(U), variant, _stream())
    if t0 is not None:
        PROFILER.end(d, 1, t0)
    return dx


def conv2d_wgrad(d, x, dy, dw, out_scale=None, dbias=None, beta=0.0, input_xf=None, dbias_scale=None):
    if PROFILER is None:
        def run():
            tmp = workspace(4 * d.R * d.S * d.C * d.K, "tune_out", x.device)
            lib().conv2d_wgrad(ctypes.byref(d), ptr(_chk(x)), ptr(_chk_y(d, dy)), ptr(out_scale), ptr(tmp), None, 0.0,
                               ptr(_conv_ws(d, 2, x.device)), _stream())
        _autotune(d, 2, run)
    ws = _conv_ws(d, 2, x.device)
    t0 = PROFILER.begin(d, 2) if PROFILER is not None else None
    if ACCOUNT is not None:
        ACCOUNT.add(d, 2)
    V, vvar = input_xf if input_xf is not None else (None, -1)
    if V is not None:
        V.record_stream(torch.cuda.current_stream())
    lib().conv2d_wgrad_ex(ctypes.byref(d), ptr(_chk(x)), ptr(_chk_y(d, dy)), ptr(out_scale), ptr(dw),
                          ptr(dbias), ptr(dbias_scale), float(beta), ptr(ws), ptr(V), vvar, _stream())
    if t0 is not None:
        PROFILER.end(d, 2, t0)
    return dw


_ptr_tables = {}


def _ptr_table(tensors, device):
    key = tuple(t.data_ptr() if t is not None else 0 for t in tensors)
    tab = _ptr_tables.get(key)
    if tab is None:
        if len(_ptr_tables) > 4096:
            _ptr_tables.clear()
        tab = torch.tensor(key, dtype=torch.int64, device=device)
        _ptr_tables[key] = tab
    return tab


def conv2d_wgrad_grouped(d, xs, dys, dws, scales=None, beta=0.0):
    n = len(xs)
    dev = xs[0].device
    for t in list(xs) + list(dys) + list(dws):
        _chk(t)
    if ACCOUNT is not None:
        ACCOUNT.add(d, 2, n)
    nb = lib().conv2d_wgrad_grouped_workspace_bytes(ctypes.byref(d), n)
    ws = workspace(nb, "wgrad_grouped", dev)
    lib().conv2d_wgrad_grouped(ctypes.byref(d), n, ptr(_ptr_table(xs, dev)), ptr(_ptr_table(dys, dev)),
                               ptr(_ptr_table(scales, dev)) if scales is not None else None,
                               ptr(_ptr_table(dws, dev)), float(beta), ptr(ws), _stream())


GROUPED_FWD = os.environ.get("MTLSSL_GROUPED_FWD", "1") != "0"
GROUPED_FWD_MAX_ROWS = 20000


class _GroupEntry(ctypes.Structure):
    _fields_ = [("w", ctypes.c_void_p), ("y", ctypes.c_void_p), ("bias", ctypes.c_void_p), ("K", ctypes.c_int32),
                ("ldy", ctypes.c_int32), ("epilogue", ctypes.c_int32), ("reserved", ctypes.c_int32)]


def conv2d_fwd_grouped(x, problems):
    d0 = problems[0][0]
    outs = []
    for d, w, bias, epi, out in problems:
        assert desc_is_pointwise(d) and (d.N, d.H, d.W, d.C) == (d0.N, d0.H, d0.W, d0.C) and d.C % 16 == 0 \
            and d.K % 4 == 0 and d.K >= 16 and not (epi & EPI_RESIDUAL), (d.C, d.K, epi)
        if out is None:
            assert not d.ldy
            out = torch.empty((d.N, d.OH, d.OW, d.K), dtype=f32, device=x.device)
        else:
            _chk_y(d, out)
        _chk(w)
        outs.append(out)
    ks = [d.K for d, _, _, _, _ in problems]
    assert len(problems) <= 4, len(problems)
    tab = (_GroupEntry * len(problems))()
    for i, ((d, w, bias, epi, _), out) in enumerate(zip(problems, outs)):
        tab[i] = _GroupEntry(w.data_ptr(), out.data_ptr(), bias.data_ptr() if bias is not None else 0, d.K, int(d.ldy),
                             int(epi), 0)
    dsum = None
    if ACCOUNT is not None or PROFILER is not None:
        dsum = ConvDesc(d0.N, d0.H, d0.W, d0.C, sum(ks), 1, 1, d0.OH, d0.OW, 1, 1, 0, 0, 0)
    t0 = PROFILER.begin(dsum, 0) if PROFILER is not None else None
    if ACCOUNT is not None:
        ACCOUNT.add(dsum, 0)
    lib().conv2d_fwd_grouped(ctypes.byref(d0), ptr(_chk(x)), len(problems), ctypes.addressof(tab), max(ks), sum(ks), _stream())
    if t0 is not None:
        PROFILER.end(dsum, 0, t0)
    return outs


SEG_DGRAD = os.environ.get("MTLSSL_SEG_DGRAD", "1") != "0"


class _SegEntry(ctypes.Structure):
    _fields_ = [("dy", ctypes.c_void_p), ("w", ctypes.c_void_p), ("K", ctypes.c_int32), ("ldy", ctypes.c_int32)]


def conv2d_dgrad_segmented(segments, residual=None, mask_ref=None, epilogue=0):
    d0 = segments[0][0]
    assert 1 <= len(segments) <= 4, len(segments)
    tab = (_SegEntry * len(segments))()
    for i, (d, dy, w) in enumerate(segments):
        assert desc_is_pointwise(d) and (d.N, d.H, d.W, d.C) == (d0.N, d0.H, d0.W, d0.C) and d.K % 16 == 0, (d.C, d.K)
        tab[i] = _SegEntry(_chk_y(d, dy).data_ptr(), _chk(w).data_ptr(), d.K, int(d.ldy))
    dx = torch.empty((d0.N, d0.H, d0.W, d0.C), dtype=f32, device=segments[0][1].device)
    dsum = None
    if ACCOUNT is not None or PROFILER is not None:
        dsum = ConvDesc(d0.N, d0.H, d0.W, d0.C, sum(d.K for d, _, _ in segments), 1, 1, d0.OH, d0.OW, 1, 1, 0, 0, 0)
    t0 = PROFILER.begin(dsum, 1) if PROFILER is not None else None
    if ACCOUNT is not None:
        ACCOUNT.add(dsum, 1)
    lib().conv2d_dgrad_segmented(ctypes.byref(d0), len(segments), ctypes.addressof(tab), ptr(residual), ptr(mask_ref), ptr(dx),
                                 int(epilogue), _stream())
    if t0 is not None:
        PROFILER.end(dsum, 1, t0)
    return dx


def depthwise_fwd(d, x, w, bias=None, epilogue=0):
    y = torch.empty((d.N, d.OH, d.OW, d.K), dtype=f32, device=x.device)
    t0 = _hbm_begin("depthwise_fwd")
    lib().depthwise_fwd(ctypes.byref(d), ptr(_chk(x)), ptr(_chk(w)), ptr(bias), ptr(y), epilogue, _stream())
    if t0 is not None:
        HBM_PROFILER.end("depthwise_fwd", 4 * (x.numel() + y.numel()), t0)
    return y


def depthwise_dgrad(d, dy, w, mask_ref=None, epilogue=0):
    dx = torch.empty((d.N, d.H, d.W, d.C), dtype=f32, device=dy.device)
    t0 = _hbm_begin("depthwise_dgrad")
    lib().depthwise_dgrad(ctypes.byref(d), ptr(_chk(dy)), ptr(_chk(w)), ptr(mask_ref), ptr(dx), epilogue,
                          _stream())
    if t0 is not None:
        HBM_PROFILER.end("depthwise_dgrad", 4 * (dy.numel() + dx.numel() + (dx.numel() if mask_ref is not None else 0)), t0)
    return dx


def depthwise_wgrad(d, x, dy, dw, out_scale=None, beta=0.0):
    ws = workspace(lib().depthwise_wgrad_workspace_bytes(ctypes.byref(d)), "dwgrad", x.device)
    t0 = _hbm_begin("depthwise_wgrad")
    lib().depthwise_wgrad(ctypes.byref(d), ptr(_chk(x)), ptr(_chk(dy)), ptr(out_scale), ptr(dw), float(beta),
                          ptr(ws), _stream())
    if t0 is not None:
        HBM_PROFILER.end("depthwise_wgrad", 4 * (x.numel() + dy.numel()), t0)
    return dw


def bn_param_grads(y, g, gamma, beta_param, dgamma, dbeta, beta=0.0):
    C = y.shape[-1]
    ws = workspace(lib().bn_param_grads_workspace_bytes(int(C)), "bngrad", y.device)
    lib().bn_param_grads(ptr(_chk(y)), ptr(_chk(g)), ptr(gamma), ptr(beta_param), ptr(dgamma), ptr(dbeta),
                         y.numel() // C, int(C), float(beta), ptr(ws), _stream())
    return dgamma, dbeta


def pool_geometry(H, W, k, stride, padding):
    if padding == "SAME":
        pt, OH = same_pad(H, k, stride)
        pl, OW = same_pad(W, k, stride)
    else:
        pt = pl = 0
        OH, OW = (H - k) // stride + 1, (W - k) // stride + 1
    return pt, pl, OH, OW


def _slice_ld(t, C):
    assert t.is_cuda and t.dtype == f32 and t.dim() == 4 and t.shape[-1] == C and t.stride(-1) == 1 \
        and t.stride(-3) == t.stride(-2) * t.shape[-2], (tuple(t.shape), t.stride())
    return int(t.stride(-2))

# ... 799 lines not shown
```

### mtl_ssl_amd/resnet.py

```python
import torch

from . import nn, ops

RESNET_UNITS = {"resnet_v1_50": (3, 4, 6, 3), "resnet_v1_101": (3, 4, 23, 3),
                "resnet_v1_152": (3, 8, 36, 3)}


class BoxClassifierTower(nn.Tower):
    out_act = "relu"
    supports_wgrad_stream = True

    def __init__(self, ps, scope, arch, cin, trainable, weight_decay, bn_trainable=False):
        self.stack = nn.BlockStack(ps, "%s/%s" % (scope, arch), cin,
                                   [("block4", 512, 3, 1, trainable)], None, 1, weight_decay, bn_trainable)
        self.trainable = trainable
        self.cout = self.stack.cout

    def layers(self):
        return self.stack.layers()

    def forward(self, crops, save):
        x, ctxs = crops, []
        for u in self.stack.units:
            x, c = u.forward(x, save)
            ctxs.append(c)
        return x, (ctxs if save else None)

    def backward(self, g_out, out, ctxs, need_input_grad, masked=False, wgrad=nn.INLINE_WGRAD):
        gp = g_out if masked else ops.relu_bwd(out, g_out)
        units = self.stack.units
        for i in range(len(units) - 1, -1, -1):
            first = i == 0
            gp = units[i].backward(gp, ctxs[i], need_input_grad=(need_input_grad or not first),
                                   mask_input=not first, wgrad=wgrad)
        return gp


class FasterRCNNResnetV1FeatureExtractor(nn.FeatureExtractor):
    channel_means = (123.68, 116.779, 103.939)
    out_act = "relu"
    supports_wgrad_stream = True

    def __init__(self, ps, architecture, is_training, first_stage_features_stride=16,
                 weight_decay=0.0, freeze_layer="block1", batch_norm_trainable=False,
                 first_stage_scope="FirstStageFeatureExtractor"):
        super().__init__(ps, is_training, first_stage_features_stride, weight_decay)
        self.bn_trainable = bool(batch_norm_trainable) and bool(is_training)
        self.arch = architecture
        n_freeze = int(freeze_layer[-1]) if freeze_layer else 0
        bt = [False] * n_freeze + [bool(is_training)] * (4 - n_freeze)
        units = RESNET_UNITS[architecture]
        prefix = "%s/%s" % (first_stage_scope, architecture)
        self.conv1 = nn.ConvBN(ps, prefix + "/conv1", 3, 64, 7, 2, 1, "RESNET_SAME", False, weight_decay,
                               gamma_init=0.015, bn_trainable=self.bn_trainable)
        blocks = [("block1", 64, units[0], 2, bt[0]), ("block2", 128, units[1], 2, bt[1]),
                  ("block3", 256, units[2], 2, bt[2])]
        self.trunk = nn.BlockStack(ps, prefix, 64, blocks, first_stage_features_stride // 4, 1, weight_decay,
                                   self.bn_trainable)
        self.cout = self.trunk.cout
        self._neg_means = None
        self.first_trainable = 0 if self.bn_trainable else next(
            (i for i, u in enumerate(self.trunk.units) if u.trainable), len(self.trunk.units))

    def layers(self):
        return [self.conv1] + self.trunk.layers()

    def preprocess(self, resized_inputs):
        if self._neg_means is None:
            self._neg_means = torch.tensor([-m for m in self.channel_means], dtype=torch.float32,
                                           device=resized_inputs.device)
        return ops.bias_add_channels(resized_inputs, self._neg_means)

    def extract_proposal_features(self, x, save=True):
        self.check_inputs(x)
        y1 = self.conv1.forward(x)
        x, pads = ops.maxpool_fwd(y1, 3, 2, "SAME")
        ctxs = []
        if save and self.bn_trainable:
            self._root_ctx = (y1, x, pads)
        for i, u in enumerate(self.trunk.units):
            x, c = u.forward(x, save and i >= self.first_trainable)
            ctxs.append(c)
        return x, ctxs

    def backward_proposal_features(self, gp, ctxs, wgrad=nn.INLINE_WGRAD):
        units = self.trunk.units
        for i in range(len(units) - 1, self.first_trainable - 1, -1):
            gp = units[i].backward(gp, ctxs[i], need_input_grad=(i > self.first_trainable or self.bn_trainable),
                                   wgrad=wgrad)
        if self.bn_trainable:
            y1, pooled, pads = self._root_ctx
            g1 = ops.maxpool_bwd(y1, pooled, gp, 3, 2, pads)
            self.conv1.bn_grad(y1, ops.relu_bwd(y1, g1))
            self._root_ctx = None

    def box_classifier_tower(self, scope, trainable):
        return BoxClassifierTower(self.ps, scope, self.arch, self.cout, trainable and self.is_training,
                                  self.weight_decay, self.bn_trainable and trainable)
```

### mtl_ssl_amd/vgg.py

```python
import torch

from . import nn, ops

_GROUPS = ((2, 64), (2, 128), (3, 256), (3, 512), (3, 512))
_INIT = ("variance_scaling", 1.0, "FAN_AVG", True)
FREEZE_LAYERS = ("",) + tuple("conv%d" % g for g in range(1, len(_GROUPS) + 1))


def trainable_groups(freeze_layer, is_training):
    if freeze_layer not in FREEZE_LAYERS:
        raise ValueError("faster_rcnn_vgg_16: feature_extractor.freeze_layer must be one of %s, got %r — the proto default "
                         "'block1' names a ResNet block, so a VGG config must set the field"
                         % (", ".join(repr(v) for v in FREEZE_LAYERS), freeze_layer))
    n = int(freeze_layer[-1]) if freeze_layer else 0
    return [bool(is_training) and g > n for g in range(1, len(_GROUPS) + 1)]


class IdentityTower(nn.Tower):
    out_act = None
    trainable = False

    def __init__(self, cin):
        self.cout = cin

    def layers(self):
        return []

    def forward(self, crops, save):
        return crops, None

    def backward(self, g_out, out, ctx, need_input_grad, masked=False, wgrad=nn.INLINE_WGRAD):
        return g_out if need_input_grad else None


class FasterRCNNVgg16FeatureExtractor(nn.FeatureExtractor):
    channel_means = (102.9801, 115.9465, 122.7717)
    out_act = "relu"
    supports_rfcn = False

    def __init__(self, ps, is_training, first_stage_features_stride=16, weight_decay=0.0005, freeze_layer="",
                 first_stage_scope="FirstStageFeatureExtractor"):
        super().__init__(ps, bool(is_training), first_stage_features_stride, weight_decay)
        self.group_trainable = trainable_groups(freeze_layer, is_training)
        self.groups = []
        cin = 3
        for g, (n, cout) in enumerate(_GROUPS, 1):
            convs = []
            for i in range(1, n + 1):
                convs.append(nn.Conv(ps, "%s/vgg_16/conv%d/conv%d_%d" % (first_stage_scope, g, g, i), cin, cout, 3, _INIT,
                                     self.group_trainable[g - 1], weight_decay, activation="relu"))
                cin = cout
            self.groups.append(convs)
        self.cout = cin
        self.first_trainable = next((g for g, t in enumerate(self.group_trainable) if t), len(_GROUPS))
        self._means = None

    def layers(self):
        return [l for convs in self.groups for l in convs]

    def preprocess(self, resized_inputs):
        if self._means is None:
            self._means = torch.tensor(self.channel_means, dtype=torch.float32, device=resized_inputs.device)
        return ops.preprocess_bgr(resized_inputs.contiguous(), self._means)

    def extract_proposal_features(self, x, save=True):
        self.check_inputs(x)
        ctx = []
        for g, convs in enumerate(self.groups):
            keep = save and self.is_training and g >= self.first_trainable
            xs = []
            for l in convs:
                xs.append(x)
                x = l.forward(x)
            last, pooled, pads = x, None, None
            if g < len(self.groups) - 1:
                pooled, pads = ops.maxpool_fwd(x, 2, 2, "VALID")
                x = pooled
            ctx.append((xs, last, pooled, pads) if keep else None)
        return x, (ctx if save else None)

    def backward_proposal_features(self, gp, ctx, wgrad=nn.INLINE_WGRAD):
        if not self.is_training:
            return
        for g in range(len(self.groups) - 1, self.first_trainable - 1, -1):
            xs, last, pooled, pads = ctx[g]
            if pooled is not None:
                gp = ops.maxpool_bwd(last, pooled, gp, 2, 2, pads)
            convs = self.groups[g]
            for i in range(len(convs) - 1, -1, -1):
                convs[i].wgrad(xs[i], gp)
                if i == 0 and g == self.first_trainable:
                    return
                gp = convs[i].dgrad(xs[i].shape, gp, mask_ref=xs[i])

    def box_classifier_tower(self, scope, trainable):
        return IdentityTower(self.cout)
```

Measured before the change: 38.10 images/sec.

## Skip zero-gradient proposal rows in closeness tower pointwise conv backward

```diff
diff --git a/include/mtlssl_hip.h b/include/mtlssl_hip.h
--- a/include/mtlssl_hip.h
+++ b/include/mtlssl_hip.h
@@ -14,7 +14,7 @@
 #define MTLSSL_ELAUNCH (-2)
 #define MTLSSL_ECOMM (-3)
 
-#define MTLSSL_ABI_VERSION 20
+#define MTLSSL_ABI_VERSION 21
 
 const char* mtlssl_last_error(void);
 int mtlssl_abi_version(void);
@@ -90,6 +90,15 @@
 int mtlssl_conv2d_force_config(const mtlssl_conv_desc* d, int mode, int cfg);
 int mtlssl_conv2d_set_winograd(int mode);
 int mtlssl_conv2d_set_pointwise(int on);
+int mtlssl_conv2d_dgrad_rs(const mtlssl_conv_desc* d, const float* dy, const float* w, const float* residual,
+                           const float* mask_ref, float* dx, int epilogue, void* workspace, const float* filter_xf,
+                           int xf_variant, const uint8_t* group_active, int rows_per_group, mtlssl_stream_t stream);
+int mtlssl_conv2d_wgrad_rs(const mtlssl_conv_desc* d, const float* x, const float* dy,
+                           const float* out_scale, float* dw, float* dbias, const float* dbias_scale, float beta,
+                           void* workspace, const float* input_xf, int input_variant, const uint8_t* group_active,
+                           int rows_per_group, mtlssl_stream_t stream);
+int mtlssl_row_group_flags(const float* scale, int n, uint8_t* flags, mtlssl_stream_t stream);
+int mtlssl_conv2d_set_row_skip(int on);
 int mtlssl_conv2d_set_fp32_engine(int mode);
 int mtlssl_conv2d_num_dispatches(const mtlssl_conv_desc* d, int mode);
 #define MTLSSL_PLAN_INFO_LEN 16
diff --git a/mtl_ssl_amd/csrc/conv.hip b/mtl_ssl_amd/csrc/conv.hip
--- a/mtl_ssl_amd/csrc/conv.hip
+++ b/mtl_ssl_amd/csrc/conv.hip
@@ -9,6 +9,38 @@
 
 namespace mtlssl {
 
+__global__ void __launch_bounds__(256) k_row_group_flags(const float* __restrict__ scale, int n, uint8_t* __restrict__ flags) {
+  const int i = blockIdx.x * blockDim.x + threadIdx.x;
+  if (i < n) flags[i] = scale[i] != 0.f;
+}
+__global__ void __launch_bounds__(256) k_active_ksteps(const uint8_t* __restrict__ flags, int rpg, int P, int pps, int stride,
+                                                       int* __restrict__ out) {
+  const int z = blockIdx.x, pix0 = z * pps, pix1 = min(P, pix0 + pps);
+  const int ksteps = (max(pix1 - pix0, 0) + BK - 1) / BK;
+  const int lane = threadIdx.x & 63, w = threadIdx.x >> 6;
+  int* list = out + KSTEP_HDR + (int64_t)z * stride;
+  __shared__ int wave_cnt[4];
+  int base = 0;
+  for (int s0 = 0; s0 < ksteps; s0 += 256) {
+    const int s = s0 + threadIdx.x;
+    bool act = false;
+    if (s < ksteps) {
+      const int r0 = pix0 + s * BK, r1 = min(r0 + BK, pix1) - 1;
+      for (int g = r0 / rpg; g <= r1 / rpg; ++g) act |= flags[g] != 0;
+    }
+    const unsigned long long m = __ballot(act);
+    if (lane == 0) wave_cnt[w] = __popcll(m);
+    __syncthreads();
+    int off = base;
+    for (int i = 0; i < w; ++i) off += wave_cnt[i];
+    if (act) list[off + __popcll(m & ((1ull << lane) - 1ull))] = s;
+    base += wave_cnt[0] + wave_cnt[1] + wave_cnt[2] + wave_cnt[3];
+    __syncthreads();
+  }
+  if (threadIdx.x == 0) out[z] = base;
+}
+static inline int64_t kstep_list_bytes(int64_t P) { return align_up((KSTEP_HDR + 2 * cdiv(P, BK) + 128) * 4, 256); }
+static std::atomic<int>& row_skip_ref() { static std::atomic<int> v{1}; return v; }
 
 __global__ void __launch_bounds__(256) k_wgrad_reduce(const float* ws, int nsplit, int64_t total4, int K,
                                                       const float* scale, float* dw, float beta, int main_blocks,
@@ -1395,7 +1427,15 @@
 int mtlssl_conv2d_dgrad_xf(const mtlssl_conv_desc* d, const float* dy, const float* w,
                            const float* residual, const float* mask_ref, float* dx, int epi,
                            void* workspace, const float* filter_xf, int xf_variant, mtlssl_stream_t stream) {
+  return mtlssl_conv2d_dgrad_rs(d, dy, w, residual, mask_ref, dx, epi, workspace, filter_xf, xf_variant, nullptr, 0, stream);
+}
+
+int mtlssl_conv2d_dgrad_rs(const mtlssl_conv_desc* d, const float* dy, const float* w,
+                           const float* residual, const float* mask_ref, float* dx, int epi,
+                           void* workspace, const float* filter_xf, int xf_variant, const uint8_t* group_active,
+                           int rows_per_group, mtlssl_stream_t stream) {
   if (int rc = check_desc(d)) return rc;
+  MTLSSL_REQUIRE(!group_active || rows_per_group > 0, "conv_dgrad: group_active needs rows_per_group > 0");
   MTLSSL_REQUIRE(!(epi & MASK_ANY) || mask_ref, "conv_dgrad: mask_ref pointer required");
   MTLSSL_REQUIRE(!(epi & MTLSSL_EPI_RESIDUAL) || residual, "conv_dgrad: residual pointer required");
   ConvArgs p = make_args(d);
@@ -1416,6 +1456,10 @@
       parity_dgrad(r, d, dy, w, residual, mask_ref, dx, epi, workspace, S(stream));
       break;
     case FAM_DIRECT:
+      if (group_active && row_skip_ref().load() != 0 && desc_is_pointwise(d)) {
+        p.group_active = group_active;
+        p.rows_per_group = rows_per_group;
+      }
       launch_planned<MODE_DGRAD>(r.plan, p, (float*)workspace, S(stream));
       break;
     case FAM_PADDED: {
@@ -1487,6 +1531,19 @@
   const int prev = wino_env();
   if (mode >= 0 && mode <= 2) { wino_mode_ref().store(mode); routes_clear(); }
   return prev;
+}
+
+int mtlssl_conv2d_set_row_skip(int on) {
+  const int prev = row_skip_ref().load();
+  if (on == 0 || on == 1) row_skip_ref().store(on);
+  return prev;
+}
+
+int mtlssl_row_group_flags(const float* scale, int n, uint8_t* flags, mtlssl_stream_t stream) {
+  if (n <= 0) return MTLSSL_OK;
+  MTLSSL_REQUIRE(scale && flags, "row_group_flags: null pointer");
+  hipLaunchKernelGGL(k_row_group_flags, dim3(cdiv(n, 256)), dim3(256), 0, S(stream), scale, n, flags);
+  return check_launch("row_group_flags");
 }
 
 int mtlssl_conv2d_set_pointwise(int on) {
@@ -1552,7 +1609,8 @@
 
 int64_t mtlssl_conv2d_wgrad_workspace_bytes(const mtlssl_conv_desc* d) {
   if (!d) return 256;
-  return colsum_bytes(d) + route(d, MODE_WGRAD).bytes;
+  return colsum_bytes(d) + route(d, MODE_WGRAD).bytes +
+         (desc_is_pointwise(d) ? kstep_list_bytes((int64_t)d->N * d->OH * d->OW) : 0);
 }
 
 static void wgrad_group_plan(const mtlssl_conv_desc* d, int n, int* cfg, int* nsplit, int* pps) {
@@ -1619,7 +1677,16 @@
 int mtlssl_conv2d_wgrad_ex(const mtlssl_conv_desc* d, const float* x, const float* dy,
                            const float* out_scale, float* dw, float* dbias, const float* dbias_scale, float beta,
                            void* workspace, const float* input_xf, int input_variant, mtlssl_stream_t stream) {
+  return mtlssl_conv2d_wgrad_rs(d, x, dy, out_scale, dw, dbias, dbias_scale, beta, workspace, input_xf, input_variant,
+                                nullptr, 0, stream);
+}
+
+int mtlssl_conv2d_wgrad_rs(const mtlssl_conv_desc* d, const float* x, const float* dy,
+                           const float* out_scale, float* dw, float* dbias, const float* dbias_scale, float beta,
+                           void* workspace, const float* input_xf, int input_variant, const uint8_t* group_active,
+                           int rows_per_group, mtlssl_stream_t stream) {
   if (int rc = check_desc(d)) return rc;
+  MTLSSL_REQUIRE(!group_active || rows_per_group > 0, "conv_wgrad: group_active needs rows_per_group > 0");
   hipStream_t st = S(stream);
   ConvArgs p = make_args(d);
   p.a = x; p.b = dy;
@@ -1657,6 +1724,14 @@
       p.out = ws_main;
       p.M = d->C; p.NG = d->K; p.nsplit = ns; p.pix_per_split = pps;
       p.cs_part = ride ? (float*)workspace : nullptr;
+      if (group_active && row_skip_ref().load() != 0 && !split && desc_is_pointwise(d) && pointwise_ref().load() != 0 &&
+          ns <= KSTEP_HDR) {
+        int* list = (int*)((char*)ws_main + r.bytes);
+        const int stride = (int)cdiv(pps, BK);
+        hipLaunchKernelGGL(k_active_ksteps, dim3(ns), dim3(256), 0, st, group_active, rows_per_group, (int)P, pps, stride, list);
+        p.k_steps = list;
+        p.k_stride = stride;
+      }
       if (split) launch_split<MODE_WGRAD, false>(p, dim3(1, d->R * d->S, ns), st);
       else launch_mfma<MODE_WGRAD>(r.wg.cfg, p, dim3(1, d->R * d->S, ns), st);
       int64_t total4 = (int64_t)d->R * d->S * d->C * d->K / 4;
diff --git a/mtl_ssl_amd/csrc/conv_mfma.h b/mtl_ssl_amd/csrc/conv_mfma.h
--- a/mtl_ssl_amd/csrc/conv_mfma.h
+++ b/mtl_ssl_amd/csrc/conv_mfma.h
@@ -44,7 +44,19 @@
   int64_t a_bs, b_bs, o_bs;
   const float* const* a_tab;
   const float* const* b_tab;
+  const uint8_t* group_active;
+  int rows_per_group;
+  const int* k_steps;
+  int k_stride;
 };
+constexpr int KSTEP_HDR = 64;
+
+__device__ __forceinline__ bool tile_rows_active(const ConvArgs& p, int m0, int bm) {
+  const int g1 = (min(m0 + bm, p.M) - 1) / p.rows_per_group;
+  bool any = false;
+  for (int g = m0 / p.rows_per_group; g <= g1; ++g) any |= p.group_active[g] != 0;
+  return any;
+}
 
 typedef unsigned uintx4 __attribute__((ext_vector_type(4)));
 __host__ __device__ __forceinline__ int args_ldy(const ConvArgs& p) { return p.ldy ? p.ldy : p.K; }
@@ -231,6 +243,7 @@
   }
   const int ldy = args_ldy(p);
   int rs_fixed = 0, pix0 = 0, pix1 = 0, ksteps, ks_begin = 0;
+  const int* steps = nullptr;
   if constexpr (MODE == MODE_FWD) {
     ksteps = p.R * p.S * (p.C / BKT);
   } else if constexpr (MODE == MODE_DGRAD) {
@@ -242,6 +255,11 @@
     pix0 = split * p.pix_per_split;
     pix1 = min(P, pix0 + p.pix_per_split);
     ksteps = (max(pix1 - pix0, 0) + BKT - 1) / BKT;
+    if constexpr (PW && !BATCH)
+      if (p.k_steps) {
+        steps = p.k_steps + KSTEP_HDR + split * p.k_stride;
+        ksteps = p.k_steps[split];
+      }
   }
   unsigned a_rec = p.a_bytes, b_rec = p.b_bytes;
   if constexpr (PW && MODE == MODE_WGRAD) {
@@ -256,6 +274,8 @@
       ksteps = min(ksteps, ks_begin + p.ks_per_split);
     }
   }
+  if constexpr (PW && MODE == MODE_DGRAD && !SEG && !BATCH)
+    if (p.group_active && !tile_rows_active(p, m0, BM)) ksteps = ks_begin;
 
   int a_base[A_LD], a_y[A_LD], a_x[A_LD], a_n[A_LD];
   bool a_ok[A_LD];
@@ -532,16 +552,22 @@
       for (int e = 0; e < 16; ++e) acc[i][j][e] = 0.f;
 
   const int nk = ksteps - ks_begin;
+  auto kmap = [&](int it) { return steps ? steps[it] : ks_begin + it; };
+  int step_pf = 0;
   if (nk > 0) {
-    load_tile(ks_begin, Set0{});
+    load_tile(kmap(0), Set0{});
     store_tile(0, Set0{});
   }
-  if (nk > 1) load_tile(ks_begin + 1, Set1{});
+  if (nk > 1) load_tile(kmap(1), Set1{});
+  if (steps && nk > 2) step_pf = steps[2];
   __syncthreads();
   auto kstep = [&](int it, auto next, auto spare) {
     const int cur = it & 1;
     if constexpr (!(LAB & 1))
-      if (it + 2 < nk) load_tile(ks_begin + it + 2, spare);
+      if (it + 2 < nk) {
+        load_tile(steps ? step_pf : ks_begin + it + 2, spare);
+        if (steps && it + 3 < nk) step_pf = steps[it + 3];
+      }
     const float* a = sA + cur * (BKT * LDA) + wr * (BM / WR) + lo;
     const float* b = sB + cur * (BKT * LDB) + wc * (BN / 2) + lo;
     float fa[2][TM], fb[2][TN];
@@ -642,6 +668,7 @@
     if constexpr (MODE != MODE_WGRAD) p.out += (int64_t)blockIdx.y * p.o_bs;
   }
   int rs_fixed = 0, pix0 = 0, pix1 = 0, ksteps, ks_begin = 0;
+  const int* steps = nullptr;
   if constexpr (MODE == MODE_FWD) {
     ksteps = p.R * p.S * (p.C / BKT);
   } else if constexpr (MODE == MODE_DGRAD) {
@@ -653,6 +680,11 @@
     pix0 = split * p.pix_per_split;
     pix1 = min(P, pix0 + p.pix_per_split);
     ksteps = (max(pix1 - pix0, 0) + BKT - 1) / BKT;
+    if constexpr (PWISE && !BATCH)
+      if (p.k_steps) {
+        steps = p.k_steps + KSTEP_HDR + split * p.k_stride;
+        ksteps = p.k_steps[split];
+      }
   }
   if constexpr (MODE != MODE_WGRAD) {
     if (p.nsplit > 1) {
@@ -660,6 +692,8 @@
       ksteps = min(ksteps, ks_begin + p.ks_per_split);
     }
   }
+  if constexpr (PWISE && MODE == MODE_DGRAD && !BATCH)
+    if (p.group_active && !tile_rows_active(p, m0, BM)) ksteps = ks_begin;
 
   const int ldy = args_ldy(p);
   unsigned a_rec = p.a_bytes, b_rec = p.b_bytes;
@@ -856,9 +890,11 @@
 
   const int nk = ksteps - ks_begin;
   constexpr int NDMA = ((LAB & 64) ? 0 : PA) + ((LAB & 128) ? 0 : PB);
+  int step_pf = 0;
 #pragma unroll
   for (int s = 0; s < NSTAGE - 1; ++s)
-    if (s < nk) issue_tile(ks_begin + s, s);
+    if (s < nk) issue_tile(steps ? steps[s] : ks_begin + s, s);
+  if (steps && NSTAGE - 1 < nk) step_pf = steps[NSTAGE - 1];
   if (NSTAGE == 3 && nk > 1) asm volatile("s_waitcnt vmcnt(%0)" ::"n"(NDMA) : "memory");
   else asm volatile("s_waitcnt vmcnt(0)" ::: "memory");
   __builtin_amdgcn_s_barrier();
@@ -872,7 +908,10 @@
   for (int it = 0; it < nk; ++it) {
     const bool more = it + NSTAGE - 1 < nk;
     if constexpr (!(LAB & 1))
-      if (more) issue_tile(ks_begin + it + NSTAGE - 1, nxt);
+      if (more) {
+        issue_tile(steps ? step_pf : ks_begin + it + NSTAGE - 1, nxt);
+        if (steps && it + NSTAGE < nk) step_pf = steps[it + NSTAGE];
+      }
     const float* a = smem + cur * STAGE;
     const float* b = a + A_FL;
     if constexpr (CS)
diff --git a/mtl_ssl_amd/frcnn.py b/mtl_ssl_amd/frcnn.py
--- a/mtl_ssl_amd/frcnn.py
+++ b/mtl_ssl_amd/frcnn.py
@@ -731,6 +731,7 @@
             losses["closeness_classification_loss"] = ops.reduce_sum(rl)
             if want_grad:
                 d["closeness_predictions"] = d_clo
+                pd["_clo_active"] = ops.row_group_flags(clo_s)
         return cls_s
 
     def _loss_refined_classifier(self, pd, cls_s, losses, d, want_grad):
@@ -829,7 +830,11 @@
                 cfeat = pd["_cfeat"]
                 g = self.closeness_predictor.backward(pd["_cp"], d["closeness_predictions"], None, cfeat.shape,
                                                       **self.closeness_tower.out_mask(cfeat))
-                gc = self.closeness_tower.backward(g, cfeat, pd["_cctx"], need_input_grad=not stop, masked=True)
+                active = pd.get("_clo_active")
+                if active is not None:
+                    active.record_stream(torch.cuda.current_stream())
+                gc = self.closeness_tower.backward(g, cfeat, pd["_cctx"], need_input_grad=not stop, masked=True,
+                                                   active=active)
                 if not stop:
                     todo.append((gc, pd["_argmax"], pd["proposal_boxes_normalized"].view(-1, 4), pd["_box_ind"]))
             if mtl.window:
diff --git a/mtl_ssl_amd/inception_resnet_v2.py b/mtl_ssl_amd/inception_resnet_v2.py
--- a/mtl_ssl_amd/inception_resnet_v2.py
+++ b/mtl_ssl_amd/inception_resnet_v2.py
@@ -303,7 +303,7 @@
         out = self.conv_7b.forward(x)
         return out, ((c7, ctxs, x) if save else None)
 
-    def backward(self, g_out, out, ctx, need_input_grad, masked=False, wgrad=nn.INLINE_WGRAD):
+    def backward(self, g_out, out, ctx, need_input_grad, masked=False, wgrad=nn.INLINE_WGRAD, active=None):
         c7, ctxs, pre7b = ctx
         gp = g_out if masked else ops.relu_bwd(out, g_out)
         wgrad.run(self.conv_7b, pre7b, gp)
diff --git a/mtl_ssl_amd/lib.py b/mtl_ssl_amd/lib.py
--- a/mtl_ssl_amd/lib.py
+++ b/mtl_ssl_amd/lib.py
@@ -73,7 +73,7 @@
             fn.argtypes = argtypes
             if restype is ctypes.c_int and name not in ("mtlssl_abi_version", "mtlssl_conv2d_tile_config", "mtlssl_conv2d_num_dispatches",
                                                         "mtlssl_conv2d_set_winograd", "mtlssl_conv2d_set_fp32_engine", "mtlssl_conv2d_filter_xf_variant",
-                                                        "mtlssl_conv2d_set_pointwise"):
+                                                        "mtlssl_conv2d_set_pointwise", "mtlssl_conv2d_set_row_skip"):
                 setattr(self, name[len("mtlssl_"):], self._checked(fn, name))
             else:
                 setattr(self, name[len("mtlssl_"):], fn)
diff --git a/mtl_ssl_amd/mobilenet.py b/mtl_ssl_amd/mobilenet.py
--- a/mtl_ssl_amd/mobilenet.py
+++ b/mtl_ssl_amd/mobilenet.py
@@ -48,7 +48,7 @@
         a13 = self.pw13.forward(d13)
         return a13, ((crops, d12, a12, d13) if save else None)
 
-    def backward(self, g_out, out, ctx, need_input_grad, masked=False, wgrad=nn.INLINE_WGRAD):
+    def backward(self, g_out, out, ctx, need_input_grad, masked=False, wgrad=nn.INLINE_WGRAD, active=None):
         crops, d12, a12, d13 = ctx
         gp = g_out if masked else ops.relu6_bwd(out, g_out)
         self.pw13.bn_grad(out, gp)
diff --git a/mtl_ssl_amd/nn.py b/mtl_ssl_amd/nn.py
--- a/mtl_ssl_amd/nn.py
+++ b/mtl_ssl_amd/nn.py
@@ -19,24 +19,24 @@
     def __init__(self, stream):
         self.stream = stream
 
-    def run(self, layer, x, g):
+    def run(self, layer, x, g, **kw):
         if not layer.trainable:
             return
         ev = torch.cuda.Event()
         ev.record(torch.cuda.current_stream())
         self.stream.wait_event(ev)
-        for t in (x, g):
+        for t in (x, g) + tuple(kw.values()):
             t.record_stream(self.stream)
         with torch.cuda.stream(self.stream):
-            layer.wgrad(x, g)
+            layer.wgrad(x, g, **kw)
 
 
 class _InlineWgrad:
     stream = None
 
     @staticmethod
-    def run(layer, x, g):
-        layer.wgrad(x, g)
+    def run(layer, x, g, **kw):
+        layer.wgrad(x, g, **kw)
 
 
 INLINE_WGRAD = _InlineWgrad()
@@ -156,16 +156,17 @@
             self._kept.clear()
         return self._kept
 
-    def wgrad(self, x, g):
+    def wgrad(self, x, g, active=None):
         if self.trainable:
             db = self.ps.grad(self.beta.name) if (self.bn_trainable and self.gamma is None) else None
             ops.conv2d_wgrad(self.desc(x.shape), x, g, self.ps.grad(self.w.name), out_scale=self.scale,
-                             dbias=db, beta=1.0, input_xf=self._kept.pop(x.data_ptr(), None))
+                             dbias=db, beta=1.0, input_xf=self._kept.pop(x.data_ptr(), None), active=active)
             self.ps.grad_ready(self.w, self.beta if db is not None else None)
 
-    def dgrad(self, x_shape, g, residual=None, mask_ref=None, out=None, accum=False, mask6=False):
+    def dgrad(self, x_shape, g, residual=None, mask_ref=None, out=None, accum=False, mask6=False, active=None):
         return ops.conv2d_dgrad(self.desc(x_shape), g, self.w_eff, residual, mask_ref,
-                                dgrad_epilogue(residual, accum, mask_ref, mask6), out=out, xf_cache=self.ps.filter_cache)
+                                dgrad_epilogue(residual, accum, mask_ref, mask6), out=out, xf_cache=self.ps.filter_cache,
+                                active=active)
 
 
 class DepthwiseBN(_FrozenBN):
@@ -328,7 +329,8 @@
             ctx = ctx + (out, sc)
         return out, ctx
 
-    def backward(self, gp, ctx, need_input_grad=True, mask_input=True, wgrad=INLINE_WGRAD):
+    def backward(self, gp, ctx, need_input_grad=True, mask_input=True, wgrad=INLINE_WGRAD, active=None):
+        kw = {} if active is None else dict(active=active)
         x, a1, a2, sc_sub = ctx[:4]
         if self.bn_trainable:
             out, sc = ctx[4], ctx[5]
@@ -337,26 +339,26 @@
             del o3
             if self.shortcut is not None:
                 self.shortcut.bn_grad(sc, gp)
-        wgrad.run(self.conv3, a2, gp)
-        gp2 = self.conv3.dgrad(a2.shape, gp, mask_ref=a2)
+        wgrad.run(self.conv3, a2, gp, **kw)
+        gp2 = self.conv3.dgrad(a2.shape, gp, mask_ref=a2, **kw)
         if self.bn_trainable:
             self.conv2.bn_grad(a2, gp2)
         wgrad.run(self.conv2, a1, gp2)
         gp1 = self.conv2.dgrad(a1.shape, gp2, mask_ref=a1)
         if self.bn_trainable:
             self.conv1.bn_grad(a1, gp1)
-        wgrad.run(self.conv1, x, gp1)
+        wgrad.run(self.conv1, x, gp1, **kw)
         if self.shortcut is not None:
-            wgrad.run(self.shortcut, x, gp)
+            wgrad.run(self.shortcut, x, gp, **kw)
         if not need_input_grad:
             return None
         if self.shortcut is not None:
-            addend = self.shortcut.dgrad(x.shape, gp)
+            addend = self.shortcut.dgrad(x.shape, gp, **kw)
         elif self.stride > 1:
             addend = ops.maxpool_bwd(x, sc_sub, gp, 1, self.stride, (0, 0))
         else:
             addend = gp
-        return self.conv1.dgrad(x.shape, gp1, residual=addend, mask_ref=x if mask_input else None)
+        return self.conv1.dgrad(x.shape, gp1, residual=addend, mask_ref=x if mask_input else None, **kw)
 
 
 class BlockStack:
@@ -396,7 +398,7 @@
     def out_mask(cls, feat):
         return dict(mask_ref=None if cls.out_act is None else feat, mask6=cls.out_act == "relu6")
 
-    def backward(self, g_out, out, ctx, need_input_grad, masked=False, wgrad=INLINE_WGRAD):
+    def backward(self, g_out, out, ctx, need_input_grad, masked=False, wgrad=INLINE_WGRAD, active=None):
         raise NotImplementedError
 
 
diff --git a/mtl_ssl_amd/ops.py b/mtl_ssl_amd/ops.py
--- a/mtl_ssl_amd/ops.py
+++ b/mtl_ssl_amd/ops.py
@@ -497,7 +497,24 @@
     return y
 
 
-def conv2d_dgrad(d, dy, w, residual=None, mask_ref=None, epilogue=0, out=None, xf_cache=None):
+def set_row_skip(on):
+    return lib().conv2d_set_row_skip(int(on))
+
+
+def row_group_flags(scale):
+    flags = torch.empty(scale.numel(), dtype=torch.uint8, device=scale.device)
+    lib().row_group_flags(ptr(_chk(scale)), scale.numel(), ptr(flags), _stream())
+    return flags
+
+
+def _active_arg(d, active, rows=None):
+    if active is None:
+        return None, 0
+    assert active.dtype == torch.uint8 and active.is_contiguous() and active.numel() == d.N, (active.dtype, active.shape, d.N)
+    return ptr(active), rows if rows is not None else d.OH * d.OW
+
+
+def conv2d_dgrad(d, dy, w, residual=None, mask_ref=None, epilogue=0, out=None, xf_cache=None, active=None):
     dx = out if out is not None else torch.empty((d.N, d.H, d.W, d.C), dtype=f32, device=dy.device)
     if PROFILER is None:
         def run():
@@ -510,14 +527,14 @@
         ACCOUNT.add(d, 1)
     ws = _conv_ws(d, 1, dy.device)
     U, variant = xf_cache.get(d, 1, w) if (xf_cache is not None and d.R == 3 and d.S == 3) else (None, -1)
-    lib().conv2d_dgrad_xf(ctypes.byref(d), ptr(_chk_y(d, dy)), ptr(_chk(w)), ptr(residual), ptr(mask_ref),
-                          ptr(dx), epilogue, ptr(ws), ptr(U), variant, _stream())
+    lib().conv2d_dgrad_rs(ctypes.byref(d), ptr(_chk_y(d, dy)), ptr(_chk(w)), ptr(residual), ptr(mask_ref),
+                          ptr(dx), epilogue, ptr(ws), ptr(U), variant, *_active_arg(d, active, d.H * d.W), _stream())
     if t0 is not None:
         PROFILER.end(d, 1, t0)
     return dx
 
 
-def conv2d_wgrad(d, x, dy, dw, out_scale=None, dbias=None, beta=0.0, input_xf=None, dbias_scale=None):
+def conv2d_wgrad(d, x, dy, dw, out_scale=None, dbias=None, beta=0.0, input_xf=None, dbias_scale=None, active=None):
     if PROFILER is None:
         def run():
             tmp = workspace(4 * d.R * d.S * d.C * d.K, "tune_out", x.device)
@@ -531,8 +548,8 @@
     V, vvar = input_xf if input_xf is not None else (None, -1)
     if V is not None:
         V.record_stream(torch.cuda.current_stream())
-    lib().conv2d_wgrad_ex(ctypes.byref(d), ptr(_chk(x)), ptr(_chk_y(d, dy)), ptr(out_scale), ptr(dw),
-                          ptr(dbias), ptr(dbias_scale), float(beta), ptr(ws), ptr(V), vvar, _stream())
+    lib().conv2d_wgrad_rs(ctypes.byref(d), ptr(_chk(x)), ptr(_chk_y(d, dy)), ptr(out_scale), ptr(dw),
+                          ptr(dbias), ptr(dbias_scale), float(beta), ptr(ws), ptr(V), vvar, *_active_arg(d, active), _stream())
     if t0 is not None:
         PROFILER.end(d, 2, t0)
     return dw
diff --git a/mtl_ssl_amd/resnet.py b/mtl_ssl_amd/resnet.py
--- a/mtl_ssl_amd/resnet.py
+++ b/mtl_ssl_amd/resnet.py
@@ -26,13 +26,13 @@
             ctxs.append(c)
         return x, (ctxs if save else None)
 
-    def backward(self, g_out, out, ctxs, need_input_grad, masked=False, wgrad=nn.INLINE_WGRAD):
+    def backward(self, g_out, out, ctxs, need_input_grad, masked=False, wgrad=nn.INLINE_WGRAD, active=None):
         gp = g_out if masked else ops.relu_bwd(out, g_out)
         units = self.stack.units
         for i in range(len(units) - 1, -1, -1):
             first = i == 0
             gp = units[i].backward(gp, ctxs[i], need_input_grad=(need_input_grad or not first),
-                                   mask_input=not first, wgrad=wgrad)
+                                   mask_input=not first, wgrad=wgrad, active=active)
         return gp
 
 
diff --git a/mtl_ssl_amd/vgg.py b/mtl_ssl_amd/vgg.py
--- a/mtl_ssl_amd/vgg.py
+++ b/mtl_ssl_amd/vgg.py
@@ -29,7 +29,7 @@
     def forward(self, crops, save):
         return crops, None
 
-    def backward(self, g_out, out, ctx, need_input_grad, masked=False, wgrad=nn.INLINE_WGRAD):
+    def backward(self, g_out, out, ctx, need_input_grad, masked=False, wgrad=nn.INLINE_WGRAD, active=None):
         return g_out if need_input_grad else None
 
 
```

Measured after the change: 40.75 images/sec (median of 6 runs). +7.0%, better.
